# Rickyeeeeee/ParallelRayTracing

Measured on AMD Instinct MI355X. Metric: Mrays/sec at 1920x1080, 4 bounces, ~1M-tri scene, higher is better.
Workload: dtype f32; 1 GPU; C3: dragon.ply refined by longest-edge bisection = 870000 triangles + ground quad + emissive quad, 1920x1080, max_depth 5 segments (= 4 bounces), 256 spp per step (15360 spp timed of the config's 256), image tiled over 1 GPU(s) + per-step gather to rank 0; triangles=870000, bvh_nodes=681504, bvh_max_depth=25, bvh8_nodes=137301, bvh8_depth=9, width=1920, height=1080, max_depth=5, samples_in_flight=256, seed=0, jitter=0, variant=0, gather=render stream

## Files before the change

parallelraytracing_amd/csrc/prt_api.cpp:

```cpp
#include <hip/hip_runtime.h>

#include <algorithm>
#include <atomic>
#include <cfloat>
#include <chrono>
#include <cmath>
#include <cstdarg>
#include <cstdio>
#include <cstdlib>
#include <cstring>
#include <limits>
#include <string>
#include <utility>
#include <vector>

#include "../../include/prt.h"
#include "bvh.h"
#include "bvh_gpu.h"
#include "prt_adaptive.h"
#include "prt_denoise.h"
#include "prt_denoise_contract.h"
#include "prt_devmem.h"
#include "prt_feature_samples.h"
#include "prt_features.h"
// ... 12 lines not shown

int prt_dev_alloc(void** p, size_t bytes) {
    const hipError_t e = hipMalloc(p, bytes);
    if (e == hipSuccess) g_live_bytes += bytes, ++g_alloc_calls;
    return (int)e;
}
void prt_dev_free(void* p, size_t bytes) {
    (void)hipFree(p);
    g_live_bytes -= bytes;
}
int prt_dev_copy_in(void* dst, const void* src, size_t bytes) { return (int)hipMemcpy(dst, src, bytes, hipMemcpyHostToDevice); }
void prt_dev_adopted(size_t bytes) { g_live_bytes += bytes; }
void prt_dev_taken(size_t bytes) { g_live_bytes -= bytes; }
int prt_pinned_alloc(void** p, size_t bytes) { return (int)hipHostMalloc(p, bytes, hipHostMallocDefault); }
void prt_pinned_free(void* p) { (void)hipHostFree(p); }
int prt_event_create(void** ev, bool timing) {
    return (int)(timing ? hipEventCreate((hipEvent_t*)ev) : hipEventCreateWithFlags((hipEvent_t*)ev, hipEventDisableTiming));
}
void prt_event_destroy(void* ev) { (void)hipEventDestroy((hipEvent_t)ev); }

namespace {

constexpr float kPadCoeff = 1.0f / 262144.0f;
constexpr size_t kRayStatWords = (size_t)PRT_RAY_STAT_SLOTS * PRT_MAX_DEPTH;
constexpr uint32_t kTravStatsWords = 16 + PRT_TIMELINE_WORDS * (PRT_MAX_DEPTH + 1);
constexpr size_t kLightStatWords = 2 * (size_t)PRT_RAY_STAT_SLOTS;

struct EventPair {
    DevEvent a, b;
    int kind = 0;
};

hipEvent_t ev(const DevEvent& e) { return (hipEvent_t)e.h; }

struct RayMem {
    DevBuf o, d, t, hit, hd2;
    int alloc(uint64_t n) {
        int e = o.ensure(n * sizeof(float4));
        if (!e) e = d.ensure(n * sizeof(float4));
        if (!e) e = t.ensure(n * sizeof(float4));
        if (!e) e = hit.ensure(n * sizeof(uint32_t));
        if (!e) e = hd2.ensure(n * sizeof(float));
        return e;
    }
    PrtRayBuf view() const { return PrtRayBuf{o.as<float4>(), d.as<float4>(), t.as<float4>(), hit.as<uint32_t>(), hd2.as<float>()}; }
};
struct BuiltTree {
    DevBuf nodes8, tris, nrms;
    uint32_t n_nodes = 0;
};
struct SceneMem {
    DevBuf prims, mat_rgbs, mat_type, nodes, nodes4, nodes8, insts, tlas_inst, abvh_nodes, abvh_order, tris, nrms, lights, prim_light;
    DevBuf refit_keep;
};
struct MeshLightMem {
    DevBuf records, thr, bucket, runs;
    DevBuf lc_boxes, lc_range, lc_members, lc_thr, lc_cand, lc_pmf;
};
struct EnvMem {
    DevBuf texels, row, col, last;
};
struct TexMem {
    DevBuf texels, desc, mat, uvs, inst;
};
struct PathMem {
    RayMem rays[2];
    DevBuf rad;
};
struct LightMem {
    RayMem sh;
    DevBuf pdf_b, lrad;
};
struct PrimaryMem {
    DevBuf pid, list, hit;
};
struct FilmMem {
    DevBuf local;
    DevBuf stat;
    DevBuf tile_sel;
    PinnedBuf tile_count;
};
struct WorkMem {
    DevBuf counts;
    DevBuf ray_stats;
    DevBuf trav_stats;
    DevBuf work;
    DevBuf pix;
    DevBuf sort;
    DevBuf light_stats;
    PinnedBuf flag;
    PinnedBuf counts_host;
    DevEvent ev_counts[PRT_MAX_DEPTH + 2];
    DevEvent ev_prod[PRT_MAX_DEPTH + 2];
};

}

struct PrtContext {
    int device = -1;
    bool has_device = false;
    hipStream_t own_stream = nullptr;
    hipStream_t stream = nullptr;
    std::string err;

    bool has_scene = false;
    PrtHostScene hs;
    double refit_ms = 0.0;
    struct RefitKeep {
        bool ready = false;
        std::vector<uint32_t> tri_first, vert_first, level_start;
        uint32_t n_nodes = 0, n_light_tris = 0;
        uint32_t *d_corner = nullptr, *d_csr_start = nullptr, *d_csr_corner = nullptr, *d_light_tris = nullptr, *d_valid = nullptr;
        float *d_normals = nullptr, *d_light_verts = nullptr;
        PrtRefitScratch scratch{};
    } rk;
    bool host_copies_stale = false;
    PrtRefitInfo rinfo{};
    PrtCopyTally* tally = nullptr;
    PrtInstanceUpdateInfo inst_info{};
    DevScene dsc{};
    SceneMem scene;

    bool has_camera = false;
    DevCamera cam{};

    bool has_film = false;
    PrtTileMap tm{};
    uint32_t valid_local = 0;
    FilmMem film;
    bool film_stats = false;
    uint32_t tile_sel_entries = 0;

    uint32_t S = 1;
    uint64_t cap_paths = 0;
    PathMem path;
    PrtRayBuf rb[2] = {{nullptr, nullptr, nullptr, nullptr, nullptr}, {nullptr, nullptr, nullptr, nullptr, nullptr}};
    WorkMem wk;
    unsigned long long* ray_stats_target = nullptr;
    bool pix_records_blank = false;

    DevBuf scratch;

    bool timing = false;
    std::vector<EventPair> events;
    std::vector<EventPair> event_pool;
    PrtStats stats{};
    uint64_t dead_paths = 0;
    int variant = 0;
    int abvh_enabled = 1;
    int measure_spp = 1;
    float pad_coeff = kPadCoeff;
    int node_stride = 0;
    int compact_primary = 1;
    int primary_walk = 1;
    const char* shade_instance = "";
    const char* batch_instance[4] = {"", "", "", ""};
    bool batch_walked = false;
    int gpu_build = 0;
    PrtSampling sampling{0u, 0u, 0.0f};
    PrtLens lens{0.0f, 0.0f, 0.0f};
    PrtTravTuning tune{1024u, 256u, 16u, 0xFFFFFFFFu , 0u, 2u, 0u , 0u, 0u, 0u, 1u, 8u, 1u, 0u, nullptr, 0u, 2500000u, 2u , 8u , 96u , 32u , 1u};
    unsigned long long* d_shade_div = nullptr;
    uint32_t last_segment = 2;
    uint32_t last_segment_active = 0;
    uint32_t last_batch_depth = 0;
    uint32_t sort_rays = 0;
    size_t sort_entries = 0, sort_temp = 0;
    hipStream_t count_stream = nullptr;
    uint32_t pix_entries = 0;
    PrimaryMem prim;
    uint64_t prim_pid_entries = 0;
    uint32_t prim_pix_entries = 0;
    PrtPrimaryKey primary_key{};
    uint64_t camera_gen = 1, scene_gen = 1;
    uint32_t primary_counts[2] = {0u, 0u};
    int primary_reuse = 1;
    uint32_t primary_reuse_active = 0;
    uint32_t primary_reused_batches = 0;
    DevBuf spill;

    uint32_t lighting = PRT_LIGHTING_OFF;
    uint32_t light_sources = PRT_LIGHT_SOURCES_ANALYTIC;
    uint32_t light_selection = PRT_LIGHT_SELECTION_POWER;
    uint32_t light_max_clusters = 0;
    int light_buckets = 1;
    MeshLightMem ml;
    LightMem light;
    PrtLightBufs lb{};
    uint64_t cap_light = 0;

    PrtEnvTables env;
    EnvMem envm;
    uint64_t t_env_dev = 0;

    PrtTexTables tex;
    TexMem texm;
    uint64_t tex_bytes = 0;

    DevBuf feat;
    uint32_t feat_W = 0, feat_H = 0;
    bool feat_valid = false;
    PrtFeatureTrace ftrace{0u, 0.1f};
    DevBuf guide;
    bool guide_valid = false;
    PrtFeatureSampling fsamp{0u, 0u, 0u};
    DevBuf samp;
    bool samp_valid = false;
    int feature_chunk = 0;
    int radiance_chunk = 0;
    int bake_chunk = 0;
    DevBuf bake;
    DevBuf dn;
    DevBuf tp;
    DevBuf tp_mt;
    DevBuf tpa;
    uint32_t tp_W = 0, tp_H = 0;
    int tp_set = 0;
    bool tp_valid = false;
    PrtCameraBasis tp_K{};
    std::vector<float> tp_mats;
    std::vector<uint32_t> tp_mt_host;
    PrtTemporalInfo tp_info{};
    int dn_lds = 1;
};

namespace {

int fail(PrtContext* c, int code, const char* fmt, ...) {
    if (c) {
        char buf[512];
        va_list ap;
        va_start(ap, fmt);
        vsnprintf(buf, sizeof(buf), fmt, ap);
        va_end(ap);
        c->err = buf;
    }
    return code;
}

#define HIPCHECK(c, call)                                                                              \
    do {                                                                                               \
        const hipError_t e_ = (hipError_t)(call);                                                      \
        if (e_ != hipSuccess) return fail((c), PRT_ERR_HIP, "%s failed: %s", #call, hipGetErrorString(e_)); \
    } while (0)

int need_device(PrtContext* c) {
    if (!c) return PRT_ERR_INVALID;
    if (!c->has_device)
        return fail(c, PRT_ERR_NO_DEVICE,
                    "no HIP device bound to this context: the MI355X kernels are the only compute path (no CPU fallback)");
    const hipError_t e = hipSetDevice(c->device);
    if (e != hipSuccess) return fail(c, PRT_ERR_HIP, "hipSetDevice(%d) failed: %s", c->device, hipGetErrorString(e));
    return PRT_OK;
}

void drop_history(PrtContext* c) {
    c->tp_valid = false;
    c->tp_info.steps = 0;
    c->tp_info.hit_pixels = 0;
    c->tp_info.reprojected = 0;
    ++c->tp_info.resets;
}

int ensure(PrtContext* c, DevBuf& buf, size_t need) {
    HIPCHECK(c, buf.ensure(need));
    return PRT_OK;
}

int commit(PrtContext* c, const PrtWorkspace& ws, DevBuf& buf) {
    const int rc = ensure(c, buf, ws.bytes());
    if (rc || ws.bind(buf.p, buf.bytes)) return rc;
    return fail(c, PRT_ERR_INVALID, "a workspace of %d arrays in %zu bytes does not fit its buffer of %zu", ws.regions(), ws.bytes(), buf.bytes);
}

template <class T>
int upload(PrtContext* c, T* dst, const T* src, size_t count) {
    HIPCHECK(c, hipMemcpyAsync(dst, src, count * sizeof(T), hipMemcpyHostToDevice, c->stream));
    return PRT_OK;
}
template <class T>
int download(PrtContext* c, T* dst, const T* src, size_t count) {
    HIPCHECK(c, hipMemcpyAsync(dst, src, count * sizeof(T), hipMemcpyDeviceToHost, c->stream));
    return PRT_OK;
}

PrtFeatureBufs feature_view(void* base, size_t n) {
    float4* a = (float4*)base;
    return PrtFeatureBufs{a, a + n, a + 2 * n};
}

struct ChainScratch {
    float *o, *d;
    float4* s[4];
    uint32_t* cnt;
    void declare(PrtWorkspace& ws, size_t n) {
        ws.add(&o, 3 * n).add(&d, 3 * n);
        for (float4*& p : s) ws.add(&p, n);
        ws.add(&cnt, PRT_FEATURE_MAX_SPECULAR + 1u);
    }
};

struct FilterScratch {
    float4 *rec = nullptr, *cv0 = nullptr, *cv1 = nullptr;
    float *out = nullptr, *var = nullptr;
    void declare_arrays(PrtWorkspace& ws, size_t n) { ws.add(&rec, 3 * n).add(&cv0, n).add(&cv1, n); }
    int commit_film(PrtContext* c, size_t n) {
        PrtWorkspace ws;
        ws.add(&cv0, n).add(&cv1, n).add(&out, 3 * n).add(&var, n);
        return commit(c, ws, c->dn);
    }
};

void declare_history(PrtWorkspace& ws, PrtHistoryBufs* h, size_t n) { ws.add(&h->cn, n).add(&h->nrm, n).add(&h->pos, n).add(&h->mm, n); }

struct TemporalScratch {
    PrtHistoryBufs cur, prev, next;
    void declare(PrtWorkspace& ws, size_t n) {
        declare_history(ws, &cur, n);
        declare_history(ws, &prev, n);
        next.nrm = next.pos = nullptr;
        ws.add(&next.cn, n).add(&next.mm, n);
    }
};

int ensure_path_state(PrtContext* c, uint64_t n_paths) {
    if (n_paths <= c->cap_paths) return PRT_OK;
    c->path = PathMem();
    c->cap_paths = 0;
    const uint64_t n = std::max<uint64_t>(n_paths, 256);
    int e = c->path.rays[0].alloc(n);
    if (!e) e = c->path.rays[1].alloc(n);
    if (!e) e = c->path.rad.ensure(n * sizeof(float4));
    for (int i = 0; i < 2; ++i) c->rb[i] = c->path.rays[i].view();
    HIPCHECK(c, e);
    c->cap_paths = n;
    return PRT_OK;
}

void touch_scene(PrtContext* c) { ++c->scene_gen; }
void touch_camera(PrtContext* c) { ++c->camera_gen; }

int ensure_primary_state(PrtContext* c, uint64_t n_paths, uint32_t n_pix_local) {
    if (n_paths > c->prim_pid_entries) {
        c->primary_key.valid = false;
        c->prim_pid_entries = 0;
        const uint64_t n = std::max<uint64_t>(n_paths, 256);
        HIPCHECK(c, c->prim.pid.ensure(n * sizeof(uint32_t)));
        c->prim_pid_entries = n;
    }
    if (n_pix_local > c->prim_pix_entries) {
        c->primary_key.valid = false;
        c->prim_pix_entries = 0;
        const uint32_t n = std::max<uint32_t>(n_pix_local, 256u);
        HIPCHECK(c, c->prim.list.ensure((size_t)n * sizeof(uint32_t)));
        HIPCHECK(c, c->prim.hit.ensure((size_t)n * sizeof(uint32_t)));
        c->prim_pix_entries = n;
    }
    return PRT_OK;
}

int ensure_light_state(PrtContext* c, uint64_t n_paths) {
    if (!c->wk.light_stats.p) {
        HIPCHECK(c, c->wk.light_stats.ensure(kLightStatWords * sizeof(unsigned long long)));
        HIPCHECK(c, hipMemsetAsync(c->wk.light_stats.p, 0, kLightStatWords * sizeof(unsigned long long), c->stream));
    }
    c->lb.stats = c->wk.light_stats.as<unsigned long long>();
    if (n_paths <= c->cap_light) return PRT_OK;
    c->light = LightMem();
    c->cap_light = 0;
    const uint64_t n = std::max<uint64_t>(n_paths, 256);
    int e = c->light.sh.alloc(n);
    if (!e) e = c->light.pdf_b.ensure(n * sizeof(float));
    if (!e) e = c->light.lrad.ensure(n * sizeof(float4));
    c->lb.sh = c->light.sh.view();
    c->lb.pdf_b = c->light.pdf_b.as<float>();
    c->lb.lrad = c->light.lrad.as<float4>();
    HIPCHECK(c, e);
    c->cap_light = n;
    return PRT_OK;
}

bool mesh_lights_on(const PrtContext* c) { return (c->light_sources & PRT_LIGHT_SOURCES_MESH) != 0u; }

DevLights dev_lights(const PrtContext* c) {
    const uint32_t mode = c->lighting == PRT_LIGHTING_NEE ? (uint32_t)PRT_LIGHTING_NEE : (uint32_t)PRT_LIGHTING_NEE_MIS;
    if (mesh_lights_on(c)) return DevLights{c->ml.records.as<float4>(), c->scene.prim_light.as<uint32_t>(), c->hs.ml.n_search, mode};
    return DevLights{c->scene.lights.as<float4>(), c->scene.prim_light.as<uint32_t>(), (uint32_t)(c->hs.lights.size() / (4 * PRT_LIGHT_F4)), mode};
}

DevMeshLights dev_mesh_lights(const PrtContext* c) {
    return DevMeshLights{c->ml.thr.as<uint32_t>(), c->light_buckets ? c->ml.bucket.as<uint32_t>() : nullptr,
                         c->ml.runs.as<DevLightRun>(), c->hs.ml.bucket_shift, (uint32_t)c->hs.ml.runs.size()};
}

bool clusters_on(const PrtContext* c) { return mesh_lights_on(c) && c->light_selection == (uint32_t)PRT_LIGHT_SELECTION_CLUSTERED; }

DevLightClusters dev_light_clusters(const PrtContext* c) {
    const MeshLightMem& m = c->ml;
    return DevLightClusters{m.lc_boxes.as<float4>(), m.lc_range.as<uint4>(), m.lc_members.as<uint32_t>(),
                            m.lc_thr.as<uint32_t>(), m.lc_cand.as<uint32_t>(), m.lc_pmf.as<float>(), c->hs.lc.n_clusters()};
}

uint32_t light_set_size(const PrtContext* c) {
    return mesh_lights_on(c) ? (uint32_t)c->hs.ml.visible.size() : (uint32_t)(c->hs.lights.size() / (4 * PRT_LIGHT_F4));
}

bool env_on(const PrtContext* c) { return c->env.W != 0u; }
uint64_t env_threshold(const PrtContext* c) { return prt_environment_threshold(c->env, light_set_size(c)); }

DevEnv dev_env(const PrtContext* c) {
    const uint64_t te = env_threshold(c);
    return DevEnv{c->envm.texels.as<float4>(), c->envm.row.as<uint32_t>(), c->envm.col.as<uint32_t>(),
                  c->envm.last.as<uint32_t>(), c->env.W, c->env.H, c->env.row_last, (uint32_t)te, te == 4294967296ull ? 1u : 0u,
                  (float)((double)te / 4294967296.0)};
}

int upload_env(PrtContext* c) {
    HIPCHECK(c, hipSetDevice(c->device));
    HIPCHECK(c, hipStreamSynchronize(c->stream));
    c->envm = EnvMem();
    if (!env_on(c)) return PRT_OK;
    HIPCHECK(c, c->envm.texels.alloc_copy(c->env.texels.data(), c->env.texels.size() * 4));
    HIPCHECK(c, c->envm.row.alloc_copy(c->env.row_thr.data(), c->env.row_thr.size() * 4));
    HIPCHECK(c, c->envm.col.alloc_copy(c->env.col_thr.data(), c->env.col_thr.size() * 4));
    HIPCHECK(c, c->envm.last.alloc_copy(c->env.col_last.data(), c->env.col_last.size() * 4));
    return PRT_OK;
}

bool tex_on(const PrtContext* c) { return c->tex.is_set && c->tex.n_textured_materials != 0u; }

DevTex dev_tex(const PrtContext* c) {
    return DevTex{c->texm.texels.as<float4>(), c->texm.desc.as<uint4>(), c->texm.mat.as<uint32_t>(), c->texm.uvs.as<float2>(),
                  c->texm.inst.as<uint32_t>(), c->tex.n_textures};
}

void free_tex(PrtContext* c) {
    c->texm = TexMem();
    c->tex_bytes = 0;
}

int upload_tex(PrtContext* c) {
    HIPCHECK(c, hipSetDevice(c->device));
    HIPCHECK(c, hipStreamSynchronize(c->stream));
    free_tex(c);
    if (!c->tex.is_set) return PRT_OK;
    auto up = [&](DevBuf& dst, const auto& src) {
        const int e = dst.alloc_copy(src.data(), src.size() * 4);
        if (!e) c->tex_bytes += src.size() * 4;
        return e;
    };
    const PrtTexTables& t = c->tex;
    HIPCHECK(c, up(c->texm.texels, t.texels));
    HIPCHECK(c, up(c->texm.desc, t.desc));
    HIPCHECK(c, up(c->texm.mat, t.mat_tex));
    HIPCHECK(c, up(c->texm.uvs, t.uvs));
    HIPCHECK(c, up(c->texm.inst, t.inst_uv_base));
    return PRT_OK;
}

void drop_tex(PrtContext* c) {
    if (c->has_device && c->texm.texels.p) {
        (void)hipSetDevice(c->device);
        (void)hipStreamSynchronize(c->stream);
        free_tex(c);
    }
    c->tex = PrtTexTables();
}

int sync_light_tables(PrtContext* c) {
    const uint64_t te = env_threshold(c);
    if (te == c->t_env_dev || !c->has_device) return PRT_OK;
    std::vector<float> a, b;
    const bool ml = mesh_lights_on(c) && c->ml.records.p;
    prt_scaled_light_tables(c->hs, te, &a, ml ? &b : nullptr);
    HIPCHECK(c, hipSetDevice(c->device));
    HIPCHECK(c, hipStreamSynchronize(c->stream));
    if (!a.empty() && c->scene.lights.p) HIPCHECK(c, hipMemcpy(c->scene.lights.p, a.data(), a.size() * 4, hipMemcpyHostToDevice));
    if (!a.empty() && c->scene.lights.p && c->tally) c->tally->h2d += a.size() * 4;
    if (ml && !b.empty()) HIPCHECK(c, hipMemcpy(c->ml.records.p, b.data(), b.size() * 4, hipMemcpyHostToDevice));
    if (ml && !b.empty() && c->tally) c->tally->h2d += b.size() * 4;
    if (ml && c->ml.lc_pmf.p) {
        prt_cluster_pmf_in(c->hs, te, &a);
        if (!a.empty()) HIPCHECK(c, hipMemcpy(c->ml.lc_pmf.p, a.data(), a.size() * 4, hipMemcpyHostToDevice));
        if (!a.empty() && c->tally) c->tally->h2d += a.size() * 4;
    }
    c->t_env_dev = te;
    return PRT_OK;
}

int upload_mesh_lights(PrtContext* c) {
    static_assert(sizeof(DevLightRun) == sizeof(PrtLightRun), "DevLightRun is PrtLightRun");
    HIPCHECK(c, hipSetDevice(c->device));
    HIPCHECK(c, hipStreamSynchronize(c->stream));
    c->ml = MeshLightMem();
    const PrtMeshLights& ml = c->hs.ml;
    auto up = [&](DevBuf& dst, const void* src, size_t bytes) {
        const int e = dst.alloc_copy(src, bytes);
        if (!e && c->tally) c->tally->h2d += bytes;
        return e;
    };
    HIPCHECK(c, up(c->ml.records, ml.records.data(), ml.records.size() * 4));
    HIPCHECK(c, up(c->ml.thr, ml.thr.data(), ml.thr.size() * 4));
    HIPCHECK(c, up(c->ml.bucket, ml.bucket.data(), ml.bucket.size() * 4));
    HIPCHECK(c, up(c->ml.runs, ml.runs.data(), ml.runs.size() * sizeof(PrtLightRun)));
// ... 53 lines not shown
void free_scene(PrtContext* c) {
    drop_refit_keep(c);
    c->scene = SceneMem();
    c->ml = MeshLightMem();
    c->has_scene = false;
}

int read_ray_stats(PrtContext* c, const unsigned long long* d_set, unsigned long long (&out)[PRT_MAX_DEPTH]) {
    std::vector<unsigned long long> h(kRayStatWords);
    HIPCHECK(c, hipMemcpy(h.data(), d_set, kRayStatWords * sizeof(unsigned long long), hipMemcpyDeviceToHost));
    for (int d = 0; d < PRT_MAX_DEPTH; ++d) {
        out[d] = 0;
        for (size_t sl = 0; sl < PRT_RAY_STAT_SLOTS; ++sl) out[d] += h[sl * PRT_MAX_DEPTH + (size_t)d];
    }
    return PRT_OK;
}

int begin_event(PrtContext* c, int kind, EventPair* ep) {
    if (!c->timing) return PRT_OK;
    if (!c->event_pool.empty()) {
        *ep = std::move(c->event_pool.back());
        c->event_pool.pop_back();
    } else {
        HIPCHECK(c, ep->a.create(true));
        HIPCHECK(c, ep->b.create(true));
    }
    ep->kind = kind;
    HIPCHECK(c, hipEventRecord(ev(ep->a), c->stream));
    return PRT_OK;
}
int end_event(PrtContext* c, EventPair* ep) {
    if (!c->timing) return PRT_OK;
    HIPCHECK(c, hipEventRecord(ev(ep->b), c->stream));
    c->events.push_back(std::move(*ep));
    return PRT_OK;
}
int drain_events(PrtContext* c) {
    for (EventPair& ep : c->events) {
        float ms = 0.0f;
        HIPCHECK(c, hipEventSynchronize(ev(ep.b)));
        HIPCHECK(c, hipEventElapsedTime(&ms, ev(ep.a), ev(ep.b)));
        switch (ep.kind) {
            case 0: c->stats.raygen_ms += ms; break;
            case 1: c->stats.intersect_ms += ms; break;
            case 2: c->stats.shade_ms += ms; break;
            case 4: c->stats.scan_ms += ms; break;
            default: c->stats.accumulate_ms += ms; break;
        }
        c->event_pool.push_back(std::move(ep));
    }
    c->events.clear();
    return PRT_OK;
}

float lens_tan_fov_y(const PrtLens& l) { return l.fov_y == 0.0f ? tanf(0.5f) : tanf(0.5f * l.fov_y); }

f3 h_normalize(f3 v) {
    const float d = (v.x * v.x + v.y * v.y) + v.z * v.z;
    const float s = 1.0f / std::sqrt(d);
    return f3{v.x * s, v.y * s, v.z * s};
}
f3 h_cross(f3 a, f3 b) { return f3{a.y * b.z - b.y * a.z, a.z * b.x - b.z * a.x, a.x * b.y - b.x * a.y}; }

PrtBatchView whole_film(const PrtContext* c) { return PrtBatchView{c->tm, nullptr}; }

PrtWalkFacts walk_facts(const PrtContext* c, const PrtTravTuning& tune, PrtWalkRequest request, uint32_t max_rays, bool stats, bool primary) {
    PrtWalkFacts f{};
    f.has8 = c->dsc.nodes8 != nullptr, f.has4 = c->dsc.nodes4 != nullptr, f.has2 = c->dsc.nodes != nullptr;
    f.insts = c->dsc.n_insts != 0u, f.abvh = c->dsc.abvh_nodes != nullptr;
    f.depth8 = c->dsc.depth8, f.node_stride = c->dsc.node_stride, f.depth2 = c->hs.bvh.max_depth, f.max_stack4 = c->hs.bvh.max_stack4;
    f.wide = tune.wide, f.stack_lds = tune.stack_lds, f.stack_cap = tune.stack_cap, f.exit_max = tune.exit_max, f.tri_min = tune.tri_min;
    f.grid_blocks = tune.grid_blocks, f.steal = tune.steal, f.variant = c->variant, f.max_rays = max_rays, f.request = request, f.stats = stats, f.primary = primary;
    return f;
}

void walk_rays(PrtContext* c, const PrtRayBuf& rays, const uint32_t* count, uint32_t max_rays, bool any, const PrtTravTuning& tune,
               unsigned long long* stats, const PrtPrimary* primary, bool seeded = false) {
    const PrtWalkRequest request = !any ? PRT_WALK_CLOSEST : seeded ? PRT_WALK_SEEDED : PRT_WALK_ANY;
    const PrtWalkPlan plan = prt_plan_walk(walk_facts(c, tune, request, max_rays, stats != nullptr, primary != nullptr));
    prt_launch_walk(c->stream, plan, PrtWalkArgs{&c->dsc, rays, count, c->wk.work.as<uint32_t>(), c->spill.as<uint32_t>(), stats, primary, &tune});
}

int sort_front_rays(PrtContext* c, const PrtRayBuf& in, const uint32_t* front_count, uint32_t n_paths, EventPair* ep, PrtTravTuning* tune) {
    int rc;
    uint32_t n_front = 0;
    HIPCHECK(c, hipMemcpyAsync(&n_front, front_count, sizeof(uint32_t), hipMemcpyDeviceToHost, c->stream));
    HIPCHECK(c, hipStreamSynchronize(c->stream));
    if (n_front <= 1u) return PRT_OK;
    if (c->sort_entries < n_paths) {
        c->wk.sort = DevBuf();
        c->sort_entries = 0;
        c->sort_temp = prt_sort_rays_temp_bytes(n_paths);
        HIPCHECK(c, c->wk.sort.ensure(4 * (size_t)n_paths * sizeof(uint32_t) + c->sort_temp));
        c->sort_entries = n_paths;
    }
    EventPair es{};
    if ((rc = begin_event(c, 4, &es))) return rc;
    uint32_t* q = c->wk.sort.as<uint32_t>();
    if (prt_sort_rays(c->stream, in.o, in.d, n_front, c->dsc.root_min, c->dsc.root_max, c->sort_rays, q, q + n_paths,
                      q + 2 * (size_t)n_paths, q + 3 * (size_t)n_paths, q + 4 * (size_t)n_paths, c->sort_temp))
        return fail(c, PRT_ERR_HIP, "ray sort failed");
    if ((rc = end_event(c, &es))) return rc;
    if (c->timing) HIPCHECK(c, hipEventRecord(ev(ep->a), c->stream));
    tune->perm = q + 3 * (size_t)n_paths;
    return PRT_OK;
}

int run_batch(PrtContext* c, const PrtBatchView& view, uint32_t S_cur, uint32_t max_depth, uint32_t seed, uint32_t first_sample,
              bool accumulate, unsigned long long* trav_stats) {
    const PrtTileMap& tm = view.tm;
    if (view.list && !c->film.stat.p) return fail(c, PRT_ERR_INVALID, "a tile list needs film statistics");
    const uint64_t n_paths64 = (uint64_t)S_cur * tm.n_pix_local;
    c->batch_walked = false;
    c->primary_reuse_active = 0u;
    if (n_paths64 == 0) return PRT_OK;
    if (n_paths64 > 0xFFFFFF00ull) return fail(c, PRT_ERR_INVALID, "too many paths in flight");
    const uint32_t n_paths = (uint32_t)n_paths64;
    int rc = ensure_path_state(c, n_paths);
    if (rc) return rc;
    if ((rc = ensure_spill(c))) return rc;
    if ((rc = sync_light_tables(c))) return rc;
    const PrtWalkFacts wf = walk_facts(c, c->tune, PRT_WALK_PATH, n_paths, trav_stats != nullptr, false);
    PrtRouteFacts f{};
    f.lit = c->lighting != PRT_LIGHTING_OFF;
    f.mesh_lights = mesh_lights_on(c);
    f.light_clusters = clusters_on(c);
    f.env = env_on(c);
    f.tex = tex_on(c);
    f.lens = c->lens.aperture > 0.0f;
    f.listed = view.list != nullptr;
    f.film_stats = c->film_stats;
    f.has_nodes = c->dsc.n_nodes != 0u;
    f.has_bvh2 = wf.has2;
    f.insts = wf.insts;
    f.abvh = wf.abvh;
    f.few_prims = c->dsc.n_prims <= 16u;
    f.jitter = c->sampling.jitter != 0u;
    f.sa = c->sampling.rr_depth != 0u || c->sampling.clamp > 0.0f;
    f.multi_sample = S_cur > 1u;
    f.variant0 = wf.variant == 0;
    f.compact_primary = c->compact_primary;
    f.primary_walk = c->primary_walk;
    f.takes_primary = prt_traverse_takes_primary(wf);
    f.primary_hit = c->tune.primary_hit != 0u;
    f.path_gate = !trav_stats && !c->d_shade_div && c->sort_rays == 0u && n_paths <= c->tune.path_max && prt_path_kernel_applies(wf);
    f.path_kernel = c->tune.path_kernel;
    f.fuse = c->tune.fuse;
    f.mesh_emissive = c->hs.mesh_emissive;
    f.depth_ge2 = max_depth >= 2u;
    f.sort_rays = c->sort_rays != 0u;
    f.last_segment = c->last_segment;
    const PrtRoutePlan plan = prt_plan_route(f);
    const bool lit = f.lit, compact = plan.compact, walk = plan.walk;
    const DevEnv denv = dev_env(c);
    const DevTex dtex = dev_tex(c);
    const DevLens dlens{c->lens.aperture, c->lens.focus_distance};
    const bool exact = c->dsc.n_nodes != 0u && c->tune.exact_grids != 0u && (n_paths > (16384u * 512u) || c->tune.exact_grids == 2u);
    if (exact && !c->wk.counts_host.p) {
        HIPCHECK(c, c->wk.counts_host.alloc((PRT_MAX_DEPTH + 2) * 64 * sizeof(uint32_t)));
        for (DevEvent& e : c->wk.ev_counts) HIPCHECK(c, e.create(false));
        for (DevEvent& e : c->wk.ev_prod) HIPCHECK(c, e.create(false));
        HIPCHECK(c, hipStreamCreateWithFlags(&c->count_stream, hipStreamNonBlocking));
    }
    uint32_t* const d_counts = c->wk.counts.as<uint32_t>();
    uint32_t* const d_work = c->wk.work.as<uint32_t>();
    uint32_t* const h_counts = c->wk.counts_host.as<uint32_t>();
    float4* const d_rad = c->path.rad.as<float4>();
    auto read_back = [&](uint32_t d) -> hipError_t {
        hipError_t e = hipEventRecord(ev(c->wk.ev_prod[d]), c->stream);
        if (e == hipSuccess) e = hipStreamWaitEvent(c->count_stream, ev(c->wk.ev_prod[d]), 0);
        if (e == hipSuccess)
            e = hipMemcpyAsync(h_counts + 64 * (size_t)d, d_counts + (size_t)d * PRT_CNT_STRIDE, 33 * sizeof(uint32_t),
                               hipMemcpyDeviceToHost, c->count_stream);
        return e != hipSuccess ? e : hipEventRecord(ev(c->wk.ev_counts[d]), c->count_stream);
    };
    EventPair ep{};
    auto accumulate_batch = [&]() -> int {
        if ((rc = begin_event(c, 3, &ep))) return rc;
        const PrtAccumulateArgs aa{d_rad, lit ? c->lb.lrad : nullptr, c->film.local.as<float4>(), c->film.stat.as<float2>(), tm, S_cur, max_depth,
                                   accumulate, c->ray_stats_target, compact ? c->wk.pix.as<float4>() + tm.n_pix_local : nullptr, view.list};
        if (!prt_launch_accumulate(c->stream, plan.accumulate, aa)) return fail(c, PRT_ERR_INVALID, "no such accumulate instance");
        c->batch_instance[PRT_STAGE_ACCUMULATE] = prt_accumulate_name(plan.accumulate);
        if ((rc = end_event(c, &ep))) return rc;
        if (accumulate && !view.list) c->stats.samples += S_cur;
        HIPCHECK(c, hipGetLastError());
        return PRT_OK;
    };
    c->shade_instance = "";
    for (const char*& n : c->batch_instance) n = "";
    c->last_segment_active = plan.last_segment;
    c->last_batch_depth = plan.path ? 0u : max_depth;
    if (plan.path) {
        HIPCHECK(c, hipMemsetAsync(d_work, 0, 256 * sizeof(uint32_t), c->stream));
        PrtPathArgs pa{c->cam, tm, c->sampling, d_rad, first_sample, seed, max_depth, n_paths};
        if ((rc = begin_event(c, 1, &ep))) return rc;
        prt_launch_path(c->stream, prt_plan_walk(wf), c->dsc, pa, d_work, c->tune);
        if ((rc = end_event(c, &ep))) return rc;
        ++c->stats.intersect_launches;
        return accumulate_batch();
    }
    if (compact && c->pix_entries < tm.n_pix_local) {
        c->pix_entries = 0;
        c->primary_key.valid = false;
        HIPCHECK(c, c->wk.pix.ensure(4 * (size_t)tm.n_pix_local * sizeof(float4)));
        c->pix_entries = tm.n_pix_local;
        c->pix_records_blank = false;
    }
    const bool instrumented = trav_stats != nullptr || c->d_shade_div != nullptr;
    const bool persistent = compact && (walk || S_cur == 1u);
    if (persistent && (rc = ensure_primary_state(c, n_paths, tm.n_pix_local))) return rc;
    float4* const d_pix = c->wk.pix.as<float4>();
    PrtRayBuf rb0 = c->rb[0];
    if (persistent) rb0.t = c->prim.pid.as<float4>(), rb0.hd2 = c->prim.list.as<float>(), rb0.hit = c->prim.hit.as<uint32_t>();
    PrtPrimaryKey now{};
    now.valid = persistent && c->primary_reuse != 0 && !instrumented;
    if (now.valid) {
        const PrtWalkPlan wp0 = prt_plan_walk(walk_facts(c, c->tune, PRT_WALK_CLOSEST, walk ? tm.n_pix_local : n_paths, false, true));
        now.camera_gen = c->camera_gen, now.scene_gen = c->scene_gen;
        now.W = tm.W, now.H = tm.H, now.rank = tm.rank, now.world = tm.world, now.n_pix_local = tm.n_pix_local;
        now.S_cur = S_cur, now.max_depth = max_depth;
        now.plan = plan;
        now.walk_row = (uint32_t)wp0.launch[0].row, now.walk_prim = wp0.launch[0].prim;
        now.compact = compact, now.walk = walk, now.primary_hit = plan.primary_hit, now.lens = f.lens, now.jitter = f.jitter;
        now.rr_depth = c->sampling.rr_depth, now.clamp = c->sampling.clamp;
        now.listed = view.list != nullptr, now.instrumented = instrumented, now.exact = exact;
    }
    const bool reuse = prt_primary_reusable(c->primary_key, now);
    c->primary_reuse_active = reuse ? 1u : 0u;
    if (reuse) ++c->primary_reused_batches;
    if (reuse) HIPCHECK(c, hipMemsetAsync(d_counts + PRT_CNT_STRIDE, 0, (size_t)max_depth * PRT_CNT_STRIDE * sizeof(uint32_t), c->stream));
    else HIPCHECK(c, hipMemsetAsync(d_counts, 0, (size_t)(max_depth + 1) * PRT_CNT_STRIDE * sizeof(uint32_t), c->stream));
    const DevLights lt = dev_lights(c);
    const DevMeshLights mlt = dev_mesh_lights(c);
    const DevLightClusters lct = dev_light_clusters(c);
    if (lit) {
        if ((rc = ensure_light_state(c, n_paths))) return rc;
        HIPCHECK(c, hipMemsetAsync(c->lb.lrad, 0, (size_t)n_paths * sizeof(float4), c->stream));
    }
    c->batch_walked = walk;
    const PrtPrimary primary{(const uint32_t*)rb0.t, d_pix, {c->cam.pos.x, c->cam.pos.y, c->cam.pos.z}, tm.n_pix_local,
                             1.0f / (float)tm.n_pix_local, first_sample, seed, walk ? 1u : 0u};
    PrtPrimary primary_list = primary;
    if (walk) primary_list.pid = (const uint32_t*)rb0.hd2;
    c->batch_instance[PRT_STAGE_RAYGEN] = prt_raygen_name(plan.raygen);
    if (!reuse) {
        c->primary_key.valid = false;
        if ((rc = begin_event(c, 0, &ep))) return rc;
        const PrtRaygenArgs ra{&c->dsc, c->cam, tm, n_paths, first_sample, seed, max_depth, rb0, d_rad, d_counts, d_work, c->sampling,
                               compact ? d_pix : nullptr, walk, f.env ? &denv : nullptr, f.lens ? &dlens : nullptr, view.list};
        if (!prt_launch_raygen(c->stream, plan.raygen, ra)) return fail(c, PRT_ERR_INVALID, "no such raygen instance");
        if ((rc = end_event(c, &ep))) return rc;
        if (exact) HIPCHECK(c, read_back(0));
    }
    for (uint32_t d = 0; d < max_depth; ++d) {
        const PrtRayBuf& in = d == 0 ? rb0 : c->rb[d & 1];
        const PrtRayBuf& out = c->rb[(d + 1) & 1];
        const uint32_t* front_count = d_counts + (size_t)d * PRT_CNT_STRIDE;
        const PrtPrimary* prim_d = (compact && d == 0) ? &primary : nullptr;
        const bool held = reuse && d == 0;
        if (c->dsc.n_nodes && !held) {
            if ((rc = begin_event(c, 1, &ep))) return rc;
            PrtTravTuning tune = c->tune;
            tune.probe_slot = d;
            tune.perm = nullptr;
            if (plan.walk8 && c->sort_rays && !prim_d && (d > 0 || c->sampling.jitter || f.lens))
                if ((rc = sort_front_rays(c, in, front_count, n_paths, &ep, &tune))) return rc;
            if (walk && d == 0)
                walk_rays(c, in, d_counts + PRT_CNT_LIST, tm.n_pix_local, false, tune, trav_stats, &primary_list);
            else if (plan.last_segment == 2u && d + 1u == max_depth && !trav_stats)
                walk_rays(c, in, front_count, n_paths, true, tune, nullptr, nullptr, true);
            else
                walk_rays(c, in, front_count, n_paths, false, tune, trav_stats, prim_d);
            if ((rc = end_event(c, &ep))) return rc;
            ++c->stats.intersect_launches;
            if (prim_d) {
                if (plan.primary_hit) {
                    if ((rc = begin_event(c, 2, &ep))) return rc;
                    prt_launch_primary_hit(c->stream, c->dsc, primary, in.hit, d_pix, d_counts);
                    if ((rc = end_event(c, &ep))) return rc;
                    c->pix_records_blank = false;
                } else if (!c->pix_records_blank) {
                    HIPCHECK(c, hipMemsetAsync(d_pix + 2 * (size_t)tm.n_pix_local, 0xFF, 2 * (size_t)tm.n_pix_local * sizeof(float4), c->stream));
                    c->pix_records_blank = true;
                }
            }
        }
        uint32_t n_rays_known = 0xFFFFFFFFu;
        if (exact && held) {
            n_rays_known = c->primary_counts[0] + c->primary_counts[1];
        } else if (exact) {
            HIPCHECK(c, hipEventSynchronize(ev(c->wk.ev_counts[d])));
            n_rays_known = h_counts[64 * (size_t)d] + h_counts[64 * (size_t)d + 32];
            if (d == 0) c->primary_counts[0] = h_counts[0], c->primary_counts[1] = h_counts[32];
        }
        if (n_rays_known == 0u) break;
        if (d == 0 && !reuse && now.valid) c->primary_key = now;
        if (c->d_shade_div) prt_launch_shade_divstats(c->stream, c->dsc, in, d_counts, d, n_paths, c->d_shade_div, prim_d);
        if ((rc = begin_event(c, 2, &ep))) return rc;
        const PrtShadeInst shade = d == 0 ? plan.shade0 : plan.shade;
        const PrtShadeArgs sa{&c->dsc, in, out, d_rad, d_counts, d_work, d, max_depth, n_paths, c->sampling, n_rays_known, prim_d, plan.last_segment,
                              f.env ? &denv : nullptr, f.tex ? &dtex : nullptr, lit ? &lt : nullptr, (lit && f.mesh_lights) ? &mlt : nullptr,
                              lit ? &c->lb : nullptr, (lit && f.light_clusters) ? &lct : nullptr};
        if (!prt_launch_shade(c->stream, shade, sa)) return fail(c, PRT_ERR_INVALID, "no such shade instance");
        c->shade_instance = prt_shade_name(shade);
        c->batch_instance[(d == 0 && plan.shade0 != plan.shade) ? PRT_STAGE_SHADE0 : PRT_STAGE_SHADE] = c->shade_instance;
        if (lit && (lt.n_lights || (f.env && (denv.t_all | denv.t_env)))) {
            const uint32_t* scount = d_counts + (size_t)d * PRT_CNT_STRIDE + 48u;
            const uint32_t nmax = n_rays_known == 0xFFFFFFFFu ? n_paths : n_rays_known;
            prt_launch_scan_prims_bounded(c->stream, c->dsc, c->lb.sh, scount, d_work, nmax);
            if (c->dsc.n_nodes) walk_rays(c, c->lb.sh, scount, nmax, true, c->tune, nullptr, nullptr);
            prt_launch_light_accum(c->stream, c->dsc, c->lb, scount, d_work, nmax);
        }
        if ((rc = end_event(c, &ep))) return rc;
        if (exact && d + 1 < max_depth) HIPCHECK(c, read_back(d + 1));
    }
    return accumulate_batch();
}

void fill_dev_scene(PrtContext* c, uint32_t node_stride, uint32_t depth8) {
    const PrtSceneScalars& k = c->hs.sc;
    DevScene d{};
    const SceneMem& m = c->scene;
    d.prims = m.prims.as<DevPrim>();
    d.mat_rgbs = m.mat_rgbs.as<float4>();
    d.mat_type = m.mat_type.as<uint32_t>();
    d.nodes = m.nodes.as<float4>();
    d.nodes4 = m.nodes4.as<float4>();
    d.nodes8 = m.nodes8.as<uint4>();
    d.tris = m.tris.as<float4>();
    d.tri_normals = m.nrms.as<float4>();
    d.abvh_nodes = m.abvh_nodes.as<float4>();
    d.abvh_order = m.abvh_order.as<uint32_t>();
    d.insts = m.insts.as<DevInstance>();
    d.tlas_inst = m.tlas_inst.as<uint32_t>();
    d.n_insts = k.n_insts;
    d.node_stride = node_stride;
    d.depth8 = depth8;
    d.n_prims = k.n_prims;
    d.n_nodes = k.n_nodes;
    d.n_tris = k.n_tris;
    d.pad = k.pad;
    memcpy(d.abvh_q, k.abvh_q, sizeof(d.abvh_q));
    d.extent = k.extent;
    memcpy(d.root_min, k.root_min, sizeof(d.root_min));
    memcpy(d.root_max, k.root_max, sizeof(d.root_max));
    memcpy(d.sky, k.sky, sizeof(d.sky));
    c->dsc = d;
    touch_scene(c);
}

int upload_scene(PrtContext* c, BuiltTree* gb) {
    HIPCHECK(c, hipSetDevice(c->device));
    HIPCHECK(c, hipStreamSynchronize(c->stream));
    free_scene(c);
    SceneMem& m = c->scene;
    if (gb) {
        m.nodes8 = std::move(gb->nodes8);
        m.tris = std::move(gb->tris);
        m.nrms = std::move(gb->nrms);
    }
    const std::vector<uint32_t>& n8 = c->hs.nodes8_all.empty() ? c->hs.bvh.nodes8 : c->hs.nodes8_all;
    const size_t n_nodes8 = gb ? (size_t)gb->n_nodes : n8.size() / 20;
    const uint32_t node_stride = c->node_stride ? (uint32_t)c->node_stride : (n_nodes8 * 80 > ((size_t)64 << 20) ? 8u : 5u);
    if (node_stride == 8u && n_nodes8) {
        DevBuf wide;
        HIPCHECK(c, wide.ensure(128 * n_nodes8));
        hipError_t e = hipMemset(wide.p, 0, 128 * n_nodes8);
        if (e == hipSuccess)
            e = gb ? hipMemcpy2D(wide.p, 128, m.nodes8.p, 80, 80, n_nodes8, hipMemcpyDeviceToDevice)
                   : hipMemcpy2D(wide.p, 128, n8.data(), 80, 80, n_nodes8, hipMemcpyHostToDevice);
        if (e == hipSuccess) e = hipDeviceSynchronize();
        HIPCHECK(c, e);
        m.nodes8 = std::move(wide);
    }
    std::vector<float> rgbs(4 * c->hs.materials.size());
    std::vector<uint32_t> mtype(c->hs.materials.size());
    for (size_t i = 0; i < c->hs.materials.size(); ++i) {
        rgbs[4 * i + 0] = c->hs.materials[i].rgb[0];
        rgbs[4 * i + 1] = c->hs.materials[i].rgb[1];
        rgbs[4 * i + 2] = c->hs.materials[i].rgb[2];
        rgbs[4 * i + 3] = c->hs.materials[i].scalar;
        mtype[i] = c->hs.materials[i].type;
    }
    HIPCHECK(c, m.prims.alloc_copy(c->hs.prims.data(), c->hs.prims.size() * sizeof(DevPrim)));
    HIPCHECK(c, m.mat_rgbs.alloc_copy(rgbs.data(), rgbs.size() * 4));
    HIPCHECK(c, m.mat_type.alloc_copy(mtype.data(), mtype.size() * 4));
    if (!c->hs.scene_device_built) {
        HIPCHECK(c, m.nodes.alloc_copy(c->hs.bvh.nodes.data(), c->hs.bvh.nodes.size() * 4));
        HIPCHECK(c, m.nodes4.alloc_copy(c->hs.bvh.nodes4.data(), c->hs.bvh.nodes4.size() * 4));
    }
    if (!gb && !n8.empty() && node_stride != 8u) HIPCHECK(c, m.nodes8.alloc_copy(n8.data(), n8.size() * 4));
    if (!c->hs.abvh.nodes4.empty()) {
        HIPCHECK(c, m.abvh_nodes.alloc_copy(c->hs.abvh.nodes4.data(), c->hs.abvh.nodes4.size() * 4));
        HIPCHECK(c, m.abvh_order.alloc_copy(c->hs.abvh.order.data(), c->hs.abvh.order.size() * 4));
    }
    if (!c->hs.dev_insts.empty()) {
        HIPCHECK(c, m.insts.alloc_copy(c->hs.dev_insts.data(), c->hs.dev_insts.size() * sizeof(DevInstance)));
        HIPCHECK(c, m.tlas_inst.alloc_copy(c->hs.tlas_inst.data(), c->hs.tlas_inst.size() * 4));
    }
    HIPCHECK(c, m.lights.alloc_copy(c->hs.lights.data(), c->hs.lights.size() * 4));
    HIPCHECK(c, m.prim_light.alloc_copy(c->hs.prim_light.data(), c->hs.prim_light.size() * 4));
    if (!gb) {
        HIPCHECK(c, m.tris.alloc_copy(c->hs.tri_records.data(), c->hs.tri_records.size() * 4));
        HIPCHECK(c, m.nrms.alloc_copy(c->hs.nrm_records.data(), c->hs.nrm_records.size() * 4));
    }
    if (mesh_lights_on(c)) {
        const int rc_ml = upload_mesh_lights(c);
        if (rc_ml) return rc_ml;
    }
    fill_dev_scene(c, node_stride, c->hs.bvh_info.depth8);
    const int rc_cnt = ensure_counters(c);
    if (rc_cnt) return rc_cnt;
    c->has_scene = true;
    c->t_env_dev = 0;
    return sync_light_tables(c);
}

int device_build(PrtContext* c, const float* verts, const float* norms, const uint32_t* tri_mat, uint32_t n, uint32_t n_prims,
                 std::vector<uint32_t>& nodes8, uint32_t& depth, float* tri_rec, float* nrm_rec, BuiltTree* keep, float leaf_cost, double* ms,
                 int builder) {
    float cmin[3] = {FLT_MAX, FLT_MAX, FLT_MAX}, cmax[3] = {-FLT_MAX, -FLT_MAX, -FLT_MAX};
    for (size_t t = 0; t < (size_t)n; ++t)
        for (int a = 0; a < 3; ++a) {
            const float* v = &verts[9 * t];
            const float lo = std::min(v[a], std::min(v[3 + a], v[6 + a])), hi = std::max(v[a], std::max(v[3 + a], v[6 + a]));
            const float cc = 0.5f * lo + 0.5f * hi;
            cmin[a] = std::min(cmin[a], cc);
            cmax[a] = std::max(cmax[a], cc);
        }
    HIPCHECK(c, hipSetDevice(c->device));
    HIPCHECK(c, hipStreamSynchronize(c->stream));
    PrtGpuBvh gb{};
    int brc = 0;
    {
        DevBuf dv, dn, dm;
        hipError_t e = (hipError_t)dv.ensure(36 * (size_t)n);
        if (e == hipSuccess) e = (hipError_t)dn.ensure(36 * (size_t)n);
        if (e == hipSuccess) e = (hipError_t)dm.ensure(4 * (size_t)n);
        if (e == hipSuccess) e = hipMemcpy(dv.p, verts, 36 * (size_t)n, hipMemcpyHostToDevice);
        if (e == hipSuccess) e = norms ? hipMemcpy(dn.p, norms, 36 * (size_t)n, hipMemcpyHostToDevice) : hipMemsetAsync(dn.p, 0, 36 * (size_t)n, c->stream);
        if (e == hipSuccess) e = tri_mat ? hipMemcpy(dm.p, tri_mat, 4 * (size_t)n, hipMemcpyHostToDevice) : hipMemsetAsync(dm.p, 0, 4 * (size_t)n, c->stream);
        if (e != hipSuccess) return fail(c, PRT_ERR_HIP, "device-side BVH build: %s", hipGetErrorString(e));
        const auto t0 = std::chrono::steady_clock::now();
        brc = builder == 2 ? prt_gpu_bvh8_build(c->stream, dv.as<float>(), dn.as<float>(), dm.as<uint32_t>(), n, n_prims, cmin, cmax, &gb)
                           : prt_gpu_bvh8_build_ploc(c->stream, dv.as<float>(), dn.as<float>(), dm.as<uint32_t>(), n, n_prims, cmin, cmax, &gb, leaf_cost);
        *ms += std::chrono::duration<double, std::milli>(std::chrono::steady_clock::now() - t0).count();
    }
    if (brc < 0) {
        (void)fail(c, PRT_ERR_INVALID, "device-side BVH build gave up (%d)", brc);
// ... 2767 lines not shown

int prt_measure_shade_divergence(PrtContext* c, uint32_t max_depth, uint32_t seed, uint32_t sample, uint64_t* out) {
    int rc = check_ready(c);
    if (rc) return rc;
    if (!out || max_depth == 0 || max_depth > PRT_MAX_DEPTH) return PRT_ERR_INVALID;
    HIPCHECK(c, hipStreamSynchronize(c->stream));
    const size_t bytes = 16 * (size_t)PRT_MAX_DEPTH * sizeof(unsigned long long);
    DevBuf buf;
    HIPCHECK(c, buf.ensure(bytes));
    hipError_t e = hipMemsetAsync(buf.p, 0, bytes, c->stream);
    if (e == hipSuccess) {
        c->d_shade_div = buf.as<unsigned long long>();
        c->ray_stats_target = c->wk.ray_stats.as<unsigned long long>() + kRayStatWords;
        const bool timing = c->timing;
        const uint64_t launches = c->stats.intersect_launches;
        c->timing = false;
        rc = run_batch(c, whole_film(c), (uint32_t)std::max(1, c->measure_spp), max_depth, seed, sample, false, nullptr);
        c->timing = timing;
        c->stats.intersect_launches = launches;
        c->d_shade_div = nullptr;
        c->ray_stats_target = c->wk.ray_stats.as<unsigned long long>();
        if (!rc) e = hipStreamSynchronize(c->stream);
        if (!rc && e == hipSuccess) e = hipMemcpy(out, buf.p, 16 * (size_t)max_depth * sizeof(unsigned long long), hipMemcpyDeviceToHost);
    }
    if (rc) return rc;
    HIPCHECK(c, e);
    return PRT_OK;
}

int prt_kernel_occupancy(PrtContext* c, PrtOccupancy* out) {
    int rc = need_device(c);
    if (rc) return rc;
    if (!out) return PRT_ERR_INVALID;
    if (!c->has_scene) return fail(c, PRT_ERR_INVALID, "prt_set_scene has not been called");
    int nb = 0, vg = 0, sg = 0, lds = 0;
    const PrtWalkPlan plan = prt_plan_walk(walk_facts(c, c->tune, PRT_WALK_CLOSEST, 0u, false, false));
    if (prt_walk_occupancy(plan, &nb, &vg, &sg, &lds)) return fail(c, PRT_ERR_HIP, "occupancy query failed");
    hipDeviceProp_t prop;
    HIPCHECK(c, hipGetDeviceProperties(&prop, c->device));
    out->blocks_per_cu = (uint32_t)nb;
    out->waves_per_cu = (uint32_t)nb * 4u;
    out->max_waves_per_cu = (uint32_t)(prop.maxThreadsPerMultiProcessor / 64);
    out->vgprs = (uint32_t)vg;
    out->lds_bytes_per_block = (uint32_t)lds;
    out->compute_units = (uint32_t)prop.multiProcessorCount;
    out->resident_grid_blocks = plan.resident_grid;
    return PRT_OK;
}

int prt_kernel_instance(PrtContext* c, char* name, uint32_t capacity) {
    if (!c || !name || capacity == 0u) return PRT_ERR_INVALID;
    if (!c->has_scene) return fail(c, PRT_ERR_INVALID, "prt_set_scene has not been called");
    snprintf(name, capacity, "%s", prt_plan_walk(walk_facts(c, c->tune, PRT_WALK_CLOSEST, 0u, false, false)).name);
    return PRT_OK;
}

int prt_shade_instance(PrtContext* c, char* name, uint32_t capacity) {
    if (!c || !name || capacity == 0u) return PRT_ERR_INVALID;
    snprintf(name, capacity, "%s", c->shade_instance);
    return PRT_OK;
}

int prt_batch_instance(PrtContext* c, uint32_t stage, char* name, uint32_t capacity) {
    if (!c || !name || capacity == 0u || stage > PRT_STAGE_ACCUMULATE) return PRT_ERR_INVALID;
    snprintf(name, capacity, "%s", c->batch_instance[stage]);
    return PRT_OK;
}

int prt_instance_name(uint32_t stage, uint32_t index, char* name, uint32_t capacity) {
    if (!name || capacity == 0u) return PRT_ERR_INVALID;
    const char* s = nullptr;
    if (stage == PRT_STAGE_RAYGEN && index < PRT_RAYGEN_NONE) s = prt_raygen_name(PrtRaygenInst(index));
    else if ((stage == PRT_STAGE_SHADE0 || stage == PRT_STAGE_SHADE) && index < PRT_SHADE_NONE) s = prt_shade_name(PrtShadeInst(index));
    else if (stage == PRT_STAGE_ACCUMULATE && index < PRT_ACCUMULATE_NONE) s = prt_accumulate_name(PrtAccumulateInst(index));
    if (!s) return PRT_ERR_INVALID;
    snprintf(name, capacity, "%s", s);
    return PRT_OK;
}

int prt_last_segment(PrtContext* c, uint32_t* active, uint32_t* front_rays) {
    if (!c || !active) return PRT_ERR_INVALID;
    *active = c->last_segment_active;
    if (front_rays) {
        *front_rays = 0u;
        if (c->last_batch_depth != 0u && c->wk.counts.p) {
            HIPCHECK(c, hipSetDevice(c->device));
            HIPCHECK(c, hipStreamSynchronize(c->stream));
            HIPCHECK(c, hipMemcpy(front_rays, c->wk.counts.as<uint32_t>() + (size_t)(c->last_batch_depth - 1u) * PRT_CNT_STRIDE, sizeof(uint32_t),
                                  hipMemcpyDeviceToHost));
        }
    }
    return PRT_OK;
}

int prt_primary_reuse(PrtContext* c, uint32_t* active, uint32_t* reused_batches) {
    if (!c || !active) return PRT_ERR_INVALID;
    *active = c->primary_reuse_active;
    if (reused_batches) *reused_batches = c->primary_reused_batches;
    return PRT_OK;
}

int prt_bvh_info(PrtContext* c, PrtBvhInfo* out) {
    if (!c || !out) return PRT_ERR_INVALID;
    if (!c->has_scene) return fail(c, PRT_ERR_INVALID, "prt_set_scene has not been called");
    *out = c->hs.bvh_info;
    return PRT_OK;
}

int prt_bvh_read4(PrtContext* c, float* nodes4) {
    if (!c) return PRT_ERR_INVALID;
    if (!c->has_scene) return fail(c, PRT_ERR_INVALID, "prt_set_scene has not been called");
    if (nodes4) memcpy(nodes4, c->hs.bvh.nodes4.data(), c->hs.bvh.nodes4.size() * 4);
    return PRT_OK;
}

int prt_bvh_read8(PrtContext* c, uint32_t* nodes8) {
    if (!c) return PRT_ERR_INVALID;
    if (!c->has_scene) return fail(c, PRT_ERR_INVALID, "prt_set_scene has not been called");
    if (const int rc = refresh_host_copies(c)) return rc;
    const std::vector<uint32_t>& n8 = c->hs.nodes8_all.empty() ? c->hs.bvh.nodes8 : c->hs.nodes8_all;
    if (nodes8) memcpy(nodes8, n8.data(), n8.size() * 4);
    return PRT_OK;
}

int prt_bvh_read(PrtContext* c, float* nodes, float* tris) {
    if (!c) return PRT_ERR_INVALID;
    if (!c->has_scene) return fail(c, PRT_ERR_INVALID, "prt_set_scene has not been called");
    if (const int rc = refresh_host_copies(c)) return rc;
    if (nodes) memcpy(nodes, c->hs.bvh.nodes.data(), c->hs.bvh.nodes.size() * 4);
    if (tris) memcpy(tris, c->hs.tri_records.data(), c->hs.tri_records.size() * 4);
    return PRT_OK;
}

int prt_set_param(PrtContext* c, const char* name, int value) {
    if (!c || !name) return PRT_ERR_INVALID;
    touch_scene(c);
    const std::string n = name;
    if (n == "variant") c->variant = value;
    else if (n == "primary_reuse" && (value == 0 || value == 1)) c->primary_reuse = value;
    else if (n == "grid_blocks" && value > 0 && value <= 8192) c->tune.grid_blocks = (uint32_t)value;
    else if (n == "chunk" && value >= 64 && value % 64 == 0) c->tune.chunk = (uint32_t)value;
    else if (n == "xcd_affinity" && (value == 0 || value == 1)) c->tune.xcd_affinity = (uint32_t)value;
    else if (n == "wide" && (value == 0 || value == 1 || value == 2)) c->tune.wide = (uint32_t)value;
    else if (n == "stack_lds" && (value == 0 || value == 1 || value == 2 || value == 3 || value == 4 || value == 5 || value == 6 || value == 24 || value == 39)) c->tune.stack_lds = (uint32_t)value;
    else if (n == "exact_grids" && (value == 0 || value == 1 || value == 2)) c->tune.exact_grids = (uint32_t)value;
    else if (n == "steal" && value >= 0 && value <= 64) c->tune.steal = (uint32_t)value;
    else if (n == "primary_hit" && (value == 0 || value == 1)) c->tune.primary_hit = (uint32_t)value;
    else if (n == "path_kernel" && value >= 0 && value <= 2) c->tune.path_kernel = (uint32_t)value;
    else if (n == "path_max" && value >= 1) c->tune.path_max = (uint32_t)value;
    else if (n == "sort_rays" && value >= 0 && value <= 2) c->sort_rays = (uint32_t)value;
    else if (n == "last_segment" && value >= 0 && value <= 2) c->last_segment = (uint32_t)value;
    else if (n == "compact_primary" && (value == 0 || value == 1)) c->compact_primary = value;
    else if (n == "primary_walk" && (value == 0 || value == 1)) c->primary_walk = value;
    else if (n == "node_stride" && (value == 0 || value == 5 || value == 8)) c->node_stride = value;
    else if (n == "pad_log2" && value >= 8 && value <= 22) c->pad_coeff = std::ldexp(1.0f, -value);
    else if (n == "tail" && value >= 0 && value <= 64) c->tune.tail = (uint32_t)value;
    else if (n == "big" && value >= 1 && value <= 16) c->tune.big = (uint32_t)value;
    else if (n == "static_small" && value >= 0 && value <= 4096) c->tune.static_small = (uint32_t)value;
    else if (n == "big_min" && value >= 1 && value <= 100000) c->tune.big_min = (uint32_t)value;
    else if (n == "big_keep" && value >= 0 && value <= 1024) c->tune.big_keep = (uint32_t)value;
    else if (n == "stack_cap" && value >= 0 && value <= 64) c->tune.stack_cap = (uint32_t)value;
    else if (n == "prim_bvh" && (value == 0 || value == 1)) c->abvh_enabled = value;
    else if (n == "measure_spp" && value >= 1 && value <= 1024) c->measure_spp = value;
    else if (n == "gpu_build" && (value == 0 || value == 1 || value == 2)) c->gpu_build = value;
    else if (n == "fuse" && (value == 0 || value == 1)) c->tune.fuse = (uint32_t)value;
    else if (n == "tri_min" && value >= 0 && value <= 1024) c->tune.tri_min = (uint32_t)value;
    else if (n == "refill_min" && value >= 1 && value <= 64) c->tune.refill_min = (uint32_t)value;
    else if (n == "light_buckets" && (value == 0 || value == 1)) c->light_buckets = value;
    else if (n == "denoise_lds" && value >= 0 && value <= 2) c->dn_lds = value;
    else if (n == "feature_chunk" && value >= 0 && value <= (int)PRT_FEATURE_MAX_SAMPLES) c->feature_chunk = value;
    else if (n == "radiance_chunk" && value >= 0 && value <= (int)PRT_RADIANCE_MAX_SAMPLES) c->radiance_chunk = value;
    else if (n == "bake_chunk" && value >= 0 && value <= (int)PRT_RADIANCE_MAX_SAMPLES) c->bake_chunk = value;
    else if (n == "exit_max" && value >= 0 && value < 64) c->tune.exit_max = (uint32_t)value;
    else return fail(c, PRT_ERR_INVALID, "unknown parameter or bad value: %s = %d", name, value);
    return PRT_OK;
}

int prt_set_variant(PrtContext* c, int variant) {
    if (!c) return PRT_ERR_INVALID;
    touch_scene(c);
    c->variant = variant;
    return PRT_OK;
}

}
```

parallelraytracing_amd/csrc/prt_kernels.h:

```cpp
#pragma once
#include <hip/hip_runtime_api.h>
#include <hip/hip_vector_types.h>
#include <stdint.h>

#include "../../include/prt.h"
#include "prt_route.h"
#include "prt_walk.h"
#include "prt_scene_pod.h"

struct f3 {
    float x, y, z;
};

struct DevCamera {
    f3 pos, front, right, up;
    float W, H, tan_fov_y;
};
struct DevLens {
    float aperture, focus;
};

#define PRT_DIR_MIN 9.094947017729282e-13f

struct DevScene {
    const DevPrim* prims;
    const float4* mat_rgbs;
    const uint32_t* mat_type;
    const float4* nodes;
    const float4* nodes4;
    const uint4* nodes8;
    const float4* tris;
    const float4* tri_normals;
    const float4* abvh_nodes;
    const uint32_t* abvh_order;
    const DevInstance* insts;
    const uint32_t* tlas_inst;
    uint32_t n_insts;
    uint32_t node_stride;
    uint32_t depth8;
    uint32_t n_prims;
    uint32_t n_nodes;
    uint32_t n_tris;
    float pad;
    float abvh_q[3];
    float extent;
    float root_min[3], root_max[3];
    float sky[3];
};

struct PrtTileMap {
    uint32_t W, H, tiles_x, tiles_y, rank, world;
    uint32_t n_tiles_local;
    uint32_t n_pix_local;
    uint32_t stride;
};

struct PrtBatchView {
    PrtTileMap tm;
    const uint32_t* list;
};

#define PRT_TIMELINE_WORDS 8
#define PRT_RAY_STAT_SLOTS 256u

struct PrtRayBuf {
    float4* o;
    float4* d;
    float4* t;
    uint32_t* hit;
    float* hd2;
};

struct PrtPrimary {
    const uint32_t* pid;
    const float4* pix;
    float origin[3];
    uint32_t n_pix_local;
    float inv_n;
    uint32_t first_sample, seed;
    uint32_t walk;
};

struct PrtPathArgs {
    DevCamera cam;
    PrtTileMap tm;
    PrtSampling sp;
    float4* rad;
    uint32_t first_sample, seed, max_depth, n_paths;
};

#define PRT_CNT_STRIDE 64u
#define PRT_CNT_LIST 8u

struct DevLights {
    const float4* lights;
    const uint32_t* prim_light;
    uint32_t n_lights;
    uint32_t mode;
};
struct DevLightRun {
    uint32_t prim_first, n_tris, light_first, world;
};
struct DevMeshLights {
    const uint32_t* thr;
    const uint32_t* bucket;
    const DevLightRun* runs;
    uint32_t bucket_shift;
    uint32_t n_runs;
};
struct DevLightClusters {
    const float4* boxes;
    const uint4* range;
    const uint32_t* members;
    const uint32_t* thr;
    const uint32_t* cand_cluster;
    const float* cand_pmf_in;
    uint32_t n_clusters;
};
struct DevEnv {
    const float4* texels;
    const uint32_t* row_thr;
    const uint32_t* col_thr;
    const uint32_t* col_last;
    uint32_t W, H;
    uint32_t row_last;
    uint32_t t_env;
    uint32_t t_all;
    float p_env;
};

struct DevTex {
    const float4* texels;
    const uint4* desc;
    const uint32_t* mat_tex;
    const float2* uvs;
    const uint32_t* inst_uv_base;
    uint32_t n_textures;
};

struct PrtLightBufs {
    PrtRayBuf sh;
    float* pdf_b;
    float4* lrad;
    unsigned long long* stats;
};

struct PrtRaygenArgs {
    const DevScene* sc;
    DevCamera cam;
    PrtTileMap tm;
    uint32_t n_paths, first_sample, seed, max_depth;
    PrtRayBuf out;
    float4* rad;
    uint32_t* counts;
    uint32_t* work;
    PrtSampling sp;
    float4* compact_pix;
    bool primary_walk;
    const DevEnv* env;
    const DevLens* lens;
    const uint32_t* list;
};
bool prt_launch_raygen(hipStream_t st, PrtRaygenInst inst, const PrtRaygenArgs& a);
void prt_launch_scan_prims(hipStream_t st, const DevScene& sc, const PrtRayBuf& in, const uint32_t* count_ptr,
                           uint32_t* work, uint32_t max_rays, unsigned long long* stats);
struct PrtWalkArgs {
    const DevScene* sc;
    PrtRayBuf rays;
    const uint32_t* count;
    uint32_t* work;
    uint32_t* spill;
    unsigned long long* stats;
    const PrtPrimary* primary;
    const PrtTravTuning* tune;
};
void prt_launch_walk(hipStream_t st, const PrtWalkPlan& plan, const PrtWalkArgs& a);
void prt_launch_path(hipStream_t st, const PrtWalkPlan& plan, const DevScene& sc, const PrtPathArgs& pa, uint32_t* work, const PrtTravTuning& tune);
int prt_walk_occupancy(const PrtWalkPlan& plan, int* blocks_per_cu, int* vgprs, int* sgprs, int* lds_bytes);
#define PRT_LAST_SEGMENT_FLAG 0x80000000u
struct PrtShadeArgs {
    const DevScene* sc;
    PrtRayBuf in, out;
    float4* rad;
    uint32_t* counts;
    uint32_t* work;
    uint32_t depth, max_depth, cap;
    PrtSampling sp;
    uint32_t n_rays_known;
    const PrtPrimary* primary;
    uint32_t last_segment;
    const DevEnv* env;
    const DevTex* tex;
    const DevLights* lights;
    const DevMeshLights* mesh_lights;
    const PrtLightBufs* lb;
    const DevLightClusters* clusters;
};
bool prt_launch_shade(hipStream_t st, PrtShadeInst inst, const PrtShadeArgs& a);
void prt_launch_shade_divstats(hipStream_t st, const DevScene& sc, const PrtRayBuf& in, const uint32_t* counts, uint32_t iter,
                               uint32_t cap, unsigned long long* out, const PrtPrimary* primary = nullptr);
void prt_launch_primary_hit(hipStream_t st, const DevScene& sc, const PrtPrimary& pr, const uint32_t* hit, float4* pix,
                            const uint32_t* counts);
struct PrtAccumulateArgs {
    const float4* rad;
    const float4* lrad;
    float4* film_local;
    float2* stat;
    PrtTileMap tm;
    uint32_t S, max_depth;
    bool update_film;
    unsigned long long* ray_stats;
    const float4* pix_end;
    const uint32_t* list;
};
bool prt_launch_accumulate(hipStream_t st, PrtAccumulateInst inst, const PrtAccumulateArgs& a);
void prt_launch_resolve(hipStream_t st, const float4* gathered, uint32_t world, uint32_t stride, uint32_t W,
                        uint32_t H, float* rgb, float* weight);
void prt_launch_tonemap(hipStream_t st, const float* rgb, const float* weight, uint32_t n_pix, float exposure,
                        float inv_gamma, uint8_t* out);
void prt_launch_camera_rays(hipStream_t st, const DevCamera& cam, uint32_t n, const float* px, const float* py,
                            float* o, float* d);
void prt_launch_camera_rays_lens(hipStream_t st, const DevCamera& cam, const DevLens& lens, uint32_t n, const float* px,
                                 const float* py, uint32_t* keys, float* o, float* d);
void prt_launch_pack_rays(hipStream_t st, uint32_t n, const float* o, const float* d, const PrtRayBuf& out,
                          uint32_t* counts);
void prt_launch_hit_records(hipStream_t st, const DevScene& sc, uint32_t n, const PrtRayBuf& in, PrtHit* out);
void prt_launch_pack_occlusion_rays(hipStream_t st, uint32_t n, const float* o, const float* d, const float* tmax,
                                    const PrtRayBuf& out, uint32_t* counts);
void prt_launch_scan_prims_bounded(hipStream_t st, const DevScene& sc, const PrtRayBuf& in, const uint32_t* count_ptr,
                                   uint32_t* work, uint32_t max_rays);
void prt_launch_occlusion_bytes(hipStream_t st, const DevScene& sc, uint32_t n, const PrtRayBuf& in, const float* tmax,
                                uint8_t* out);
void prt_launch_scatter_test(hipStream_t st, const DevScene& sc, uint32_t n, const float* in_d, const PrtHit* hits,
                             uint32_t* rng_io, uint32_t* scattered, float* atten, float* emitted, float* o_out,
                             float* d_out);
void prt_launch_light_accum(hipStream_t st, const DevScene& sc, const PrtLightBufs& lb, const uint32_t* count_ptr,
                            uint32_t* work, uint32_t max_rays);
void prt_launch_sample_light_test(hipStream_t st, const DevScene& sc, const DevLights& lt, uint32_t n, const float* in_d,
                                  const PrtHit* hits, const uint32_t* keys, float* out_f, uint32_t* out_light,
                                  const DevMeshLights* ml = nullptr, const DevEnv* env = nullptr, const DevLightClusters* lc = nullptr);
void prt_launch_light_cluster_pmf(hipStream_t st, const DevLightClusters& lc, uint32_t n, const float* x, uint32_t* M);
void prt_launch_environment_eval(hipStream_t st, const DevEnv& env, uint32_t n, const float* dirs, float* rgb, uint32_t* texel,
                                 float* pdf_w);
void prt_launch_texture_eval(hipStream_t st, const DevTex& tex, uint32_t n, const uint32_t* texture, const float* uv, float* rgb);
void prt_launch_hit_uv(hipStream_t st, const DevScene& sc, const DevTex& tex, uint32_t n, const PrtRayBuf& in, float* uv, float* albedo);

void prt_launch_tile_select(hipStream_t st, const float4* film_local, const float2* stat, const PrtTileMap& tm, const uint32_t* prev,
                            uint32_t n_in, float threshold, float noise_floor, uint32_t* flags, uint32_t* out, uint32_t* count);
```

parallelraytracing_amd/csrc/prt_kernels.hip:

```cpp
#include "prt_kernels.h"

#include "prt_adaptive.h"
#include "prt_device.h"

#define HIT_MISS 0xFFFFFFFFu
#define HIT_DEAD 0xFFFFFFFEu

PRT_DEV uint32_t xcd_remap(uint32_t b, uint32_t n) {
    const uint32_t q = n >> 3, r = n & 7u;
    const uint32_t xcd = b & 7u, i = b >> 3;
    const uint32_t start = xcd < r ? xcd * (q + 1u) : r * (q + 1u) + (xcd - r) * q;
    return start + i;
}

#define CNT_STRIDE PRT_CNT_STRIDE
#define CNT_A(c, d) (c)[(d) * CNT_STRIDE]
#define CNT_B(c, d) (c)[(d) * CNT_STRIDE + 32u]
#define CNT_C(c, d) (c)[(d) * CNT_STRIDE + 16u]
#define PRODUCER_BLOCK 1024
#ifndef SHADE_BLOCK
#define SHADE_BLOCK 512
#endif

template <int BLOCK>
PRT_DEV uint32_t block_alloc2(bool front, bool back, bool done, uint32_t* cntA, uint32_t* cntB, uint32_t* cntC,
                              uint32_t cap, uint32_t mult = 1u, uint32_t* stride = nullptr, uint32_t* base = nullptr) {
    __shared__ uint32_t s_a[BLOCK / 64], s_b[BLOCK / 64], s_c[BLOCK / 64];
    __shared__ uint32_t s_base_a, s_base_b, s_tot_a, s_tot_b;
    const unsigned long long ma = __ballot(front), mb = __ballot(back), mc = __ballot(done);
    const uint32_t lane = lane_id(), wave = threadIdx.x >> 6;
    if (lane == 0) {
        s_a[wave] = (uint32_t)__popcll(ma);
        s_b[wave] = (uint32_t)__popcll(mb);
        s_c[wave] = (uint32_t)__popcll(mc);
    }
    __syncthreads();
    if (threadIdx.x == 0) {
        uint32_t ta = 0, tb = 0, tc = 0;
        for (uint32_t w = 0; w < BLOCK / 64; ++w) {
            ta += s_a[w];
            tb += s_b[w];
            tc += s_c[w];
        }
        s_base_a = ta ? atomicAdd(cntA, ta * mult) : 0u;
        s_base_b = tb ? atomicAdd(cntB, tb * mult) : 0u;
        if (tc) atomicAdd(cntC, tc);
        s_tot_a = ta;
        s_tot_b = tb;
    }
    __syncthreads();
    uint32_t slot = 0xFFFFFFFFu;
    if (front) {
        uint32_t j = s_base_a + (uint32_t)__popcll(ma & ((1ull << lane) - 1ull));
        for (uint32_t w = 0; w < wave; ++w) j += s_a[w];
        slot = j;
        if (stride) *stride = s_tot_a;
        if (base) *base = s_base_a;
    } else if (back) {
        uint32_t j = s_base_b + (uint32_t)__popcll(mb & ((1ull << lane) - 1ull));
        for (uint32_t w = 0; w < wave; ++w) j += s_b[w];
        slot = cap - 1u - j;
        if (stride) *stride = s_tot_b;
        if (base) *base = s_base_b;
    }
    return slot;
}

template <int BLOCK, int K>
PRT_DEV void block_alloc2k(const bool (&front)[K], const bool (&back)[K], uint32_t* cntA, uint32_t* cntB, uint32_t cap,
                           uint32_t (&slot)[K]) {
    __shared__ uint32_t s_a[BLOCK / 64], s_b[BLOCK / 64];
    __shared__ uint32_t s_base_a, s_base_b;
    const uint32_t lane = lane_id(), wave = threadIdx.x >> 6;
    const unsigned long long below = (1ull << lane) - 1ull;
    uint32_t ja[K], jb[K], na = 0, nb = 0;
#pragma unroll
    for (int k = 0; k < K; ++k) {
        const unsigned long long ma = __ballot(front[k]), mb = __ballot(back[k]);
        ja[k] = na + (uint32_t)__popcll(ma & below);
        jb[k] = nb + (uint32_t)__popcll(mb & below);
        na += (uint32_t)__popcll(ma);
        nb += (uint32_t)__popcll(mb);
    }
    if (lane == 0) {
        s_a[wave] = na;
        s_b[wave] = nb;
    }
    __syncthreads();
    if (threadIdx.x == 0) {
        uint32_t ta = 0, tb = 0;
        for (uint32_t w = 0; w < BLOCK / 64; ++w) {
            ta += s_a[w];
            tb += s_b[w];
        }
        s_base_a = ta ? atomicAdd(cntA, ta) : 0u;
        s_base_b = tb ? atomicAdd(cntB, tb) : 0u;
    }
    __syncthreads();
    uint32_t wa = s_base_a, wb = s_base_b;
    for (uint32_t w = 0; w < wave; ++w) {
        wa += s_a[w];
        wb += s_b[w];
    }
#pragma unroll
    for (int k = 0; k < K; ++k) slot[k] = front[k] ? wa + ja[k] : back[k] ? cap - 1u - (wb + jb[k]) : 0xFFFFFFFFu;
}

PRT_DEV bool tile_pixel(const PrtTileMap& tm, uint32_t pl, uint32_t& x, uint32_t& y) {
    const uint32_t lt = pl >> 6, lane = pl & 63u;
    const uint32_t gt = lt * tm.world + tm.rank;
    const uint32_t tx = gt % tm.tiles_x, ty = gt / tm.tiles_x;
    x = tx * 8u + (lane & 7u);
    y = ty * 8u + (lane >> 3);
    return gt < tm.tiles_x * tm.tiles_y && x < tm.W && y < tm.H;
}

PRT_DEV void primary_ray(const PrtPrimary& pr, uint32_t i, f3& o, f3& d, uint32_t& pixel, uint32_t& sample, uint32_t* local_pixel = nullptr) {
    uint32_t q = (uint32_t)((float)i * pr.inv_n);
    uint32_t r = i - q * pr.n_pix_local;
    if ((int32_t)r < 0) {
        --q;
        r += pr.n_pix_local;
    }
    if (r >= pr.n_pix_local) {
        ++q;
        r -= pr.n_pix_local;
    }
    sample = q;
    if (local_pixel) *local_pixel = r;
    const float4 P = pr.pix[r];
    o = mk3(pr.origin[0], pr.origin[1], pr.origin[2]);
    d = mk3(P.x, P.y, P.z);
    pixel = __float_as_uint(P.w);
}

template <bool ABVH, int BLOCK>
__device__ bool classify_ray(const DevScene& sc, f3 o, f3 d, uint32_t& id0, float& d2_0);
__device__ bool ends_here(const DevScene& sc, bool front, uint32_t id0, f3 thr, f3& L);

PRT_DEV float4 path_result(f3 L, float clamp, uint32_t depth) {
    if (clamp > 0.0f) {
        L.x = L.x > clamp ? clamp : L.x;
        L.y = L.y > clamp ? clamp : L.y;
        L.z = L.z > clamp ? clamp : L.z;
    }
    return make_float4(L.x, L.y, L.z, __uint_as_float(depth));
}


template <int BUDGET, bool INST, bool ABVH, int BLOCK, bool PRE = false, bool ENV = false, bool TEX = false, bool LASTSEG = false>
PRT_DEV int advance_path(const DevScene& sc, uint32_t id, f3& o, f3& d, f3& thr, uint32_t& rng, uint32_t& depth,
                         uint32_t max_depth, const PrtSampling& sp, float4* __restrict__ rad_slot, uint32_t& id0,
                         float& d2_0, float4 pre_a = float4{0.f, 0.f, 0.f, 0.f}, float4 pre_b = float4{0.f, 0.f, 0.f, 0.f},
                         const DevEnv* env = nullptr, const DevTex* tex = nullptr, bool last_route = false) {
#pragma unroll
    for (int it = 0; it <= BUDGET; ++it) {
        if (id == HIT_MISS) {
            st_stream(rad_slot, path_result(thr * (ENV ? env_radiance(*env, d) : mk3(sc.sky[0], sc.sky[1], sc.sky[2])), sp.clamp, depth));
            return 0;
        }
        if (LASTSEG && last_route && it == 0 && depth + 1u >= max_depth && id >= sc.n_prims) {
            st_stream(rad_slot, path_result(thr * mk3(0.f, 0.f, 0.f), sp.clamp, depth));
            return 0;
        }
        if (it == BUDGET) {
            const uint32_t m = sc.prims[id].material;
            if (sc.mat_type[m] == 4u) {
                const float4 e = sc.mat_rgbs[m];
                st_stream(rad_slot, path_result(thr * mk3(e.x, e.y, e.z), sp.clamp, depth));
                return 0;
            }
            id0 = id;
            return 2;
        }
        WorldHit w;
        float uv[2] = {0.0f, 0.0f};
        if (PRE && it == 0 && __float_as_uint(pre_a.w) == id) {
            w.pos = mk3(pre_a.x, pre_a.y, pre_a.z);
            w.normal = mk3(pre_b.x, pre_b.y, pre_b.z);
            w.material = __float_as_uint(pre_b.w) & 0x7FFFFFFFu;
            w.front = (__float_as_uint(pre_b.w) >> 31) != 0u;
        } else if (TEX) {
            world_hit_from_id<INST, true>(sc, id, o, d, w, tex, uv);
        } else {
            world_hit_from_id<INST>(sc, id, o, d, w);
        }
        const uint32_t type = sc.mat_type[w.material];
        const float4 rgbs = TEX ? textured_rgbs(sc, *tex, w.material, uv) : sc.mat_rgbs[w.material];
        f3 atten, emitted, so, sd;
        bool scattered = false;
        if (depth + 1u >= max_depth) {
            emitted = (type == 4u) ? mk3(rgbs.x, rgbs.y, rgbs.z) : mk3(0.f, 0.f, 0.f);
        } else {
            scattered = material_scatter(type, rgbs, d, w.pos, w.normal, w.front, rng, atten, emitted, so, sd);
        }
        if (!scattered) {
            st_stream(rad_slot, path_result(thr * emitted, sp.clamp, depth));
            return 0;
        }
        thr = thr * atten;
        o = so;
        d = normalize3(sd);
        if (sp.rr_depth != 0u && depth + 1u >= sp.rr_depth) {
            float p = thr.x > thr.y ? thr.x : thr.y;
            p = p > thr.z ? p : thr.z;
            p = p > 1.0f ? 1.0f : p;
            p = p < 0.05f ? 0.05f : p;
            if (!(rnd01(rng) < p)) {
                st_stream(rad_slot, path_result(mk3(0.f, 0.f, 0.f), 0.0f, depth));
                return 0;
            }
            thr = mk3(thr.x / p, thr.y / p, thr.z / p);
        }
        ++depth;
        if (LASTSEG) {
            const bool front = classify_ray<ABVH, BLOCK>(sc, o, d, id0, d2_0);
            if (last_route && depth + 1u >= max_depth && id0 != HIT_MISS && sc.mat_type[sc.prims[id0].material] != 4u) {
                st_stream(rad_slot, path_result(thr * mk3(0.f, 0.f, 0.f), sp.clamp, depth));
                return 0;
            }
            if (front) return 1;
        } else if (classify_ray<ABVH, BLOCK>(sc, o, d, id0, d2_0)) return 1;
        id = id0;
    }
    return 2;
}

#define RAYGEN_GROUP 8
#ifndef RAYGEN_ALLOC
#define RAYGEN_ALLOC 4
#endif
#define RAYGEN_GROUP_NOJITTER 64u
template <bool JITTER, bool SAMPLING, bool ABVH, bool COMPACT, bool ENV, bool LENS = false, bool LIST = false>
PRT_DEV void raygen_step(DevScene sc, DevCamera cam, PrtTileMap tm, uint32_t S, uint32_t first_sample, uint32_t seed,
                         float4* __restrict__ ro, float4* __restrict__ rd, float4* __restrict__ rt, uint32_t* __restrict__ hit,
                         float* __restrict__ hd2, float4* __restrict__ rad, uint32_t* __restrict__ counts,
                         uint32_t* __restrict__ work, uint32_t max_depth, PrtSampling sp_arg, float4* __restrict__ pix,
                         const DevEnv* env, const DevLens* lens = nullptr, const uint32_t* __restrict__ list = nullptr) {
    const PrtSampling sp = SAMPLING ? sp_arg : PrtSampling{0u, 0u, 0.0f};
    const uint32_t pl = blockIdx.x * (uint32_t)PRODUCER_BLOCK + threadIdx.x;
    if (blockIdx.y == 0 && pl < 8u) work[32u * pl] = 0u;
    if (blockIdx.y == 0 && pl == 8u) work[512] = 0u;
    const uint32_t n_paths = S * tm.n_pix_local;
    const bool in_range = pl < tm.n_pix_local;
    bool valid = false, front0 = false;
    f3 o0 = mk3(0.f, 0.f, 0.f), d0 = mk3(0.f, 0.f, 1.f);
    uint32_t id00 = HIT_MISS, pixel = 0, px = 0, py = 0;
    float d2_00 = 3.402823466e+38f;
    if (in_range) {
        valid = tile_pixel(tm, LIST ? (list[pl >> 6] << 6) | (pl & 63u) : pl, px, py);
        if (valid) {
            pixel = py * tm.W + px;
            if (!JITTER && !LENS) {
                camera_ray(cam, (float)px + 0.5f, (float)py + 0.5f, o0, d0);
                if (COMPACT && blockIdx.y == 0) pix[pl] = make_float4(d0.x, d0.y, d0.z, __uint_as_float(pixel));
                front0 = classify_ray<ABVH, PRODUCER_BLOCK>(sc, o0, d0, id00, d2_00);
            }
        }
    }
    const uint32_t group = (JITTER || LENS) ? RAYGEN_GROUP : RAYGEN_GROUP_NOJITTER;
    const uint32_t s0 = blockIdx.y * group;
    const uint32_t s1 = (s0 + group < S) ? s0 + group : S;
    if (!JITTER && !LENS) {
        f3 o = o0, d = d0, thr = mk3(1.f, 1.f, 1.f);
        uint32_t rng = 0, depth = 0, id0 = id00;
        float d2_0 = d2_00;
        float4 L0 = make_float4(0.f, 0.f, 0.f, __uint_as_float(0xFFFFFFFFu));
        bool front = false, back = false;
        if (valid) {
            front = front0;
            if (!front) {
                const int r = advance_path<0, false, ABVH, PRODUCER_BLOCK, false, ENV>(sc, id00, o, d, thr, rng, depth, max_depth, sp, &L0, id0, d2_0,
                                                                                         float4{0.f, 0.f, 0.f, 0.f}, float4{0.f, 0.f, 0.f, 0.f}, env);
                back = r == 2;
            }
        }
        uint32_t stride = 0, base = 0;
        const uint32_t slot0 = block_alloc2<PRODUCER_BLOCK>(front, back, false, &CNT_A(counts, 0), &CNT_B(counts, 0),
                                                            &CNT_C(counts, 0), n_paths, s1 - s0, &stride, &base);
        uint32_t first_slot = slot0;
        const bool walk = COMPACT && hd2 != nullptr;
        uint32_t list_slot = 0xFFFFFFFFu;
        if (walk && blockIdx.y == 0) {
            __shared__ uint32_t s_list_base;
            if (front && slot0 == base) s_list_base = atomicAdd(&counts[PRT_CNT_LIST], stride);
            __syncthreads();
            if (front) {
                list_slot = s_list_base + (slot0 - base);
                ((uint32_t*)hd2)[list_slot] = pl;
            }
        }
        if (s1 - s0 < 8u) {
            if (in_range && slot0 != 0xFFFFFFFFu) {
                for (uint32_t sl = s0; sl < s1; ++sl) {
                    const uint32_t i = sl * tm.n_pix_local + pl;
                    const uint32_t slot = front ? slot0 + (sl - s0) * stride : slot0 - (sl - s0) * stride;
                    if (COMPACT) {
                        ((uint32_t*)rt)[slot] = i;
                    } else {
                        ro[slot] = make_float4(o.x, o.y, o.z, __uint_as_float(i));
                        rd[slot] = make_float4(d.x, d.y, d.z, __uint_as_float(path_seed(pixel, first_sample + sl, seed)));
                        rt[slot] = make_float4(1.f, 1.f, 1.f, __uint_as_float(0u));
                    }
                    if (!COMPACT) {
                        hit[slot] = id0;
                        hd2[slot] = d2_0;
                    }
                }
            }
        } else {
            const uint32_t mult = s1 - s0;
            const bool stored = slot0 != 0xFFFFFFFFu;
            uint32_t first = 0u;
            if (front) first = base + (slot0 - base) * mult;
            if (back) first = n_paths - 1u - (base + ((n_paths - 1u - slot0) - base) * mult);
            first_slot = first;
            const uint32_t lane = lane_id();
            for (unsigned long long m = __ballot(stored); m; m &= m - 1ull) {
                const int p = __builtin_ctzll(m);
                const uint32_t f = (uint32_t)__builtin_amdgcn_readlane((int)first, p);
                const bool fr = __builtin_amdgcn_readlane((int)front, p) != 0;
                const uint32_t plp = (uint32_t)__builtin_amdgcn_readlane((int)pl, p);
                const uint32_t idp = (uint32_t)__builtin_amdgcn_readlane((int)id0, p);
                const float d2p = __uint_as_float((uint32_t)__builtin_amdgcn_readlane((int)__float_as_uint(d2_0), p));
                float4 Op = make_float4(0.f, 0.f, 0.f, 0.f), Dp = Op;
                uint32_t pixp = 0u;
                if (!COMPACT) {
#define PRT_RL(X) __uint_as_float((uint32_t)__builtin_amdgcn_readlane((int)__float_as_uint(X), p))
                    Op = make_float4(PRT_RL(o.x), PRT_RL(o.y), PRT_RL(o.z), 0.f);
                    Dp = make_float4(PRT_RL(d.x), PRT_RL(d.y), PRT_RL(d.z), 0.f);
#undef PRT_RL
                    pixp = (uint32_t)__builtin_amdgcn_readlane((int)pixel, p);
                }
                if (lane < mult) {
                    const uint32_t slot = fr ? f + lane : f - lane;
                    const uint32_t i = (s0 + lane) * tm.n_pix_local + plp;
                    if (COMPACT) {
                        ((uint32_t*)rt)[slot] = i;
                    } else {
                        ro[slot] = make_float4(Op.x, Op.y, Op.z, __uint_as_float(i));
                        rd[slot] = make_float4(Dp.x, Dp.y, Dp.z, __uint_as_float(path_seed(pixp, first_sample + s0 + lane, seed)));
                        rt[slot] = make_float4(1.f, 1.f, 1.f, __uint_as_float(0u));
                    }
                    if (!COMPACT) {
                        hit[slot] = idp;
                        hd2[slot] = d2p;
                    }
                }
            }
        }
        {
            const bool stored = slot0 != 0xFFFFFFFFu;
            if (COMPACT) {
                if (in_range && blockIdx.y == 0)
                    pix[tm.n_pix_local + pl] = stored ? make_float4(__uint_as_float(walk ? list_slot : first_slot), __uint_as_float(id0), d2_0, __uint_as_float(0xFFFFFFFEu)) : L0;
            } else if (in_range && !stored) {
                for (uint32_t sl = s0; sl < s1; ++sl) rad[sl * tm.n_pix_local + pl] = L0;
            }
        }
        return;
    }
    constexpr int KA = (ABVH || LENS) ? 2 : RAYGEN_ALLOC;
    for (uint32_t sl = s0; sl < s1; sl += KA) {
        f3 dk[KA];
        f3 ok[KA];
        uint32_t rngk[KA], idk[KA], slotk[KA];
        float d2k[KA];
        bool frontk[KA], backk[KA];
#pragma unroll
        for (int kk = 0; kk < KA; ++kk) {
            const uint32_t sk = sl + (uint32_t)kk;
            const uint32_t i = sk * tm.n_pix_local + pl;
            f3 o = o0, d = d0, thr = mk3(1.f, 1.f, 1.f);
            uint32_t rng = 0, depth = 0, id0 = id00;
            float d2_0 = d2_00;
            bool front = false, back = false;
            if (sk < s1 && valid) {
                rng = path_seed(pixel, first_sample + sk, seed);
                {
                    const float u1 = JITTER ? rnd01(rng) : 0.5f;
                    const float u2 = JITTER ? rnd01(rng) : 0.5f;
                    if (LENS)
                        lens_camera_ray(cam, *lens, (float)px + u1, (float)py + u2, rng, o, d);
                    else
                        camera_ray(cam, (float)px + u1, (float)py + u2, o, d);
                    front = classify_ray<ABVH, PRODUCER_BLOCK>(sc, o, d, id0, d2_0);
                }
                if (!front) {
                    const int r = advance_path<0, false, ABVH, PRODUCER_BLOCK, false, ENV>(sc, id0, o, d, thr, rng, depth, max_depth, sp, &rad[i], id0, d2_0,
                                                                                             float4{0.f, 0.f, 0.f, 0.f}, float4{0.f, 0.f, 0.f, 0.f}, env);
                    front = r == 1;
                    back = r == 2;
                }
            } else if (sk < s1 && in_range) {
                rad[i] = make_float4(0.f, 0.f, 0.f, __uint_as_float(0xFFFFFFFFu));
            }
            dk[kk] = d;
            if (LENS) ok[kk] = o;
            rngk[kk] = rng;
            idk[kk] = id0;
            d2k[kk] = d2_0;
            frontk[kk] = front;
            backk[kk] = back;
        }
        block_alloc2k<PRODUCER_BLOCK, KA>(frontk, backk, &CNT_A(counts, 0), &CNT_B(counts, 0), n_paths, slotk);
#pragma unroll
        for (int kk = 0; kk < KA; ++kk) {
            const uint32_t slot = slotk[kk];
            if (slot != 0xFFFFFFFFu) {
                const uint32_t i = (sl + (uint32_t)kk) * tm.n_pix_local + pl;
                const f3 ok_ = LENS ? ok[kk] : cam.pos;
                ro[slot] = make_float4(ok_.x, ok_.y, ok_.z, __uint_as_float(i));
                rd[slot] = make_float4(dk[kk].x, dk[kk].y, dk[kk].z, __uint_as_float(rngk[kk]));
                rt[slot] = make_float4(1.f, 1.f, 1.f, __uint_as_float(0u));
                hit[slot] = idk[kk];
                hd2[slot] = d2k[kk];
            }
        }
        __syncthreads();
    }
}

template <bool JITTER, bool SAMPLING, bool ABVH, bool COMPACT = false>
__global__ void __launch_bounds__(PRODUCER_BLOCK) k_raygen(DevScene sc, DevCamera cam, PrtTileMap tm, uint32_t S,
                                                            uint32_t first_sample, uint32_t seed,
                                                            float4* __restrict__ ro, float4* __restrict__ rd,
                                                            float4* __restrict__ rt, uint32_t* __restrict__ hit,
                                                            float* __restrict__ hd2, float4* __restrict__ rad,
                                                            uint32_t* __restrict__ counts, uint32_t* __restrict__ work,
                                                            uint32_t max_depth, PrtSampling sp_arg, float4* __restrict__ pix) {
    raygen_step<JITTER, SAMPLING, ABVH, COMPACT, false>(sc, cam, tm, S, first_sample, seed, ro, rd, rt, hit, hd2, rad, counts, work,
                                                        max_depth, sp_arg, pix, nullptr);
}

template <bool JITTER, bool ABVH>
__global__ void __launch_bounds__(PRODUCER_BLOCK) k_raygen_env(DevScene sc, DevEnv env, DevCamera cam, PrtTileMap tm, uint32_t S,
                                                                uint32_t first_sample, uint32_t seed,
                                                                float4* __restrict__ ro, float4* __restrict__ rd,
                                                                float4* __restrict__ rt, uint32_t* __restrict__ hit,
                                                                float* __restrict__ hd2, float4* __restrict__ rad,
                                                                uint32_t* __restrict__ counts, uint32_t* __restrict__ work,
                                                                uint32_t max_depth, PrtSampling sp_arg) {
    raygen_step<JITTER, true, ABVH, false, true>(sc, cam, tm, S, first_sample, seed, ro, rd, rt, hit, hd2, rad, counts, work,
                                                 max_depth, sp_arg, nullptr, &env);
}

template <bool JITTER, bool ABVH>
__global__ void __launch_bounds__(PRODUCER_BLOCK) k_raygen_lens(DevScene sc, DevLens lens, DevCamera cam, PrtTileMap tm, uint32_t S,
                                                                 uint32_t first_sample, uint32_t seed,
                                                                 float4* __restrict__ ro, float4* __restrict__ rd,
                                                                 float4* __restrict__ rt, uint32_t* __restrict__ hit,
                                                                 float* __restrict__ hd2, float4* __restrict__ rad,
                                                                 uint32_t* __restrict__ counts, uint32_t* __restrict__ work,
                                                                 uint32_t max_depth, PrtSampling sp_arg) {
    raygen_step<JITTER, true, ABVH, false, false, true>(sc, cam, tm, S, first_sample, seed, ro, rd, rt, hit, hd2, rad, counts, work,
                                                        max_depth, sp_arg, nullptr, nullptr, &lens);
}
template <bool JITTER, bool ABVH>
__global__ void __launch_bounds__(PRODUCER_BLOCK) k_raygen_lens_env(DevScene sc, DevEnv env, DevLens lens, DevCamera cam, PrtTileMap tm,
                                                                     uint32_t S, uint32_t first_sample, uint32_t seed,
                                                                     float4* __restrict__ ro, float4* __restrict__ rd,
                                                                     float4* __restrict__ rt, uint32_t* __restrict__ hit,
                                                                     float* __restrict__ hd2, float4* __restrict__ rad,
                                                                     uint32_t* __restrict__ counts, uint32_t* __restrict__ work,
                                                                     uint32_t max_depth, PrtSampling sp_arg) {
    raygen_step<JITTER, true, ABVH, false, true, true>(sc, cam, tm, S, first_sample, seed, ro, rd, rt, hit, hd2, rad, counts, work,
                                                       max_depth, sp_arg, nullptr, &env, &lens);
}

template <bool JITTER, bool ABVH, bool ENV, bool LENS>
__global__ void __launch_bounds__(PRODUCER_BLOCK) k_raygen_list(DevScene sc, DevEnv env, DevLens lens, DevCamera cam, PrtTileMap tm,
                                                                 const uint32_t* __restrict__ list, uint32_t S,
                                                                 uint32_t first_sample, uint32_t seed,
                                                                 float4* __restrict__ ro, float4* __restrict__ rd,
                                                                 float4* __restrict__ rt, uint32_t* __restrict__ hit,
                                                                 float* __restrict__ hd2, float4* __restrict__ rad,
                                                                 uint32_t* __restrict__ counts, uint32_t* __restrict__ work,
                                                                 uint32_t max_depth, PrtSampling sp_arg) {
    raygen_step<JITTER, true, ABVH, false, ENV, LENS, true>(sc, cam, tm, S, first_sample, seed, ro, rd, rt, hit, hd2, rad, counts, work,
                                                            max_depth, sp_arg, nullptr, ENV ? &env : nullptr, LENS ? &lens : nullptr,
                                                            list);
}

struct Closest {
    float d2;
    uint32_t id;
    uint32_t prim;
};

PRT_DEV float limit_from_d2(float d2, float pad) {
    return (d2 < 3.0e38f) ? __builtin_sqrtf(d2) * 1.0000153f + 4.0f * pad : 3.4e38f;
}

#define ABVH_STACK 20
template <bool ABVH, int BLOCK = 1>
PRT_DEV void scan_analytic(const DevScene& sc, f3 o, f3 d, Closest& best, uint32_t& n_tests) {
    if (!ABVH) {
        for (uint32_t i = 0; i < sc.n_prims; ++i) {
            WorldHit w;
            analytic_hit(sc.prims[i], o, d, w);
            ++n_tests;
            if (w.has && w.d2 < best.d2) {
                best.d2 = w.d2;
                best.id = i;
                best.prim = i;
            }
        }
        return;
    }
    const f3 ld = normalize3(d);
    const float A1 = __builtin_fabsf(o.x) + __builtin_fabsf(o.y) + __builtin_fabsf(o.z);
    const float pad = sc.pad * (A1 + sc.extent) + ((sc.abvh_q[0] * A1 + sc.abvh_q[1]) * A1 + sc.abvh_q[2]);
    const float ix = 1.0f / (__builtin_fabsf(ld.x) < PRT_DIR_MIN ? __builtin_copysignf(PRT_DIR_MIN, ld.x) : ld.x);
    const float iy = 1.0f / (__builtin_fabsf(ld.y) < PRT_DIR_MIN ? __builtin_copysignf(PRT_DIR_MIN, ld.y) : ld.y);
    const float iz = 1.0f / (__builtin_fabsf(ld.z) < PRT_DIR_MIN ? __builtin_copysignf(PRT_DIR_MIN, ld.z) : ld.z);
    const float ax = (o.x + pad) * ix, ay = (o.y + pad) * iy, az = (o.z + pad) * iz;
    const float bx = (o.x - pad) * ix, by = (o.y - pad) * iy, bz = (o.z - pad) * iz;
    float tlimit = limit_from_d2(best.d2, pad);
    __shared__ uint32_t s_astk[ABVH ? ABVH_STACK * BLOCK : 1];
    uint32_t* const stk = &s_astk[threadIdx.x];
    const uint32_t sstride = (uint32_t)BLOCK;
    int sp = 0;
    uint32_t node = 0;
    for (;;) {
        const float4* nb = sc.abvh_nodes + 8 * (size_t)node;
        const float4 mnx = nb[0], mxx = nb[1], mny = nb[2], mxy = nb[3], mnz = nb[4], mxz = nb[5], rf = nb[6];
#define ABVH_CHILD(C)                                                                                              \
    {                                                                                                              \
        const float x0 = __builtin_fmaf(mnx.C, ix, -ax), x1 = __builtin_fmaf(mxx.C, ix, -bx);                      \
        const float y0 = __builtin_fmaf(mny.C, iy, -ay), y1 = __builtin_fmaf(mxy.C, iy, -by);                      \
        const float z0 = __builtin_fmaf(mnz.C, iz, -az), z1 = __builtin_fmaf(mxz.C, iz, -bz);                      \
        const float tn = __builtin_fmaxf(__builtin_fmaxf(__builtin_fminf(x0, x1), __builtin_fminf(y0, y1)),        \
                                         __builtin_fmaxf(__builtin_fminf(z0, z1), 0.0f));                          \
        const float tf = __builtin_fminf(__builtin_fminf(__builtin_fmaxf(x0, x1), __builtin_fmaxf(y0, y1)),        \
                                         __builtin_fminf(__builtin_fmaxf(z0, z1), tlimit));                        \
        if (tn <= tf * 1.0000005f) {                                                                               \
            const int ref = __float_as_int(rf.C);                                                                  \
            if (ref >= 0) {                                                                                        \
                stk[(sp++) * sstride] = (uint32_t)ref;                                                             \
            } else {                                                                                               \
                const uint32_t lr = ~(uint32_t)ref, first = lr >> 4, cnt = lr & 15u;                               \
                for (uint32_t k = 0; k < cnt; ++k) {                                                               \
                    const uint32_t i = sc.abvh_order[first + k];                                                   \
                    WorldHit w;                                                                                    \
                    analytic_hit(sc.prims[i], o, d, w);                                                            \
                    ++n_tests;                                                                                     \
                    if (w.has && (w.d2 < best.d2 || (w.d2 == best.d2 && best.id != HIT_MISS && i < best.prim))) {  \
                        best.d2 = w.d2;                                                                            \
                        best.id = i;                                                                               \
                        best.prim = i;                                                                             \
                        tlimit = limit_from_d2(best.d2, pad);                                                      \
                    }                                                                                              \
                }                                                                                                  \
            }                                                                                                      \
        }                                                                                                          \
    }
        if (sp + 4 > ABVH_STACK) {
            best.d2 = 3.402823466e+38f;
            best.id = HIT_MISS;
            best.prim = 0xFFFFFFFFu;
            scan_analytic<false, 1>(sc, o, d, best, n_tests);
            return;
        }
        ABVH_CHILD(x)
        ABVH_CHILD(y)
        ABVH_CHILD(z)
        ABVH_CHILD(w)
#undef ABVH_CHILD
        if (sp == 0) break;
        node = stk[(--sp) * sstride];
    }
}


template <bool ABVH, int BLOCK>
__device__ __forceinline__ bool classify_ray(const DevScene& sc, f3 o, f3 d, uint32_t& id0, float& d2_0) {
    Closest best;
    best.d2 = 3.402823466e+38f;
    best.id = HIT_MISS;
    best.prim = 0xFFFFFFFFu;
    uint32_t n_tests = 0;
    scan_analytic<ABVH, BLOCK>(sc, o, d, best, n_tests);
    id0 = best.id;
    d2_0 = best.d2;
    if (sc.n_nodes == 0u) return false;
// ... 1114 lines not shown
                    gx = I.root;
                    in_blas = true;
                } else {
                    sp = spr;
                    ld = normalize3(dw);
                    pad = pad_w;
                    lscale = 1.0f;
                    padw4 = 0.0f;
                    gx = 0u;
                    in_blas = false;
                }
                ix = __builtin_amdgcn_rcpf(__builtin_fabsf(ld.x) < PRT_DIR_MIN ? __builtin_copysignf(PRT_DIR_MIN, ld.x) : ld.x);
                iy = __builtin_amdgcn_rcpf(__builtin_fabsf(ld.y) < PRT_DIR_MIN ? __builtin_copysignf(PRT_DIR_MIN, ld.y) : ld.y);
                iz = __builtin_amdgcn_rcpf(__builtin_fabsf(ld.z) < PRT_DIR_MIN ? __builtin_copysignf(PRT_DIR_MIN, ld.z) : ld.z);
                const bool nx = ix < 0.0f, ny = iy < 0.0f, nz = iz < 0.0f;
                anx = (nx ? o.x - pad : o.x + pad) * ix; afx = (nx ? o.x + pad : o.x - pad) * ix;
                any = (ny ? o.y - pad : o.y + pad) * iy; afy = (ny ? o.y + pad : o.y - pad) * iy;
                anz = (nz ? o.z - pad : o.z + pad) * iz; afz = (nz ? o.z + pad : o.z - pad) * iz;
                octinv4 = (7u - ((nx ? 1u : 0u) | (ny ? 2u : 0u) | (nz ? 4u : 0u))) * 0x01010101u;
                tlimit = (limit_from_d2(best.d2, 0.0f) + padw4) * lscale + 4.0f * pad;
                gy = next ? (1u << (24u + (octinv4 & 7u))) : 0u;
                if (sp > STACK_L) {
                    overflow = true;
                    gy = 0u;
                    sp = 0;
                    ipm = 0u;
                    in_blas = false;
                }
                stall = false;
            }
        }
        if (PATH) {
            const unsigned long long shade_m = __ballot(need_shade);
            const uint32_t n_wait = n_idle + (uint32_t)__popcll(shade_m);
            const bool others_busy = __ballot(k != 0xFFFFFFFFu && !need_shade) != 0ull;
            if ((shade_m != 0ull || (!exhausted && n_idle != 0u)) && (n_wait >= tune.refill_min || !others_busy)) {
                bool fresh = false;
                if (!exhausted && n_idle != 0u) {
                    if (cur == cur_end) {
                        uint32_t c = blockIdx.x * 4u + wv;
                        if (!first_grab) {
                            if (n_grabs <= n_wv) c = n_grabs;
                            else if (lane == 0) c = atomicAdd(work, 1u) + n_wv;
                            c = (uint32_t)__shfl((int)c, 0, 64);
                        }
                        first_grab = false;
                        if (c >= n_grabs) {
                            exhausted = true;
                        } else {
                            const uint32_t cb = c - n_big + n_big * big;
                            const uint32_t g0 = c < n_big ? c * big * gran_per_chunk : cb < n_bulk ? cb * gran_per_chunk : n_bulk * gran_per_chunk + (cb - n_bulk);
                            const uint32_t g1 = c < n_big ? g0 + big * gran_per_chunk : cb < n_bulk ? g0 + gran_per_chunk : g0 + 1u;
                            cur = g0 << 6;
                            cur_end = (g1 << 6) < count ? (g1 << 6) : count;
                        }
                    }
                    if (!exhausted) {
                        const uint32_t qi = cur + (uint32_t)__popcll(idle_mask & ((1ull << lane) - 1ull));
                        fresh = idle && qi < cur_end;
                        if (fresh) k = qi;
                        cur = (cur + n_idle < cur_end) ? cur + n_idle : cur_end;
                    }
                }
                int r = 0;
                uint32_t id = HIT_MISS, id0 = HIT_MISS;
                float d2_0 = 3.402823466e+38f;
                if (fresh) {
                    const uint32_t smp = k / pa.tm.n_pix_local, pl = k - smp * pa.tm.n_pix_local;
                    uint32_t px, py;
                    if (!tile_pixel(pa.tm, pl, px, py)) {
                        pa.rad[k] = make_float4(0.f, 0.f, 0.f, __uint_as_float(0xFFFFFFFFu));
                    } else {
                        prng = path_seed(py * pa.tm.W + px, pa.first_sample + smp, pa.seed);
                        float fx = (float)px + 0.5f, fy = (float)py + 0.5f;
                        if (pa.sp.jitter) {
                            const float u1 = rnd01(prng);
                            const float u2 = rnd01(prng);
                            fx = (float)px + u1;
                            fy = (float)py + u2;
                        }
                        camera_ray(pa.cam, fx, fy, o, pd);
                        pthr = mk3(1.f, 1.f, 1.f);
                        pdepth = 0u;
                        r = classify_ray<false, 256>(sc, o, pd, id0, d2_0) ? 1 : 2;
                        id = id0;
                    }
                }
                if (need_shade) {
                    r = 2;
                    id = best.id;
                    need_shade = false;
                }
                while (r == 2) {
                    r = advance_path<1, false, false, 256>(sc, id, o, pd, pthr, prng, pdepth, pa.max_depth, pa.sp, &pa.rad[k], id0, d2_0);
                    id = id0;
                }
                if (r == 1) {
                    ld = normalize3(pd);
                    pad = sc.pad * (__builtin_fabsf(o.x) + __builtin_fabsf(o.y) + __builtin_fabsf(o.z) + sc.extent);
                    ix = __builtin_amdgcn_rcpf(__builtin_fabsf(ld.x) < PRT_DIR_MIN ? __builtin_copysignf(PRT_DIR_MIN, ld.x) : ld.x);
                    iy = __builtin_amdgcn_rcpf(__builtin_fabsf(ld.y) < PRT_DIR_MIN ? __builtin_copysignf(PRT_DIR_MIN, ld.y) : ld.y);
                    iz = __builtin_amdgcn_rcpf(__builtin_fabsf(ld.z) < PRT_DIR_MIN ? __builtin_copysignf(PRT_DIR_MIN, ld.z) : ld.z);
                    const bool nx = ix < 0.0f, ny = iy < 0.0f, nz = iz < 0.0f;
                    anx = (nx ? o.x - pad : o.x + pad) * ix; afx = (nx ? o.x + pad : o.x - pad) * ix;
                    any = (ny ? o.y - pad : o.y + pad) * iy; afy = (ny ? o.y + pad : o.y - pad) * iy;
                    anz = (nz ? o.z - pad : o.z + pad) * iz; afz = (nz ? o.z + pad : o.z - pad) * iz;
                    octinv4 = (7u - ((nx ? 1u : 0u) | (ny ? 2u : 0u) | (nz ? 4u : 0u))) * 0x01010101u;
                    best.id = id0;
                    best.prim = id0;
                    best.d2 = d2_0;
                    tlimit = limit_from_d2(best.d2, pad);
                    gx = 0u;
                    gy = 1u << (24u + (octinv4 & 7u));
                    sp = 0;
                } else if ((fresh || ((shade_m >> lane) & 1ull)) && r == 0) {
                    k = 0xFFFFFFFFu;
                }
            }
        }
        if (!PATH && !exhausted && (n_idle >= tune.refill_min || (INST && do_sw && n_idle != 0u))) {
            if (cur == cur_end) {
                uint32_t c = blockIdx.x * 4u + wv;
                if (!first_grab) {
                    if (n_grabs <= n_wv) c = n_grabs;
                    else if (static_small) c += my_grabs * n_wv;
                    else if (lane == 0) c = atomicAdd(work, 1u) + n_wv;
                    c = (uint32_t)__shfl((int)c, 0, 64);
                }
                first_grab = false;
                ++my_grabs;
                if (c >= n_grabs) {
                    exhausted = true;
                    if (STATS) t_exh = __builtin_amdgcn_s_memrealtime();
                } else {
                    const uint32_t cb = c - n_big + n_big * big;
                    const uint32_t g0 = c < n_big ? c * big * gran_per_chunk : cb < n_bulk ? cb * gran_per_chunk : n_bulk * gran_per_chunk + (cb - n_bulk);
                    const uint32_t g1 = c < n_big ? g0 + big * gran_per_chunk : cb < n_bulk ? g0 + gran_per_chunk : g0 + 1u;
                    cur = g0 << 6;
                    cur_end = (g1 << 6) < count ? (g1 << 6) : count;
                }
            }
            if (!exhausted) {
                const uint32_t qi_seq = cur + (uint32_t)__popcll(idle_mask & ((1ull << lane) - 1ull));
                if (idle && qi_seq < cur_end) {
                    const uint32_t qi = (!PRIM && tune.perm) ? tune.perm[qi_seq] : qi_seq;
                    uint32_t hid = PRIM ? HIT_MISS : ld_stream(&hit[qi]);
                    if (hid != HIT_DEAD && !(ANY && !SEEDED && hid != HIT_MISS)) {
                        float4 O, D;
                        float hd2_0 = 0.0f;
                        if (PRIM) {
                            f3 po, pd;
                            uint32_t pixel, sample, lp;
                            primary_ray(pr, ld_stream(&pr.pid[qi]), po, pd, pixel, sample, &lp);
                            const float4 E = pr.pix[pr.n_pix_local + lp];
                            hid = __float_as_uint(E.y);
                            hd2_0 = E.z;
#ifndef PRT_NO_OPAQUE_ORIGIN
                            asm volatile("" : "+v"(po.x), "+v"(po.y), "+v"(po.z));
#endif
                            O = make_float4(po.x, po.y, po.z, 0.f);
                            D = make_float4(pd.x, pd.y, pd.z, 0.f);
                        } else {
                            O = ld_stream(&ro[qi]);
                            D = ld_stream(&rd[qi]);
                        }
                        o = mk3(O.x, O.y, O.z);
                        ld = normalize3(mk3(D.x, D.y, D.z));
                        pad = sc.pad * (__builtin_fabsf(o.x) + __builtin_fabsf(o.y) + __builtin_fabsf(o.z) + sc.extent);
                        ix = __builtin_amdgcn_rcpf(__builtin_fabsf(ld.x) < PRT_DIR_MIN ? __builtin_copysignf(PRT_DIR_MIN, ld.x) : ld.x);
                        iy = __builtin_amdgcn_rcpf(__builtin_fabsf(ld.y) < PRT_DIR_MIN ? __builtin_copysignf(PRT_DIR_MIN, ld.y) : ld.y);
                        iz = __builtin_amdgcn_rcpf(__builtin_fabsf(ld.z) < PRT_DIR_MIN ? __builtin_copysignf(PRT_DIR_MIN, ld.z) : ld.z);
                        const bool nx = ix < 0.0f, ny = iy < 0.0f, nz = iz < 0.0f;
                        anx = (nx ? o.x - pad : o.x + pad) * ix; afx = (nx ? o.x + pad : o.x - pad) * ix;
                        any = (ny ? o.y - pad : o.y + pad) * iy; afy = (ny ? o.y + pad : o.y - pad) * iy;
                        anz = (nz ? o.z - pad : o.z + pad) * iz; afz = (nz ? o.z + pad : o.z - pad) * iz;
                        octinv4 = (7u - ((nx ? 1u : 0u) | (ny ? 2u : 0u) | (nz ? 4u : 0u))) * 0x01010101u;
                        best.id = hid;
                        best.prim = hid;
                        best.d2 = PRIM ? hd2_0 : ld_stream(&hd2[qi]);
                        tlimit = limit_from_d2(best.d2, pad);
                        if (LEAN) {
                            s_lray[0 * 256 + tid] = o.x; s_lray[1 * 256 + tid] = o.y; s_lray[2 * 256 + tid] = o.z;
                            s_lray[3 * 256 + tid] = ld.x; s_lray[4 * 256 + tid] = ld.y; s_lray[5 * 256 + tid] = ld.z;
                            s_key[tid] = ((unsigned long long)__float_as_uint(best.d2) << 32) | (hid == HIT_MISS ? 0u : hid);
                            s_slot[tid] = hid;
                        }
                        k = qi;
                        if (STATS) ray_steps = 0u;
                        gx = 0u;
                        gy = 1u << (24u + (octinv4 & 7u));
                        sp = 0;
                        if (INST) {
                            in_blas = false;
                            stall = false;
                            ipm = 0u;
                            lscale = 1.0f;
                            padw4 = 0.0f;
                            s_wray[0 * 256 + tid] = O.x; s_wray[1 * 256 + tid] = O.y; s_wray[2 * 256 + tid] = O.z;
                            s_wray[3 * 256 + tid] = D.x; s_wray[4 * 256 + tid] = D.y; s_wray[5 * 256 + tid] = D.z;
                        }
                    }
                }
                cur = (cur + n_idle < cur_end) ? cur + n_idle : cur_end;
            }
        }
        if (__ballot(k != 0xFFFFFFFFu) == 0ull) {
            if (exhausted) break;
            continue;
        }
        if (STATS) {
            const unsigned long long t = __builtin_amdgcn_s_memtime();
            cyc_refill += t - t_mark;
            t_mark = t;
        }
        bool walk = (k != 0xFFFFFFFFu) && ((gy > 0x00FFFFFFu) || sp > 0 || (INST && ipm != 0u)) && !(INST && stall);
        uint32_t q_groups = 0u;
        while (walk) {
            uint32_t tm = 0u, tb = 0u;
            {
                const int spr = sp > 0 ? sp - 1 : 0;
                const uint2 top = s_stack[spr * 256 + tid];
                const bool has = gy > 0x00FFFFFFu;
                bool level_switch = false;
                if (INST) {
                    const bool enter = !in_blas && ipm != 0u;
                    const bool leave = in_blas && !has && top.x == T8_SENTINEL;
                    if (enter || leave) {
                        stall = true;
                        walk = false;
                        level_switch = true;
                    }
                }
                if (!level_switch) {
                    const uint32_t cx = has ? gx : top.x;
                    uint32_t cy = has ? gy : top.y;
                    sp = has ? sp : spr;
                    const uint32_t bit = 31u - (uint32_t)__builtin_clz(cy);
                    cy &= ~(1u << bit);
                    s_stack[sp * 256 + tid] = make_uint2(cx, cy);
                    sp += (cy > 0x00FFFFFFu) ? 1 : 0;
                    const uint32_t slot = (bit - 24u) ^ (octinv4 & 7u);
                    const uint32_t idx = cx + (uint32_t)__popc(cy & ((1u << slot) - 1u));
                    const uint4* nb = sc.nodes8 + (size_t)sc.node_stride * idx;
                    const uint4 w0 = nb[0], w1 = nb[1], w2 = nb[2], w3 = nb[3], w4 = nb[4];
                    if (STATS) {
                        ++n_nodes;
                        ++ray_steps;
                        if (ray_steps > ray_steps_max) ray_steps_max = ray_steps;
                        if ((int)lane == __ffsll((long long)__ballot(true)) - 1) ++s_iters[wv];
                        if ((uint32_t)sp > max_sp) max_sp = (uint32_t)sp;
                    }
                    T8_BOXTEST()
                    gx = w1.x;
                    gy = (hitmask & 0xFF000000u) | (eim >> 24);
                    tm = hitmask & 0x00FFFFFFu;
                    tb = w1.y;
                    if (sp > stack_cap) {
                        overflow = true;
                        gy = 0u;
                        sp = 0;
                        tm = 0u;
                        if (INST) {
                            ipm = 0u;
                            in_blas = false;
                        }
                    } else if (INST && !in_blas) {
                        ipb = tb;
                        ipm = tm;
                        tm = 0u;
                    }
                    walk = (gy > 0x00FFFFFFu) || sp > 0 || (INST && ipm != 0u);
                }
            }
            const unsigned long long qm = __ballot(tm != 0u);
            if (tm != 0u) {
                const uint32_t own = (STEAL && k >= 0xFFFFFF00u) ? (k & 63u) : lane;
                const uint32_t pos = q_groups + (uint32_t)__builtin_amdgcn_mbcnt_hi((uint32_t)(qm >> 32), __builtin_amdgcn_mbcnt_lo((uint32_t)qm, 0u));
                ((uint2*)queue)[pos] = make_uint2(tb, (own << 24) | tm);
                s_qn[wv] = q_groups + (uint32_t)__popcll(qm);
                pending = true;
            }
            q_groups += (uint32_t)__popcll(qm);
            if ((uint32_t)__popcll(__ballot(walk)) <= tune.exit_max || q_groups >= tri_min) break;
        }
        if (STATS) {
            const unsigned long long t = __builtin_amdgcn_s_memtime();
            cyc_node += t - t_mark;
            t_mark = t;
        }
        {
            __builtin_amdgcn_fence(__ATOMIC_SEQ_CST, "wavefront");
            const uint32_t G = ((volatile uint32_t*)s_qn)[wv];
            if (G != 0u) {
                const unsigned long long key_best =
                    LEAN ? 0ull : ((unsigned long long)__float_as_uint(best.d2) << 32) | (best.id == HIT_MISS ? 0u : best.prim);
                if (!LEAN) s_key[tid] = key_best;
                if (lane == 0) s_qn[wv] = 0u;
                for (uint32_t g0 = 0u; g0 < G; g0 += 64u) {
                const uint32_t cap = (G - g0 > 64u) ? T8_QCAP / 2u : T8_QCAP;
                const unsigned long long ga = g0 + lane < G ? ((volatile unsigned long long*)queue)[g0 + lane] : 0ull;
                const uint32_t base_a = (uint32_t)ga, own_a = (uint32_t)(ga >> 56);
                uint32_t ma = (uint32_t)(ga >> 32) & 0x00FFFFFFu;
                __builtin_amdgcn_fence(__ATOMIC_SEQ_CST, "wavefront");
                while (__ballot(ma != 0u) != 0ull) {
                    const uint32_t ca = (uint32_t)__popc(ma);
                    const uint32_t ia = wave_scan_add(ca);
                    const bool fit_a = ia <= cap;
// ... 47 lines not shown
                                key = ((unsigned long long)__float_as_uint(d2) << 32) | prim;
                                if (ANY)
                                    cand = key < atomicMin(&s_key[wbase + owner], key);
                                else {
                                    cand = true;
                                    atomicMin(&s_key[wbase + owner], key);
                                }
                            }
                        }
                        if (STATS && lane == 0) ++s_iters[4 + wv];
                        __builtin_amdgcn_fence(__ATOMIC_SEQ_CST, "wavefront");
                        if (cand && ((volatile unsigned long long*)s_key)[wbase + owner] == key) s_slot[wbase + owner] = LEAN ? sc.n_prims + win : win;
                        __builtin_amdgcn_fence(__ATOMIC_SEQ_CST, "wavefront");
                    }
                }
                }
                const unsigned long long won =
                    ((volatile unsigned long long*)s_key)[(STEAL && k >= 0xFFFFFF00u && k != 0xFFFFFFFFu) ? wbase + (k & 63u) : tid];
                if (LEAN) {
                    tlimit = limit_from_d2(__uint_as_float((uint32_t)(won >> 32)), pad);
                    if (ANY && k != 0xFFFFFFFFu) {
                        const uint32_t sl = ((volatile uint32_t*)s_slot)[(STEAL && k >= 0xFFFFFF00u) ? wbase + (k & 63u) : tid];
                        if (sl != HIT_MISS && (!SEEDED || sl >= sc.n_prims)) {
                            gy = 0u;
                            sp = 0;
                        }
                    }
                } else if (won != key_best) {
                    best.d2 = __uint_as_float((uint32_t)(won >> 32));
                    best.prim = (uint32_t)won;
                    best.id = sc.n_prims + ((volatile uint32_t*)s_slot)[tid];
                    tlimit = INST ? (limit_from_d2(best.d2, 0.0f) + padw4) * lscale + 4.0f * pad : limit_from_d2(best.d2, pad);
                    if (ANY && k != 0xFFFFFFFFu) {
                        gy = 0u;
                        sp = 0;
                        if (INST) {
                            ipm = 0u;
                            in_blas = false;
                            stall = false;
                        }
                    }
                }
                pending = false;
            }
        }
        if (STATS) {
            const unsigned long long t = __builtin_amdgcn_s_memtime();
            cyc_tri += t - t_mark;
            t_mark = t;
        }
    }
    if (STATS) {
        if (lane == 0) {
            atomicAdd(&stats[6], cyc_refill);
            atomicAdd(&stats[7], cyc_node);
            atomicAdd(&stats[8], cyc_tri);
            unsigned long long* tl = stats + 16 + PRT_TIMELINE_WORDS * tune.probe_slot;
            const unsigned long long t_end = __builtin_amdgcn_s_memrealtime();
            if (t_exh == 0ull) t_exh = t_end;
            if (my_xcd == 0u) {
                atomicMin(&tl[0], t_start);
                atomicMax(&tl[1], t_end);
                atomicMin(&tl[2], t_exh);
                atomicMax(&tl[3], t_exh);
            }
            atomicAdd(&tl[4], t_end - t_exh);
            atomicAdd(&tl[5], t_end - t_start);
            atomicAdd(&tl[6], 1ull);
        }
        uint32_t w_nodes = n_nodes, w_tris = n_tris, w_steps = ray_steps_max, w_sp = max_sp;
        for (int off = 32; off > 0; off >>= 1) {
            w_nodes += (uint32_t)__shfl_xor((int)w_nodes, off, 64);
            w_tris += (uint32_t)__shfl_xor((int)w_tris, off, 64);
            const uint32_t a = (uint32_t)__shfl_xor((int)w_steps, off, 64), b = (uint32_t)__shfl_xor((int)w_sp, off, 64);
            w_steps = a > w_steps ? a : w_steps;
            w_sp = b > w_sp ? b : w_sp;
        }
        if (lane == 0) {
            atomicMax(&stats[16 + PRT_TIMELINE_WORDS * tune.probe_slot + 7], (unsigned long long)w_steps);
            atomicAdd(&stats[0], (unsigned long long)w_nodes);
            atomicAdd(&stats[1], (unsigned long long)w_tris);
            atomicMax(&stats[5], (unsigned long long)w_sp);
        }
        __syncthreads();
        if (threadIdx.x < 4) atomicAdd(&stats[3], 64ull * s_iters[threadIdx.x]);
        if (threadIdx.x < 4) atomicAdd(&stats[4], 64ull * s_iters[4 + threadIdx.x]);
    }
}

template <int STACK_L, int WAVES, bool STATS, bool INST, bool LEAN = false, bool PRIM = false, bool PATH = false>
__global__ void __launch_bounds__(256, WAVES) k_traverse8_persistent(DevScene sc, const float4* __restrict__ ro,
                                                                    const float4* __restrict__ rd,
                                                                    uint32_t* __restrict__ hit,
                                                                    const float* __restrict__ hd2,
                                                                    const uint32_t* __restrict__ count_ptr,
                                                                    uint32_t* __restrict__ work,
                                                                    uint32_t* __restrict__ ovf, PrtTravTuning tune,
                                                                    unsigned long long* __restrict__ stats, PrtPrimary pr,
                                                                    PrtPathArgs pa) {
    traverse8_body<STACK_L, WAVES, STATS, INST, LEAN, PRIM, PATH, false>(sc, ro, rd, hit, hd2, count_ptr, work, ovf, tune,
                                                                         stats, pr, pa);
}

template <int STACK_L, int WAVES, bool INST, bool LEAN = false>
__global__ void __launch_bounds__(256, WAVES) k_occluded8_persistent(DevScene sc, const float4* __restrict__ ro,
                                                                    const float4* __restrict__ rd,
                                                                    uint32_t* __restrict__ hit,
                                                                    const float* __restrict__ hd2,
                                                                    const uint32_t* __restrict__ count_ptr,
                                                                    uint32_t* __restrict__ work,
                                                                    uint32_t* __restrict__ ovf, PrtTravTuning tune) {
    traverse8_body<STACK_L, WAVES, false, INST, LEAN, false, false, true>(sc, ro, rd, hit, hd2, count_ptr, work, ovf, tune,
                                                                          nullptr, PrtPrimary{}, PrtPathArgs{});
}

template <int STACK_L, int WAVES, bool INST, bool LEAN = false>
__global__ void __launch_bounds__(256, WAVES) k_occluded8_seeded(DevScene sc, const float4* __restrict__ ro,
                                                                const float4* __restrict__ rd, uint32_t* __restrict__ hit,
                                                                const float* __restrict__ hd2,
                                                                const uint32_t* __restrict__ count_ptr,
                                                                uint32_t* __restrict__ work, uint32_t* __restrict__ ovf,
                                                                PrtTravTuning tune) {
    traverse8_body<STACK_L, WAVES, false, INST, LEAN, false, false, true, true>(sc, ro, rd, hit, hd2, count_ptr, work, ovf, tune,
                                                                                nullptr, PrtPrimary{}, PrtPathArgs{});
}

template <int FUSE, bool SAMPLING, bool INST, bool ABVH, bool PRIM, bool ENV, bool TEX = false>
PRT_DEV void shade_step(DevScene sc, const float4* __restrict__ ro, const float4* __restrict__ rd, const float4* __restrict__ rt,
                        const uint32_t* __restrict__ hit, float4* __restrict__ no, float4* __restrict__ nd, float4* __restrict__ nt,
                        uint32_t* __restrict__ nhit, float* __restrict__ nhd2, float4* __restrict__ rad, uint32_t* __restrict__ counts,
                        uint32_t* __restrict__ work, uint32_t iter, uint32_t max_depth_arg, uint32_t cap, PrtSampling sp_arg, PrtPrimary pr,
                        const DevEnv* env, const DevTex* tex = nullptr) {
    const bool last_route = (max_depth_arg & PRT_LAST_SEGMENT_FLAG) != 0u;
    const uint32_t max_depth = max_depth_arg & ~PRT_LAST_SEGMENT_FLAG;
    const PrtSampling sp = SAMPLING ? sp_arg : PrtSampling{0u, 0u, 0.0f};
    const uint32_t nA = CNT_A(counts, iter), nB = CNT_B(counts, iter);
    const uint32_t count = nA + nB;
    if (blockIdx.x * (uint32_t)SHADE_BLOCK >= count) return;
    const uint32_t k = blockIdx.x * (uint32_t)SHADE_BLOCK + threadIdx.x;
    if (k < 8u) work[32u * k] = 0u;
    if (k == 8u) work[512] = 0u;
    bool front = false, back = false;
    f3 o = mk3(0.f, 0.f, 0.f), d = mk3(0.f, 0.f, 1.f), thr = mk3(0.f, 0.f, 0.f);
    uint32_t id0 = HIT_MISS, rng = 0, depth = 0, pid = 0;
    float d2_0 = 3.402823466e+38f;
    float4 pre_a = make_float4(0.f, 0.f, 0.f, 0.f), pre_b = pre_a;
    if (k < count) {
        const uint32_t src = k < nA ? k : cap - 1u - (k - nA);
        uint32_t id = (PRIM && (k >= nA || pr.walk)) ? HIT_MISS : ld_stream(&hit[src]);
        if (PRIM) {
            pid = ld_stream(&pr.pid[src]);
            uint32_t pixel, sample, lp;
            primary_ray(pr, pid, o, d, pixel, sample, &lp);
            if (k >= nA) id = __float_as_uint(pr.pix[pr.n_pix_local + lp].y);
            else if (pr.walk) id = hit[__float_as_uint(pr.pix[pr.n_pix_local + lp].x)];
            rng = path_seed(pixel, pr.first_sample + sample, pr.seed);
            depth = 0u;
            thr = mk3(1.f, 1.f, 1.f);
            pre_a = pr.pix[2u * pr.n_pix_local + lp];
            pre_b = pr.pix[3u * pr.n_pix_local + lp];
        } else {
            const float4 O = ld_stream(&ro[src]);
            const float4 D = ld_stream(&rd[src]);
            const float4 T = ld_stream(&rt[src]);
            pid = __float_as_uint(O.w);
            rng = __float_as_uint(D.w);
            depth = __float_as_uint(T.w);
            thr = mk3(T.x, T.y, T.z);
            o = mk3(O.x, O.y, O.z);
            d = mk3(D.x, D.y, D.z);
        }
        if (id != HIT_DEAD) {
            const int r = advance_path<1 + FUSE, INST, ABVH, SHADE_BLOCK, PRIM, ENV, TEX, FUSE == 0>(sc, id, o, d, thr, rng, depth, max_depth, sp, &rad[pid], id0, d2_0, pre_a, pre_b, env, tex, last_route);
            front = r == 1;
            back = r == 2;
        }
    }
    const uint32_t slot = block_alloc2<SHADE_BLOCK>(front, back, false, &CNT_A(counts, iter + 1u), &CNT_B(counts, iter + 1u),
                                                    &CNT_C(counts, iter + 1u), cap);
    if (slot != 0xFFFFFFFFu) {
        st_stream(&no[slot], make_float4(o.x, o.y, o.z, __uint_as_float(pid)));
        st_stream(&nd[slot], make_float4(d.x, d.y, d.z, __uint_as_float(rng)));
        st_stream(&nt[slot], make_float4(thr.x, thr.y, thr.z, __uint_as_float(depth)));
        st_stream(&nhit[slot], id0);
        st_stream(&nhd2[slot], d2_0);
    }
}

template <int FUSE, bool SAMPLING, bool INST, bool ABVH, bool PRIM = false>
__global__ void __launch_bounds__(SHADE_BLOCK) k_shade(DevScene sc, const float4* __restrict__ ro,
                                                      const float4* __restrict__ rd, const float4* __restrict__ rt,
                                                      const uint32_t* __restrict__ hit, float4* __restrict__ no,
                                                      float4* __restrict__ nd, float4* __restrict__ nt,
                                                      uint32_t* __restrict__ nhit, float* __restrict__ nhd2,
                                                      float4* __restrict__ rad, uint32_t* __restrict__ counts,
                                                      uint32_t* __restrict__ work, uint32_t iter, uint32_t max_depth,
                                                      uint32_t cap, PrtSampling sp_arg, PrtPrimary pr) {
    shade_step<FUSE, SAMPLING, INST, ABVH, PRIM, false>(sc, ro, rd, rt, hit, no, nd, nt, nhit, nhd2, rad, counts, work, iter, max_depth,
                                                        cap, sp_arg, pr, nullptr);
}

template <bool INST, bool ABVH>
__global__ void __launch_bounds__(SHADE_BLOCK) k_shade_env(DevScene sc, DevEnv env, const float4* __restrict__ ro,
                                                          const float4* __restrict__ rd, const float4* __restrict__ rt,
                                                          const uint32_t* __restrict__ hit, float4* __restrict__ no,
                                                          float4* __restrict__ nd, float4* __restrict__ nt,
                                                          uint32_t* __restrict__ nhit, float* __restrict__ nhd2,
                                                          float4* __restrict__ rad, uint32_t* __restrict__ counts,
                                                          uint32_t* __restrict__ work, uint32_t iter, uint32_t max_depth,
                                                          uint32_t cap, PrtSampling sp_arg) {
    shade_step<0, true, INST, ABVH, false, true>(sc, ro, rd, rt, hit, no, nd, nt, nhit, nhd2, rad, counts, work, iter, max_depth, cap,
                                                 sp_arg, PrtPrimary{}, &env);
}

template <bool INST, bool ABVH, bool ENV>
__global__ void __launch_bounds__(SHADE_BLOCK) k_shade_tex(DevScene sc, DevTex tex, DevEnv env, const float4* __restrict__ ro,
                                                          const float4* __restrict__ rd, const float4* __restrict__ rt,
                                                          const uint32_t* __restrict__ hit, float4* __restrict__ no,
                                                          float4* __restrict__ nd, float4* __restrict__ nt,
                                                          uint32_t* __restrict__ nhit, float* __restrict__ nhd2,
                                                          float4* __restrict__ rad, uint32_t* __restrict__ counts,
                                                          uint32_t* __restrict__ work, uint32_t iter, uint32_t max_depth,
                                                          uint32_t cap, PrtSampling sp_arg) {
    shade_step<0, true, INST, ABVH, false, ENV, true>(sc, ro, rd, rt, hit, no, nd, nt, nhit, nhd2, rad, counts, work, iter, max_depth, cap,
                                                      sp_arg, PrtPrimary{}, ENV ? &env : nullptr, &tex);
}

__global__ void __launch_bounds__(256) k_primary_hit(DevScene sc, PrtPrimary pr, const uint32_t* __restrict__ hit,
                                                     float4* __restrict__ pix, const uint32_t* __restrict__ counts) {
    const uint32_t pl = blockIdx.x * 256u + threadIdx.x;
    if (pl >= pr.n_pix_local) return;
    const float4 E = pix[pr.n_pix_local + pl];
    float4 a = make_float4(0.f, 0.f, 0.f, __uint_as_float(HIT_DEAD)), b = make_float4(0.f, 0.f, 0.f, 0.f);
    if (__float_as_uint(E.w) == 0xFFFFFFFEu) {
        const uint32_t first = __float_as_uint(E.x);
        const bool walked = pr.walk ? first != 0xFFFFFFFFu : first < CNT_A(counts, 0);
        const uint32_t id = walked ? hit[first] : __float_as_uint(E.y);
        if (id != HIT_MISS && id != HIT_DEAD) {
            const float4 P = pix[pl];
            WorldHit w;
            world_hit_from_id<false>(sc, id, mk3(pr.origin[0], pr.origin[1], pr.origin[2]), mk3(P.x, P.y, P.z), w);
            if (w.has) {
                a = make_float4(w.pos.x, w.pos.y, w.pos.z, __uint_as_float(id));
                b = make_float4(w.normal.x, w.normal.y, w.normal.z, __uint_as_float(w.material | (w.front ? 0x80000000u : 0u)));
            }
        }
    }
    pix[2u * pr.n_pix_local + pl] = a;
    pix[3u * pr.n_pix_local + pl] = b;
}

__global__ void __launch_bounds__(SHADE_BLOCK) k_shade_divstats(DevScene sc, const uint32_t* __restrict__ hit,
                                                                 const uint32_t* __restrict__ counts, uint32_t iter, uint32_t cap,
                                                                 unsigned long long* __restrict__ out, PrtPrimary pr, int compact) {
    const uint32_t nA = CNT_A(counts, iter), nB = CNT_B(counts, iter);
    const uint32_t count = nA + nB;
    if (blockIdx.x * (uint32_t)SHADE_BLOCK >= count) return;
    const uint32_t k = blockIdx.x * (uint32_t)SHADE_BLOCK + threadIdx.x;
    uint32_t type = 5u;
    if (k < count) {
        const uint32_t src = k < nA ? k : cap - 1u - (k - nA);
        uint32_t id;
        if (compact && (k >= nA || pr.walk)) {
            f3 o_, d_;
            uint32_t pixel, sample, lp;
            primary_ray(pr, pr.pid[src], o_, d_, pixel, sample, &lp);
            const float4 E = pr.pix[pr.n_pix_local + lp];
            id = k >= nA ? __float_as_uint(E.y) : hit[__float_as_uint(E.x)];
        } else {
            id = hit[src];
        }
        type = 0u;
        if (id != HIT_MISS && id != HIT_DEAD) {
            uint32_t m;
            if (id < sc.n_prims) {
                m = sc.prims[id].material;
            } else if (sc.n_insts) {
                const uint32_t v = id - sc.n_prims;
                uint32_t lo = 0, hi = sc.n_insts;
                while (hi - lo > 1u) {
                    const uint32_t mid = (lo + hi) >> 1;
                    if (sc.insts[mid].virt_base <= v) lo = mid; else hi = mid;
                }
                const DevInstance& I = sc.insts[lo];
                m = I.material == 0xFFFFFFFFu ? __float_as_uint(sc.tris[3 * (size_t)(I.slot_base + (v - I.virt_base)) + 1].w) : I.material;
            } else {
                m = __float_as_uint(sc.tris[3 * (size_t)(id - sc.n_prims) + 1].w);
            }
            type = sc.mat_type[m] <= 4u ? sc.mat_type[m] : 0u;
        }
    }
    unsigned long long* o = out + 16u * iter;
    const uint32_t lane = lane_id();
    uint32_t distinct = 0u;
    for (uint32_t t = 0; t < 5u; ++t) {
        const unsigned long long mk = __ballot(type == t);
        if (mk != 0ull && lane == 0u) {
            atomicAdd(&o[2 + t], (unsigned long long)__popcll(mk));
            atomicAdd(&o[8 + t], 1ull);
        }
        if (t >= 1u && t <= 3u && mk != 0ull) ++distinct;
    }
    const unsigned long long any = __ballot(type != 5u);
    if (lane == 0u && any != 0ull) {
        atomicAdd(&o[0], 1ull);
        atomicAdd(&o[1], (unsigned long long)__popcll(any));
        if (distinct) {
            atomicAdd(&o[14], (unsigned long long)distinct);
            atomicAdd(&o[15], 1ull);
        }
    }
}

__global__ void __launch_bounds__(256) k_accumulate(const float4* __restrict__ rad, float4* __restrict__ film_local,
                                                    PrtTileMap tm, uint32_t S, uint32_t max_depth, int update_film,
                                                    unsigned long long* __restrict__ ray_stats,
                                                    const float4* __restrict__ pix_end) {
    __shared__ uint32_t s_ends[PRT_MAX_DEPTH];
    if (threadIdx.x < PRT_MAX_DEPTH) s_ends[threadIdx.x] = 0u;
    __syncthreads();
    for (uint32_t pl0 = blockIdx.x * 256u; pl0 < tm.n_pix_local; pl0 += gridDim.x * 256u) {
    const uint32_t pl = pl0 + threadIdx.x;
    uint32_t x, y;
    const bool valid = pl < tm.n_pix_local && tile_pixel(tm, pl, x, y);
    float4 f = valid ? film_local[pl] : make_float4(0.f, 0.f, 0.f, 0.f);
    float4 E = make_float4(0.f, 0.f, 0.f, __uint_as_float(0xFFFFFFFEu));
    if (valid && pix_end) E = pix_end[pl];
    const bool ended = __float_as_uint(E.w) != 0xFFFFFFFEu;
    const float weight = 1.0f;
    const uint32_t lane = lane_id();
    for (uint32_t s0 = 0; s0 < S; s0 += 8u) {
        float4 r[8];
#pragma unroll
        for (uint32_t j = 0; j < 8u; ++j)
            r[j] = (valid && !ended && s0 + j < S) ? ld_stream(&rad[(size_t)(s0 + j) * tm.n_pix_local + pl]) : E;
#pragma unroll
        for (uint32_t j = 0; j < 8u; ++j) {
            if (s0 + j >= S) break;
            uint32_t e = 0xFFFFFFFFu;
            if (valid) {
                f.x += r[j].x * weight;
                f.y += r[j].y * weight;
                f.z += r[j].z * weight;
                f.w += weight;
                e = __float_as_uint(r[j].w);
            }
            for (uint32_t dd = 0; dd < max_depth; ++dd) {
                const unsigned long long mk = __ballot(e == dd);
                if (mk != 0ull && lane == 0) atomicAdd(&s_ends[dd], (uint32_t)__popcll(mk));
            }
        }
    }
    if (valid && update_film) film_local[pl] = f;
    }
    __syncthreads();
    if (threadIdx.x < max_depth) {
        unsigned long long n = 0;
        for (uint32_t e = threadIdx.x; e < max_depth; ++e) n += s_ends[e];
        if (n) atomicAdd(&ray_stats[(blockIdx.x & (PRT_RAY_STAT_SLOTS - 1u)) * PRT_MAX_DEPTH + threadIdx.x], n);
    }
}

__global__ void __launch_bounds__(256) k_accumulate_lit(const float4* __restrict__ rad, const float4* __restrict__ lrad,
                                                        float4* __restrict__ film_local, PrtTileMap tm, uint32_t S,
                                                        uint32_t max_depth, int update_film,
                                                        unsigned long long* __restrict__ ray_stats) {
    __shared__ uint32_t s_ends[PRT_MAX_DEPTH];
    if (threadIdx.x < PRT_MAX_DEPTH) s_ends[threadIdx.x] = 0u;
    __syncthreads();
    for (uint32_t pl0 = blockIdx.x * 256u; pl0 < tm.n_pix_local; pl0 += gridDim.x * 256u) {
    const uint32_t pl = pl0 + threadIdx.x;
    uint32_t x, y;
    const bool valid = pl < tm.n_pix_local && tile_pixel(tm, pl, x, y);
    float4 f = valid ? film_local[pl] : make_float4(0.f, 0.f, 0.f, 0.f);
    const float4 E = make_float4(0.f, 0.f, 0.f, __uint_as_float(0xFFFFFFFFu));
    const float weight = 1.0f;
    const uint32_t lane = lane_id();
    for (uint32_t s0 = 0; s0 < S; s0 += 8u) {
        float4 r[8];
#pragma unroll
        for (uint32_t j = 0; j < 8u; ++j)
            r[j] = (valid && s0 + j < S) ? ld_stream(&rad[(size_t)(s0 + j) * tm.n_pix_local + pl]) : E;
#pragma unroll
        for (uint32_t j = 0; j < 8u; ++j) {
            if (valid && s0 + j < S) {
                const float4 l = ld_stream(&lrad[(size_t)(s0 + j) * tm.n_pix_local + pl]);
                r[j].x = r[j].x + l.x;
                r[j].y = r[j].y + l.y;
                r[j].z = r[j].z + l.z;
            }
        }
#pragma unroll
        for (uint32_t j = 0; j < 8u; ++j) {
            if (s0 + j >= S) break;
            uint32_t e = 0xFFFFFFFFu;
            if (valid) {
                f.x += r[j].x * weight;
                f.y += r[j].y * weight;
                f.z += r[j].z * weight;
                f.w += weight;
                e = __float_as_uint(r[j].w);
            }
            for (uint32_t dd = 0; dd < max_depth; ++dd) {
                const unsigned long long mk = __ballot(e == dd);
                if (mk != 0ull && lane == 0) atomicAdd(&s_ends[dd], (uint32_t)__popcll(mk));
            }
        }
    }
    if (valid && update_film) film_local[pl] = f;
    }
    __syncthreads();
    if (threadIdx.x < max_depth) {
        unsigned long long n = 0;
        for (uint32_t e = threadIdx.x; e < max_depth; ++e) n += s_ends[e];
        if (n) atomicAdd(&ray_stats[(blockIdx.x & (PRT_RAY_STAT_SLOTS - 1u)) * PRT_MAX_DEPTH + threadIdx.x], n);
    }
}

template <bool LIT, bool LIST>
__global__ void __launch_bounds__(256) k_accumulate_stat(const float4* __restrict__ rad, const float4* __restrict__ lrad,
                                                         float4* __restrict__ film_local, float2* __restrict__ stat, PrtTileMap tm,
                                                         uint32_t S, uint32_t max_depth, int update_film,
                                                         unsigned long long* __restrict__ ray_stats,
                                                         const float4* __restrict__ pix_end, const uint32_t* __restrict__ list) {
    __shared__ uint32_t s_ends[PRT_MAX_DEPTH];
    if (threadIdx.x < PRT_MAX_DEPTH) s_ends[threadIdx.x] = 0u;
    __syncthreads();
    for (uint32_t pl0 = blockIdx.x * 256u; pl0 < tm.n_pix_local; pl0 += gridDim.x * 256u) {
    const uint32_t pl = pl0 + threadIdx.x;
    const bool in_range = pl < tm.n_pix_local;
    uint32_t fl = pl;
    if (LIST && in_range) fl = (list[pl >> 6] << 6) | (pl & 63u);
    uint32_t x, y;
    const bool valid = in_range && tile_pixel(tm, fl, x, y);
    float4 f = valid ? film_local[fl] : make_float4(0.f, 0.f, 0.f, 0.f);
    float2 m2 = valid ? stat[fl] : make_float2(0.f, 0.f);
    float4 E = make_float4(0.f, 0.f, 0.f, __uint_as_float((LIT || LIST) ? 0xFFFFFFFFu : 0xFFFFFFFEu));
    if (!LIT && !LIST && valid && pix_end) E = pix_end[pl];
    const bool ended = !LIT && !LIST && __float_as_uint(E.w) != 0xFFFFFFFEu;
    const float weight = 1.0f;
    const uint32_t lane = lane_id();
    for (uint32_t s0 = 0; s0 < S; s0 += 8u) {
        float4 r[8];
#pragma unroll
        for (uint32_t j = 0; j < 8u; ++j)
            r[j] = (valid && !ended && s0 + j < S) ? ld_stream(&rad[(size_t)(s0 + j) * tm.n_pix_local + pl]) : E;
        if (LIT) {
#pragma unroll
            for (uint32_t j = 0; j < 8u; ++j) {
                if (valid && s0 + j < S) {
                    const float4 l = ld_stream(&lrad[(size_t)(s0 + j) * tm.n_pix_local + pl]);
                    r[j].x = r[j].x + l.x;
                    r[j].y = r[j].y + l.y;
                    r[j].z = r[j].z + l.z;
                }
            }
        }
#pragma unroll
        for (uint32_t j = 0; j < 8u; ++j) {
            if (s0 + j >= S) break;
            uint32_t e = 0xFFFFFFFFu;
            if (valid) {
                f.x += r[j].x * weight;
                f.y += r[j].y * weight;
                f.z += r[j].z * weight;
                f.w += weight;
                const float lum = __fadd_rn(__fadd_rn(__fmul_rn(0.2126f, r[j].x), __fmul_rn(0.7152f, r[j].y)), __fmul_rn(0.0722f, r[j].z));
                m2.x = __fadd_rn(m2.x, lum);
                m2.y = __fadd_rn(m2.y, __fmul_rn(lum, lum));
                e = __float_as_uint(r[j].w);
            }
            for (uint32_t dd = 0; dd < max_depth; ++dd) {
                const unsigned long long mk = __ballot(e == dd);
                if (mk != 0ull && lane == 0) atomicAdd(&s_ends[dd], (uint32_t)__popcll(mk));
            }
        }
    }
    if (valid && update_film) {
        film_local[fl] = f;
        stat[fl] = m2;
    }
    }
    __syncthreads();
    if (threadIdx.x < max_depth) {
        unsigned long long n = 0;
        for (uint32_t e = threadIdx.x; e < max_depth; ++e) n += s_ends[e];
        if (n) atomicAdd(&ray_stats[(blockIdx.x & (PRT_RAY_STAT_SLOTS - 1u)) * PRT_MAX_DEPTH + threadIdx.x], n);
    }
}

__global__ void __launch_bounds__(256) k_tile_select(const float4* __restrict__ film_local, const float2* __restrict__ stat,
                                                     PrtTileMap tm, const uint32_t* __restrict__ prev, uint32_t n_in, float threshold,
                                                     float noise_floor, uint32_t* __restrict__ flags) {
    const uint32_t w = blockIdx.x * 4u + (threadIdx.x >> 6);
    if (w >= n_in) return;
    const uint32_t t = prev ? prev[w] : w;
    const uint32_t pl = (t << 6) | lane_id();
    uint32_t x, y;
    bool unconverged = false;
    const bool inside = tile_pixel(tm, pl, x, y);
    if (inside) {
        const float2 m2 = stat[pl];
        unconverged = prt_adaptive_rule(film_local[pl].w, m2.x, m2.y, threshold, noise_floor);
    }
    const unsigned long long mk = __ballot(unconverged), in_image = __ballot(inside);
    if (lane_id() == 0u) flags[w] = mk != 0ull ? (uint32_t)__popcll(in_image) : 0u;
}

__global__ void __launch_bounds__(1024) k_tile_compact(const uint32_t* __restrict__ flags, const uint32_t* __restrict__ prev,
                                                       uint32_t n_in, uint32_t* __restrict__ out, uint32_t* __restrict__ count) {
    __shared__ uint32_t s_wave[16];
    __shared__ uint32_t s_pixels;
    if (threadIdx.x == 0u) s_pixels = 0u;
    const uint32_t lane = lane_id(), wave = threadIdx.x >> 6;
    uint32_t run = 0u, pixels = 0u;
    for (uint32_t i0 = 0; i0 < n_in; i0 += 1024u) {
        const uint32_t i = i0 + threadIdx.x;
        const uint32_t flag = i < n_in ? flags[i] : 0u;
        const bool on = flag != 0u;
        pixels += flag;
        const unsigned long long mk = __ballot(on);
        if (lane == 0u) s_wave[wave] = (uint32_t)__popcll(mk);
        __syncthreads();
        uint32_t before = 0u, total = 0u;
        for (uint32_t k = 0; k < 16u; ++k) {
            const uint32_t nk = s_wave[k];
            if (k < wave) before += nk;
            total += nk;
        }
        if (on) out[run + before + (uint32_t)__popcll(mk & ((1ull << lane) - 1ull))] = prev ? prev[i] : i;
        run += total;
        __syncthreads();
    }
    __syncthreads();
    if (pixels) atomicAdd(&s_pixels, pixels);
    __syncthreads();
    if (threadIdx.x == 0u) {
        count[0] = run;
        count[1] = s_pixels;
    }
}


__global__ void __launch_bounds__(256) k_resolve(const float4* __restrict__ gathered, uint32_t world, uint32_t stride,
                                                 uint32_t W, uint32_t H, float* __restrict__ rgb,
                                                 float* __restrict__ weight) {
    const uint32_t idx = blockIdx.x * 256u + threadIdx.x;
    if (idx >= W * H) return;
    const uint32_t x = idx % W, y = idx / W;
    const uint32_t tiles_x = (W + 7u) >> 3;
    const uint32_t gt = (y >> 3) * tiles_x + (x >> 3);
    const uint32_t rank = gt % world, lt = gt / world;
    const uint32_t pl = lt * 64u + (y & 7u) * 8u + (x & 7u);
    const float4 f = gathered[(size_t)rank * stride + pl];
    rgb[3 * (size_t)idx + 0] = f.x;
    rgb[3 * (size_t)idx + 1] = f.y;
    rgb[3 * (size_t)idx + 2] = f.z;
    weight[idx] = f.w;
}

__global__ void __launch_bounds__(256) k_tonemap(const float* __restrict__ rgb, const float* __restrict__ weight,
                                                 uint32_t n_pix, float exposure, float inv_gamma,
                                                 uint8_t* __restrict__ out) {
    const uint32_t idx = blockIdx.x * 256u + threadIdx.x;
    if (idx >= n_pix * 4u) return;
    const uint32_t p = idx >> 2, c = idx & 3u;
    if (c == 3u) {
        out[idx] = 255;
        return;
    }
    const float w = weight[p];
    float value = 0.0f;
    if (w > 0.0f) {
        const float invW = 1.0f / w;
        value = rgb[3 * (size_t)p + c] * invW;
        value = value * exposure;
        value = value / (1.0f + value);
        value = powf(value, inv_gamma);
    }
    value = __builtin_fmaxf(0.0f, __builtin_fminf(1.0f, value));
    out[idx] = (uint8_t)(value * 255.0f + 0.5f);
}

__global__ void k_camera_rays_lens(DevCamera cam, DevLens lens, uint32_t n, const float* __restrict__ px, const float* __restrict__ py,
                                   uint32_t* __restrict__ keys, float* __restrict__ o_out, float* __restrict__ d_out) {
    const uint32_t i = blockIdx.x * blockDim.x + threadIdx.x;
    if (i >= n) return;
    f3 o, d;
    uint32_t rng = keys[i];
    lens_camera_ray(cam, lens, px[i], py[i], rng, o, d);
    keys[i] = rng;
    o_out[3 * (size_t)i + 0] = o.x;
    o_out[3 * (size_t)i + 1] = o.y;
    o_out[3 * (size_t)i + 2] = o.z;
    d_out[3 * (size_t)i + 0] = d.x;
    d_out[3 * (size_t)i + 1] = d.y;
    d_out[3 * (size_t)i + 2] = d.z;
}
__global__ void k_camera_rays(DevCamera cam, uint32_t n, const float* __restrict__ px, const float* __restrict__ py,
                              float* __restrict__ o_out, float* __restrict__ d_out) {
    const uint32_t i = blockIdx.x * 256u + threadIdx.x;
    if (i >= n) return;
    f3 o, d;
    camera_ray(cam, px[i], py[i], o, d);
    o_out[3 * i + 0] = o.x;
    o_out[3 * i + 1] = o.y;
    o_out[3 * i + 2] = o.z;
    d_out[3 * i + 0] = d.x;
    d_out[3 * i + 1] = d.y;
    d_out[3 * i + 2] = d.z;
}

__global__ void k_pack_rays(uint32_t n, const float* __restrict__ o, const float* __restrict__ d,
                            float4* __restrict__ ro, float4* __restrict__ rd, uint32_t* __restrict__ counts) {
    const uint32_t i = blockIdx.x * 256u + threadIdx.x;
    if (i == 0) counts[0] = n;
    if (i >= n) return;
    ro[i] = make_float4(o[3 * i], o[3 * i + 1], o[3 * i + 2], __uint_as_float(i));
    rd[i] = make_float4(d[3 * i], d[3 * i + 1], d[3 * i + 2], 0.f);
}

__global__ void k_hit_records(DevScene sc, uint32_t n, const float4* __restrict__ ro, const float4* __restrict__ rd,
                              const uint32_t* __restrict__ hit, PrtHit* __restrict__ out) {
    const uint32_t i = blockIdx.x * 256u + threadIdx.x;
    if (i >= n) return;
    PrtHit h;
    h.prim = -1;
    h.front_face = 0;
    h.material_id = 0xFFFFFFFFu;
    h.d2 = 3.402823466e+38f;
    h.position[0] = h.position[1] = h.position[2] = 0.f;
    h.normal[0] = h.normal[1] = h.normal[2] = 0.f;
    const uint32_t id = hit[i];
// ... 436 lines not shown
    if (blockIdx.x * 256u >= count) return;
    if (threadIdx.x < 2u) s_n[threadIdx.x] = 0u;
    __syncthreads();
    bool occ = false;
    if (k < count) {
        const uint32_t id = lb.sh.hit[k];
        const float4 O = lb.sh.o[k];
        const float4 T = lb.sh.t[k];
        if (id != HIT_MISS && id != HIT_DEAD) {
            const float4 D = lb.sh.d[k];
            WorldHit w;
            if (sc.n_insts)
                world_hit_from_id<true>(sc, id, mk3(O.x, O.y, O.z), mk3(D.x, D.y, D.z), w);
            else
                world_hit_from_id<false>(sc, id, mk3(O.x, O.y, O.z), mk3(D.x, D.y, D.z), w);
            occ = w.has && w.d2 < T.w * T.w;
        }
        if (!occ) {
            float4* p = &lb.lrad[__float_as_uint(O.w)];
            float4 a = *p;
            a.x = a.x + T.x;
            a.y = a.y + T.y;
            a.z = a.z + T.z;
            *p = a;
        }
    }
    const unsigned long long mn = __ballot(k < count), mo = __ballot(occ);
    if (lane_id() == 0u) {
        atomicAdd(&s_n[0], (uint32_t)__popcll(mn));
        atomicAdd(&s_n[1], (uint32_t)__popcll(mo));
    }
    __syncthreads();
    if (threadIdx.x < 2u && s_n[threadIdx.x])
        atomicAdd(&lb.stats[2u * (blockIdx.x & (PRT_RAY_STAT_SLOTS - 1u)) + threadIdx.x], (unsigned long long)s_n[threadIdx.x]);
}

template <bool MESHL, bool ENV = false, bool CLUS = false>
PRT_DEV void sample_light_test(DevScene sc, DevLights lt, const DevMeshLights* ml, uint32_t n, const float* __restrict__ in_d,
                               const PrtHit* __restrict__ hits, const uint32_t* __restrict__ keys, float* __restrict__ out,
                               uint32_t* __restrict__ out_light, const DevEnv* env = nullptr, const DevLightClusters* lc = nullptr) {
    const uint32_t i = blockIdx.x * 256u + threadIdx.x;
    if (i >= n) return;
    const PrtHit h = hits[i];
    float r[11] = {0.f, 0.f, 0.f, 0.f, 0.f, 0.f, 0.f, 0.f, 0.f, 0.f, 0.f};
    uint32_t light = 0xFFFFFFFFu;
    if (ENV && h.prim >= 0 && sc.mat_type[h.material_id] == 1u && (env->t_all | env->t_env) != 0u && env_selected(*env, keys[i])) {
        const float4 a = sc.mat_rgbs[h.material_id];
        LightSample s;
        float pb = 0.0f, wl = 0.0f, wb = 1.0f;
        f3 C;
        if (env_sample_term(*env, lt.mode, mk3(h.normal[0], h.normal[1], h.normal[2]), mk3(a.x, a.y, a.z), mk3(1.f, 1.f, 1.f), keys[i], 0.0f,
                            s, pb, wl, C)) {
            light = s.light;
            (void)env_miss(*env, lt.mode, s.w, pb, wb);
            const float vals[11] = {s.w.x, s.w.y, s.w.z, s.tmax, C.x, C.y, C.z, s.pdf_l, pb, wl, wb};
            for (int j = 0; j < 11; ++j) r[j] = vals[j];
        }
    } else if (h.prim >= 0 && sc.mat_type[h.material_id] == 1u && lt.n_lights) {
        const float4 a = sc.mat_rgbs[h.material_id];
        const f3 x = mk3(h.position[0], h.position[1], h.position[2]);
        LightSample s;
        float pb = 0.0f, wl = 0.0f;
        f3 C;
        if (light_sample_term<MESHL, CLUS>(lt, x, mk3(h.normal[0], h.normal[1], h.normal[2]), mk3(a.x, a.y, a.z), mk3(1.f, 1.f, 1.f), keys[i],
                                           0.0f, s, pb, wl, C, ml, lc)) {
            light = s.light;
            const uint32_t prim = __float_as_uint(lt.lights[PRT_LIGHT_F4 * s.light + 4u].w);
            const float vals[11] = {s.w.x, s.w.y, s.w.z, s.tmax, C.x, C.y, C.z, s.pdf_l, pb, wl,
                                    bsdf_hit_weight<MESHL, CLUS>(lt, prim, x, s.w, s.t_light * s.t_light, pb, ml, sc.n_prims, lc)};
            for (int j = 0; j < 11; ++j) r[j] = vals[j];
        }
    }
    for (int j = 0; j < 11; ++j) out[11 * (size_t)i + j] = r[j];
    out_light[i] = light;
}

__global__ void k_sample_light_test(DevScene sc, DevLights lt, uint32_t n, const float* __restrict__ in_d,
                                    const PrtHit* __restrict__ hits, const uint32_t* __restrict__ keys, float* __restrict__ out,
                                    uint32_t* __restrict__ out_light) {
    sample_light_test<false>(sc, lt, nullptr, n, in_d, hits, keys, out, out_light);
}

__global__ void k_sample_light_test_mesh(DevScene sc, DevLights lt, DevMeshLights ml, uint32_t n, const float* __restrict__ in_d,
                                         const PrtHit* __restrict__ hits, const uint32_t* __restrict__ keys, float* __restrict__ out,
                                         uint32_t* __restrict__ out_light) {
    sample_light_test<true>(sc, lt, &ml, n, in_d, hits, keys, out, out_light);
}

__global__ void k_sample_light_test_env(DevScene sc, DevLights lt, DevEnv env, uint32_t n, const float* __restrict__ in_d,
                                        const PrtHit* __restrict__ hits, const uint32_t* __restrict__ keys, float* __restrict__ out,
                                        uint32_t* __restrict__ out_light) {
    sample_light_test<false, true>(sc, lt, nullptr, n, in_d, hits, keys, out, out_light, &env);
}

__global__ void k_sample_light_test_mesh_env(DevScene sc, DevLights lt, DevMeshLights ml, DevEnv env, uint32_t n,
                                             const float* __restrict__ in_d, const PrtHit* __restrict__ hits,
                                             const uint32_t* __restrict__ keys, float* __restrict__ out, uint32_t* __restrict__ out_light) {
    sample_light_test<true, true>(sc, lt, &ml, n, in_d, hits, keys, out, out_light, &env);
}

__global__ void k_sample_light_test_clus(DevScene sc, DevLights lt, DevMeshLights ml, DevLightClusters lc, uint32_t n,
                                         const float* __restrict__ in_d, const PrtHit* __restrict__ hits,
                                         const uint32_t* __restrict__ keys, float* __restrict__ out, uint32_t* __restrict__ out_light) {
    sample_light_test<true, false, true>(sc, lt, &ml, n, in_d, hits, keys, out, out_light, nullptr, &lc);
}

__global__ void k_sample_light_test_clus_env(DevScene sc, DevLights lt, DevMeshLights ml, DevLightClusters lc, DevEnv env, uint32_t n,
                                             const float* __restrict__ in_d, const PrtHit* __restrict__ hits,
                                             const uint32_t* __restrict__ keys, float* __restrict__ out, uint32_t* __restrict__ out_light) {
    sample_light_test<true, true, true>(sc, lt, &ml, n, in_d, hits, keys, out, out_light, &env, &lc);
}

__global__ void k_light_cluster_pmf(DevLightClusters lc, uint32_t n, const float* __restrict__ x, uint32_t* __restrict__ M) {
    const uint32_t i = blockIdx.x * 256u + threadIdx.x;
    if (i >= n) return;
    uint32_t* row = M + (size_t)i * lc.n_clusters;
    cluster_thresholds(lc, mk3(x[3 * (size_t)i], x[3 * (size_t)i + 1], x[3 * (size_t)i + 2]),
                       [&](uint32_t c, uint32_t, uint32_t mc) { row[c] = mc; });
}

__global__ void k_environment_eval(DevEnv env, uint32_t n, const float* __restrict__ dirs, float* __restrict__ rgb,
                                   uint32_t* __restrict__ texel, float* __restrict__ pdf_w) {
    const uint32_t i = blockIdx.x * 256u + threadIdx.x;
    if (i >= n) return;
    const f3 d = mk3(dirs[3 * (size_t)i], dirs[3 * (size_t)i + 1], dirs[3 * (size_t)i + 2]);
    float pw;
    const f3 le = env_radiance(env, d, pw);
    if (rgb) {
        rgb[3 * (size_t)i + 0] = le.x;
        rgb[3 * (size_t)i + 1] = le.y;
        rgb[3 * (size_t)i + 2] = le.z;
    }
    if (texel) texel[i] = env_texel(env, d);
    if (pdf_w) pdf_w[i] = pw;
}

static inline uint32_t blocks_for(uint64_t n) { return (uint32_t)((n + 255u) / 256u); }

template <class T>
static const T& or_empty(const T* p) {
    static const T none{};
    return p ? *p : none;
}

bool prt_launch_raygen(hipStream_t st, PrtRaygenInst inst, const PrtRaygenArgs& a) {
    const uint32_t S = a.tm.n_pix_local ? a.n_paths / a.tm.n_pix_local : 0u;
    const uint32_t group = (a.sp.jitter || a.lens) ? (uint32_t)RAYGEN_GROUP : RAYGEN_GROUP_NOJITTER;
    const dim3 grid((a.tm.n_pix_local + PRODUCER_BLOCK - 1) / PRODUCER_BLOCK, (S + group - 1) / group);
    const DevScene& sc = *a.sc;
    const DevEnv& e = or_empty(a.env);
    const DevLens& l = or_empty(a.lens);
#define PRT_RAYGEN_HEAD a.cam, a.tm, S, a.first_sample, a.seed, a.out.o, a.out.d, a.out.t, a.out.hit
#define PRT_RAYGEN_TAIL a.rad, a.counts, a.work, a.max_depth, a.sp
#define PRT_RAYGEN_ARGS_PLAIN sc, PRT_RAYGEN_HEAD, a.out.hd2, PRT_RAYGEN_TAIL, nullptr
#define PRT_RAYGEN_ARGS_COMPACT sc, PRT_RAYGEN_HEAD, a.primary_walk ? a.out.hd2 : nullptr, PRT_RAYGEN_TAIL, a.compact_pix
#define PRT_RAYGEN_ARGS_ENV sc, e, PRT_RAYGEN_HEAD, a.out.hd2, PRT_RAYGEN_TAIL
#define PRT_RAYGEN_ARGS_LENS sc, l, PRT_RAYGEN_HEAD, a.out.hd2, PRT_RAYGEN_TAIL
#define PRT_RAYGEN_ARGS_LENS_ENV sc, e, l, PRT_RAYGEN_HEAD, a.out.hd2, PRT_RAYGEN_TAIL
#define PRT_RAYGEN_ARGS_LIST sc, e, l, a.cam, a.tm, a.list, S, a.first_sample, a.seed, a.out.o, a.out.d, a.out.t, a.out.hit, a.out.hd2, PRT_RAYGEN_TAIL
#define PRT_RAYGEN_CASE(sig, kernel, tag, ...) \
    case PRT_INST(kernel, tag): hipLaunchKernelGGL((kernel<__VA_ARGS__>), grid, dim3(PRODUCER_BLOCK), 0, st, PRT_RAYGEN_ARGS_##sig); return true;
    switch (inst) {
        PRT_RAYGEN_INSTANCES(PRT_RAYGEN_CASE)
        default: return false;
    }
#undef PRT_RAYGEN_CASE
#undef PRT_RAYGEN_ARGS_LIST
#undef PRT_RAYGEN_ARGS_LENS_ENV
#undef PRT_RAYGEN_ARGS_LENS
#undef PRT_RAYGEN_ARGS_ENV
#undef PRT_RAYGEN_ARGS_COMPACT
#undef PRT_RAYGEN_ARGS_PLAIN
#undef PRT_RAYGEN_TAIL
#undef PRT_RAYGEN_HEAD
}

void prt_launch_scan_prims(hipStream_t st, const DevScene& sc, const PrtRayBuf& in, const uint32_t* count_ptr,
                           uint32_t* work, uint32_t max_rays, unsigned long long* stats) {
    hipLaunchKernelGGL(k_scan_prims, dim3(blocks_for(max_rays)), dim3(256), 0, st, sc, in.o, in.d, in.hit, in.hd2,
                       count_ptr, work, stats);
}

__global__ void k_reset_cursors(uint32_t* work) {
    if (threadIdx.x < 8u) work[32u * threadIdx.x] = 0u;
}

static PrtTravTuning walk_tuning(const PrtTravTuning& in, const PrtWalkLaunch& l) {
    PrtTravTuning t = in;
    t.exit_max = l.exit_max, t.tri_min = l.tri_min, t.stack_cap = l.stack_cap, t.steal = l.steal;
    if (!l.keep_perm) t.perm = nullptr;
    return t;
}

template <int L, int W, bool IN, bool LN>
static void launch_walk8(hipStream_t st, const PrtWalkLaunch& l, const PrtWalkArgs& a, const PrtTravTuning& tune) {
    const dim3 grid(l.grid), block(256);
    const PrtRayBuf& in = a.rays;
    unsigned long long* stats = l.stats ? a.stats : nullptr;
#define PRT_WALK8_ARGS *a.sc, in.o, in.d, in.hit, in.hd2, a.count, a.work, a.work + 512, tune
    if (l.form == PRT_WALK_SEEDED) hipLaunchKernelGGL((k_occluded8_seeded<L, W, IN, LN>), grid, block, 0, st, PRT_WALK8_ARGS);
    else if (l.form == PRT_WALK_ANY) hipLaunchKernelGGL((k_occluded8_persistent<L, W, IN, LN>), grid, block, 0, st, PRT_WALK8_ARGS);
    else if (LN && l.prim) {
        if constexpr (LN) {
            if (stats) hipLaunchKernelGGL((k_traverse8_persistent<L, W, true, IN, LN, true>), grid, block, 0, st, PRT_WALK8_ARGS, stats, *a.primary, PrtPathArgs{});
            else hipLaunchKernelGGL((k_traverse8_persistent<L, W, false, IN, LN, true>), grid, block, 0, st, PRT_WALK8_ARGS, stats, *a.primary, PrtPathArgs{});
        }
    } else if (stats) hipLaunchKernelGGL((k_traverse8_persistent<L, W, true, IN, LN>), grid, block, 0, st, PRT_WALK8_ARGS, stats, PrtPrimary{}, PrtPathArgs{});
    else hipLaunchKernelGGL((k_traverse8_persistent<L, W, false, IN, LN>), grid, block, 0, st, PRT_WALK8_ARGS, stats, PrtPrimary{}, PrtPathArgs{});
#undef PRT_WALK8_ARGS
}

static void launch_walk_row(hipStream_t st, const PrtWalkLaunch& l, const PrtWalkArgs& a) {
    const PrtTravTuning tune = walk_tuning(*a.tune, l);
    const dim3 grid(l.grid), block(256);
    const PrtRayBuf& in = a.rays;
    uint32_t* ovf = a.work + 512;
    const uint32_t* count = l.overflow ? ovf : a.count;
    const uint32_t* list = l.overflow ? ovf + 1 : nullptr;
    unsigned long long* stats = l.stats ? a.stats : nullptr;
    if (l.reset) hipLaunchKernelGGL(k_reset_cursors, dim3(1), dim3(64), 0, st, a.work);
#define PRT_WALK_T_ARGS *a.sc, in.o, in.d, in.hit, in.hd2, count, a.work, a.spill, list, ovf, tune, stats
#define PRT_WALK_T(KERNEL, L, W, MODE)                                                                          \
    {                                                                                                           \
        if (stats) hipLaunchKernelGGL((KERNEL<L, W, MODE, true>), grid, block, 0, st, PRT_WALK_T_ARGS);         \
        else hipLaunchKernelGGL((KERNEL<L, W, MODE, false>), grid, block, 0, st, PRT_WALK_T_ARGS);              \
        break;                                                                                                  \
    }
#define PRT_WALK8_CASE(name, L, W, IN, LN) case PRT_W8_##name: launch_walk8<L, W, IN, LN>(st, l, a, tune); break;
#define PRT_WALK4_CASE(tag, L, W, MODE) case PRT_W4_##tag: PRT_WALK_T(k_traverse4_persistent, L, W, MODE)
#define PRT_WALK2_CASE(tag, L, W, MODE) case PRT_W2_##tag: PRT_WALK_T(k_traverse_persistent, L, W, MODE)
#define PRT_INTERSECT_CASE(tag, S, V)                                                                                         \
    case PRT_WI_##tag:                                                                                                        \
        if (stats) hipLaunchKernelGGL((k_intersect<S, true, V>), grid, block, 0, st, *a.sc, in.o, in.d, in.hit, a.count, stats);  \
        else hipLaunchKernelGGL((k_intersect<S, false, V>), grid, block, 0, st, *a.sc, in.o, in.d, in.hit, a.count, stats);       \
        break;
    switch (l.row) {
        PRT_WALK8_ROWS(PRT_WALK8_CASE)
        PRT_WALK4_ROWS(PRT_WALK4_CASE)
        PRT_WALK2_ROWS(PRT_WALK2_CASE)
        PRT_INTERSECT_ROWS(PRT_INTERSECT_CASE)
        case PRT_WALK_ROWS: break;
    }
#undef PRT_INTERSECT_CASE
#undef PRT_WALK2_CASE
#undef PRT_WALK4_CASE
#undef PRT_WALK8_CASE
#undef PRT_WALK_T
#undef PRT_WALK_T_ARGS
}

void prt_launch_walk(hipStream_t st, const PrtWalkPlan& plan, const PrtWalkArgs& a) {
#ifdef PRT_PROBE_REBOUND
    if (plan.launch[0].stats && a.stats && prt_walk_row(plan.launch[0].row).family != 0u) {
        PrtWalkPlan plain = plan;
        plain.launch[0].stats = plain.launch[1].stats = false;
        prt_launch_walk(st, plain, a);
        hipLaunchKernelGGL(k_reset_cursors, dim3(1), dim3(64), 0, st, a.work);
    }
#endif
    for (uint32_t i = 0; i < plan.n; ++i) launch_walk_row(st, plan.launch[i], a);
}

void prt_launch_path(hipStream_t st, const PrtWalkPlan& plan, const DevScene& sc, const PrtPathArgs& pa, uint32_t* work, const PrtTravTuning& tune_in) {
    const PrtTravTuning tune = walk_tuning(tune_in, plan.launch[0]);
    hipLaunchKernelGGL((k_traverse8_persistent<15, 4, false, false, false, false, true>), dim3(plan.launch[0].grid), dim3(256), 0, st, sc,
                       (const float4*)nullptr, (const float4*)nullptr, (uint32_t*)nullptr, (const float*)nullptr, (const uint32_t*)nullptr, work,
                       work + 512, tune, (unsigned long long*)nullptr, PrtPrimary{}, pa);
}

int prt_walk_occupancy(const PrtWalkPlan& plan, int* blocks_per_cu, int* vgprs, int* sgprs, int* lds_bytes) {
    const void* fn = (const void*)k_traverse4_persistent<32, 4, 3, false>;
#define PRT_WALK8_CASE(name, L, W, IN, LN) if (plan.occupancy == PRT_W8_##name) fn = (const void*)k_traverse8_persistent<L, W, false, IN, LN>;
    PRT_WALK8_ROWS(PRT_WALK8_CASE)
#undef PRT_WALK8_CASE
    hipFuncAttributes at;
    hipError_t e = hipFuncGetAttributes(&at, fn);
    if (e != hipSuccess) return (int)e;
    int nb = 0;
    e = hipOccupancyMaxActiveBlocksPerMultiprocessor(&nb, fn, 256, 0);
    if (e != hipSuccess) return (int)e;
    *blocks_per_cu = nb;
    *vgprs = at.numRegs;
    *sgprs = 0;
    *lds_bytes = (int)at.sharedSizeBytes;
    return 0;
}

bool prt_launch_shade(hipStream_t st, PrtShadeInst inst, const PrtShadeArgs& a) {
    const uint32_t n_for_grid = a.n_rays_known == 0xFFFFFFFFu ? a.cap : (a.n_rays_known ? a.n_rays_known : 1u);
    const dim3 grid((uint32_t)((n_for_grid + SHADE_BLOCK - 1) / SHADE_BLOCK));
    const DevScene& sc = *a.sc;
    const PrtPrimary& pr = or_empty(a.primary);
    const DevEnv& e = or_empty(a.env);
    const DevTex& tex = or_empty(a.tex);
    const DevLights& lt = or_empty(a.lights);
    const DevMeshLights& m = or_empty(a.mesh_lights);
    const DevLightClusters& lc = or_empty(a.clusters);
    const PrtLightBufs& lb = or_empty(a.lb);
#define PRT_SHADE_RAYS a.in.o, a.in.d, a.in.t, a.in.hit, a.out.o, a.out.d, a.out.t, a.out.hit, a.out.hd2
#define PRT_SHADE_TAIL_D(D) a.rad, a.counts, a.work, a.depth, D, a.cap, a.sp
#define PRT_SHADE_TAIL PRT_SHADE_TAIL_D(a.max_depth)
#define PRT_SHADE_TAIL_LS PRT_SHADE_TAIL_D((a.last_segment ? a.max_depth | PRT_LAST_SEGMENT_FLAG : a.max_depth))
#define PRT_SHADE_ARGS_PLAIN sc, PRT_SHADE_RAYS, PRT_SHADE_TAIL_LS, pr
#define PRT_SHADE_ARGS_ENV sc, e, PRT_SHADE_RAYS, PRT_SHADE_TAIL_LS
#define PRT_SHADE_ARGS_TEX sc, tex, e, PRT_SHADE_RAYS, PRT_SHADE_TAIL_LS
#define PRT_SHADE_ARGS_NEE sc, lt, PRT_SHADE_RAYS, lb, PRT_SHADE_TAIL
#define PRT_SHADE_ARGS_NEE_ENV sc, lt, e, PRT_SHADE_RAYS, lb, PRT_SHADE_TAIL
#define PRT_SHADE_ARGS_NEE_MESH sc, lt, m, PRT_SHADE_RAYS, lb, PRT_SHADE_TAIL
#define PRT_SHADE_ARGS_NEE_MESH_ENV sc, lt, m, e, PRT_SHADE_RAYS, lb, PRT_SHADE_TAIL
#define PRT_SHADE_ARGS_NEE_TEX sc, tex, lt, m, e, PRT_SHADE_RAYS, lb, PRT_SHADE_TAIL
#define PRT_SHADE_ARGS_NEE_CLUS sc, lt, m, lc, PRT_SHADE_RAYS, lb, PRT_SHADE_TAIL
#define PRT_SHADE_ARGS_NEE_CLUS_ENV sc, lt, m, lc, e, PRT_SHADE_RAYS, lb, PRT_SHADE_TAIL
#define PRT_SHADE_ARGS_NEE_CLUS_TEX sc, tex, lt, m, lc, e, PRT_SHADE_RAYS, lb, PRT_SHADE_TAIL
#define PRT_SHADE_CASE(sig, kernel, tag, ...) \
    case PRT_INST(kernel, tag): hipLaunchKernelGGL((kernel<__VA_ARGS__>), grid, dim3(SHADE_BLOCK), 0, st, PRT_SHADE_ARGS_##sig); return true;
    switch (inst) {
        PRT_SHADE_INSTANCES(PRT_SHADE_CASE)
        default: return false;
    }
#undef PRT_SHADE_CASE
#undef PRT_SHADE_ARGS_NEE_CLUS_TEX
#undef PRT_SHADE_ARGS_NEE_CLUS_ENV
#undef PRT_SHADE_ARGS_NEE_CLUS
#undef PRT_SHADE_ARGS_NEE_TEX
#undef PRT_SHADE_ARGS_NEE_MESH_ENV
#undef PRT_SHADE_ARGS_NEE_MESH
#undef PRT_SHADE_ARGS_NEE_ENV
#undef PRT_SHADE_ARGS_NEE
#undef PRT_SHADE_ARGS_TEX
#undef PRT_SHADE_ARGS_ENV
#undef PRT_SHADE_ARGS_PLAIN
#undef PRT_SHADE_TAIL_LS
#undef PRT_SHADE_TAIL
#undef PRT_SHADE_TAIL_D
#undef PRT_SHADE_RAYS
}

void prt_launch_shade_divstats(hipStream_t st, const DevScene& sc, const PrtRayBuf& in, const uint32_t* counts, uint32_t iter,
                               uint32_t cap, unsigned long long* out, const PrtPrimary* primary) {
    hipLaunchKernelGGL(k_shade_divstats, dim3((cap + SHADE_BLOCK - 1u) / SHADE_BLOCK), dim3(SHADE_BLOCK), 0, st, sc, in.hit, counts, iter, cap, out,
                       primary ? *primary : PrtPrimary{}, primary ? 1 : 0);
}

void prt_launch_primary_hit(hipStream_t st, const DevScene& sc, const PrtPrimary& pr, const uint32_t* hit, float4* pix,
                            const uint32_t* counts) {
    hipLaunchKernelGGL(k_primary_hit, dim3(blocks_for(pr.n_pix_local)), dim3(256), 0, st, sc, pr, hit, pix, counts);
}

bool prt_launch_accumulate(hipStream_t st, PrtAccumulateInst inst, const PrtAccumulateArgs& a) {
    const uint32_t nb = blocks_for(a.tm.n_pix_local ? a.tm.n_pix_local : 1);
    const dim3 grid(nb < 8192u ? nb : 8192u);
    const int upd = a.update_film ? 1 : 0;
#define PRT_ACC_ARGS_PLAIN a.rad, a.film_local, a.tm, a.S, a.max_depth, upd, a.ray_stats, a.pix_end
#define PRT_ACC_ARGS_LIT a.rad, a.lrad, a.film_local, a.tm, a.S, a.max_depth, upd, a.ray_stats
#define PRT_ACC_ARGS_STAT a.rad, a.lrad, a.film_local, a.stat, a.tm, a.S, a.max_depth, upd, a.ray_stats, a.pix_end, a.list
#define PRT_ACC_CASE_N(sig, kernel) \
    case PRT_I_##kernel: hipLaunchKernelGGL(kernel, grid, dim3(256), 0, st, PRT_ACC_ARGS_##sig); return true;
#define PRT_ACC_CASE_T(sig, kernel, tag, ...) \
    case PRT_INST(kernel, tag): hipLaunchKernelGGL((kernel<__VA_ARGS__>), grid, dim3(256), 0, st, PRT_ACC_ARGS_##sig); return true;
    switch (inst) {
        PRT_ACCUMULATE_INSTANCES(PRT_ACC_CASE_N, PRT_ACC_CASE_T)
        default: return false;
    }
#undef PRT_ACC_CASE_T
#undef PRT_ACC_CASE_N
#undef PRT_ACC_ARGS_STAT
#undef PRT_ACC_ARGS_LIT
#undef PRT_ACC_ARGS_PLAIN
}

void prt_launch_resolve(hipStream_t st, const float4* gathered, uint32_t world, uint32_t stride, uint32_t W,
                        uint32_t H, float* rgb, float* weight) {
    hipLaunchKernelGGL(k_resolve, dim3(blocks_for((uint64_t)W * H)), dim3(256), 0, st, gathered, world, stride, W, H,
                       rgb, weight);
}

void prt_launch_tonemap(hipStream_t st, const float* rgb, const float* weight, uint32_t n_pix, float exposure,
                        float inv_gamma, uint8_t* out) {
    hipLaunchKernelGGL(k_tonemap, dim3(blocks_for((uint64_t)n_pix * 4u)), dim3(256), 0, st, rgb, weight, n_pix,
                       exposure, inv_gamma, out);
}

void prt_launch_camera_rays_lens(hipStream_t st, const DevCamera& cam, const DevLens& lens, uint32_t n, const float* px,
                                 const float* py, uint32_t* keys, float* o, float* d) {
    hipLaunchKernelGGL(k_camera_rays_lens, dim3(blocks_for(n)), dim3(256), 0, st, cam, lens, n, px, py, keys, o, d);
}
void prt_launch_camera_rays(hipStream_t st, const DevCamera& cam, uint32_t n, const float* px, const float* py,
                            float* o, float* d) {
    hipLaunchKernelGGL(k_camera_rays, dim3(blocks_for(n)), dim3(256), 0, st, cam, n, px, py, o, d);
}

void prt_launch_pack_rays(hipStream_t st, uint32_t n, const float* o, const float* d, const PrtRayBuf& out,
                          uint32_t* counts) {
    hipLaunchKernelGGL(k_pack_rays, dim3(blocks_for(n)), dim3(256), 0, st, n, o, d, out.o, out.d, counts);
}

void prt_launch_hit_records(hipStream_t st, const DevScene& sc, uint32_t n, const PrtRayBuf& in, PrtHit* out) {
    hipLaunchKernelGGL(k_hit_records, dim3(blocks_for(n)), dim3(256), 0, st, sc, n, in.o, in.d, in.hit, out);
}

void prt_launch_pack_occlusion_rays(hipStream_t st, uint32_t n, const float* o, const float* d, const float* tmax,
                                    const PrtRayBuf& out, uint32_t* counts) {
    hipLaunchKernelGGL(k_pack_occlusion_rays, dim3(blocks_for(n)), dim3(256), 0, st, n, o, d, tmax, out.o, out.d, out.hit,
                       out.hd2, counts);
}

void prt_launch_scan_prims_bounded(hipStream_t st, const DevScene& sc, const PrtRayBuf& in, const uint32_t* count_ptr,
                                   uint32_t* work, uint32_t max_rays) {
    hipLaunchKernelGGL(k_scan_prims_bounded, dim3(blocks_for(max_rays)), dim3(256), 0, st, sc, in.o, in.d, in.hit, in.hd2,
                       count_ptr, work);
}

void prt_launch_occlusion_bytes(hipStream_t st, const DevScene& sc, uint32_t n, const PrtRayBuf& in, const float* tmax,
                                uint8_t* out) {
    hipLaunchKernelGGL(k_occlusion_bytes, dim3(blocks_for(n)), dim3(256), 0, st, sc, n, in.o, in.d, in.hit, tmax, out);
}

void prt_launch_scatter_test(hipStream_t st, const DevScene& sc, uint32_t n, const float* in_d, const PrtHit* hits,
                             uint32_t* rng_io, uint32_t* scattered, float* atten, float* emitted, float* o_out,
                             float* d_out) {
    hipLaunchKernelGGL(k_scatter_test, dim3(blocks_for(n)), dim3(256), 0, st, sc, n, in_d, hits, rng_io, scattered,
                       atten, emitted, o_out, d_out);
}

void prt_launch_light_accum(hipStream_t st, const DevScene& sc, const PrtLightBufs& lb, const uint32_t* count_ptr,
                            uint32_t* work, uint32_t max_rays) {
    hipLaunchKernelGGL(k_light_accum, dim3(blocks_for(max_rays ? max_rays : 1u)), dim3(256), 0, st, sc, lb, count_ptr, work);
}

void prt_launch_sample_light_test(hipStream_t st, const DevScene& sc, const DevLights& lt, uint32_t n, const float* in_d,
                                  const PrtHit* hits, const uint32_t* keys, float* out_f, uint32_t* out_light, const DevMeshLights* ml,
                                  const DevEnv* env, const DevLightClusters* lc) {
    if (lc && ml) {
        if (env)
            hipLaunchKernelGGL(k_sample_light_test_clus_env, dim3(blocks_for(n)), dim3(256), 0, st, sc, lt, *ml, *lc, *env, n, in_d, hits, keys, out_f, out_light);
        else
            hipLaunchKernelGGL(k_sample_light_test_clus, dim3(blocks_for(n)), dim3(256), 0, st, sc, lt, *ml, *lc, n, in_d, hits, keys, out_f, out_light);
        return;
    }
    if (env) {
        if (ml)
            hipLaunchKernelGGL(k_sample_light_test_mesh_env, dim3(blocks_for(n)), dim3(256), 0, st, sc, lt, *ml, *env, n, in_d, hits, keys, out_f, out_light);
        else
            hipLaunchKernelGGL(k_sample_light_test_env, dim3(blocks_for(n)), dim3(256), 0, st, sc, lt, *env, n, in_d, hits, keys, out_f, out_light);
        return;
    }
    if (ml) {
        hipLaunchKernelGGL(k_sample_light_test_mesh, dim3(blocks_for(n)), dim3(256), 0, st, sc, lt, *ml, n, in_d, hits, keys, out_f, out_light);
        return;
    }
    hipLaunchKernelGGL(k_sample_light_test, dim3(blocks_for(n)), dim3(256), 0, st, sc, lt, n, in_d, hits, keys, out_f, out_light);
}

void prt_launch_light_cluster_pmf(hipStream_t st, const DevLightClusters& lc, uint32_t n, const float* x, uint32_t* M) {
    hipLaunchKernelGGL(k_light_cluster_pmf, dim3(blocks_for(n)), dim3(256), 0, st, lc, n, x, M);
}

void prt_launch_environment_eval(hipStream_t st, const DevEnv& env, uint32_t n, const float* dirs, float* rgb, uint32_t* texel,
                                 float* pdf_w) {
    hipLaunchKernelGGL(k_environment_eval, dim3(blocks_for(n)), dim3(256), 0, st, env, n, dirs, rgb, texel, pdf_w);
}

void prt_launch_texture_eval(hipStream_t st, const DevTex& tex, uint32_t n, const uint32_t* texture, const float* uv, float* rgb) {
    hipLaunchKernelGGL(k_texture_eval, dim3(blocks_for(n)), dim3(256), 0, st, tex, n, texture, uv, rgb);
}

void prt_launch_hit_uv(hipStream_t st, const DevScene& sc, const DevTex& tex, uint32_t n, const PrtRayBuf& in, float* uv, float* albedo) {
    hipLaunchKernelGGL(k_hit_uv, dim3(blocks_for(n)), dim3(256), 0, st, sc, tex, n, in.o, in.d, in.hit, uv, albedo);
}


void prt_launch_tile_select(hipStream_t st, const float4* film_local, const float2* stat, const PrtTileMap& tm, const uint32_t* prev,
                            uint32_t n_in, float threshold, float noise_floor, uint32_t* flags, uint32_t* out, uint32_t* count) {
    if (n_in) hipLaunchKernelGGL(k_tile_select, dim3((n_in + 3u) / 4u), dim3(256), 0, st, film_local, stat, tm, prev, n_in, threshold,
                                 noise_floor, flags);
    hipLaunchKernelGGL(k_tile_compact, dim3(1), dim3(1024), 0, st, flags, prev, n_in, out, count);
}
```

parallelraytracing_amd/csrc/prt_primary_cache.h:

```cpp
#pragma once
#include <cstdint>

#include "prt_route.h"

struct PrtPrimaryKey {
    bool valid;
    uint64_t camera_gen;
    uint64_t scene_gen;
    uint32_t W, H, rank, world, n_pix_local;
    uint32_t S_cur, max_depth;
    PrtRoutePlan plan;
    uint32_t walk_row;
    bool walk_prim;
    bool compact, walk, primary_hit, lens, jitter;
    uint32_t rr_depth;
    float clamp;
    bool listed;
    bool instrumented;
    bool exact;
};

inline bool prt_route_plan_equal(const PrtRoutePlan& a, const PrtRoutePlan& b) {
    return a.path == b.path && a.compact == b.compact && a.walk == b.walk && a.primary_hit == b.primary_hit && a.walk8 == b.walk8 &&
           a.fuse == b.fuse && a.raygen == b.raygen && a.shade0 == b.shade0 && a.shade == b.shade && a.accumulate == b.accumulate &&
           a.last_segment == b.last_segment;
}

inline bool prt_primary_reusable(const PrtPrimaryKey& held, const PrtPrimaryKey& now) {
    if (!held.valid || !now.valid) return false;
    if (now.jitter || now.lens || now.listed || now.instrumented || !now.compact) return false;
    return held.camera_gen == now.camera_gen && held.scene_gen == now.scene_gen && held.W == now.W && held.H == now.H &&
           held.rank == now.rank && held.world == now.world && held.n_pix_local == now.n_pix_local && held.S_cur == now.S_cur &&
           held.max_depth == now.max_depth && prt_route_plan_equal(held.plan, now.plan) && held.walk_row == now.walk_row &&
           held.walk_prim == now.walk_prim && held.compact == now.compact && held.walk == now.walk && held.primary_hit == now.primary_hit &&
           held.lens == now.lens && held.jitter == now.jitter && held.rr_depth == now.rr_depth && held.clamp == now.clamp &&
           held.listed == now.listed && held.instrumented == now.instrumented && held.exact == now.exact;
}
```

Measured before the change: 24390 Mrays/s.

## Switch path IDs to pixel-major order with a transposing accumulate kernel

Path IDs in compact mode are now encoded as pixel*S+sample instead of sample*n_pix+pixel whenever S is at least 8. Decoding uses a magic-number division, and a new pixel-major accumulate kernel stages radiance through LDS to transpose it. The aim is to keep a pixel's samples contiguous for better locality in the ray buffers and the accumulate reads, and to make ID decode cheaper. The trade-off is that ray coherence across neighbouring threads changes: adjacent IDs now come from the same pixel rather than neighbouring pixels, which may affect traversal divergence.

```diff
diff --git a/parallelraytracing_amd/csrc/prt_api.cpp b/parallelraytracing_amd/csrc/prt_api.cpp
--- a/parallelraytracing_amd/csrc/prt_api.cpp
+++ b/parallelraytracing_amd/csrc/prt_api.cpp
@@ -188,6 +188,7 @@
     float pad_coeff = kPadCoeff;
     int node_stride = 0;
     int compact_primary = 1;
+    int path_id_order = 1;
     int primary_walk = 1;
     const char* shade_instance = "";
     const char* batch_instance[4] = {"", "", "", ""};
@@ -207,7 +208,7 @@
     PrimaryMem prim;
     uint64_t prim_pid_entries = 0;
     uint32_t prim_pix_entries = 0;
-    PrtPrimaryKey primary_key{};
+    PrtPrimaryStageKey primary_key{};
     uint64_t camera_gen = 1, scene_gen = 1;
     uint32_t primary_counts[2] = {0u, 0u};
     int primary_reuse = 1;
@@ -378,14 +379,14 @@
 
 int ensure_primary_state(PrtContext* c, uint64_t n_paths, uint32_t n_pix_local) {
     if (n_paths > c->prim_pid_entries) {
-        c->primary_key.valid = false;
+        c->primary_key.batch.valid = false;
         c->prim_pid_entries = 0;
         const uint64_t n = std::max<uint64_t>(n_paths, 256);
         HIPCHECK(c, c->prim.pid.ensure(n * sizeof(uint32_t)));
         c->prim_pid_entries = n;
     }
     if (n_pix_local > c->prim_pix_entries) {
-        c->primary_key.valid = false;
+        c->primary_key.batch.valid = false;
         c->prim_pix_entries = 0;
         const uint32_t n = std::max<uint32_t>(n_pix_local, 256u);
         HIPCHECK(c, c->prim.list.ensure((size_t)n * sizeof(uint32_t)));
@@ -745,6 +746,7 @@
     f.last_segment = c->last_segment;
     const PrtRoutePlan plan = prt_plan_route(f);
     const bool lit = f.lit, compact = plan.compact, walk = plan.walk;
+    const bool pixel_major_ids = prt_path_id_pixel_major(compact, S_cur, c->path_id_order);
     const DevEnv denv = dev_env(c);
     const DevTex dtex = dev_tex(c);
     const DevLens dlens{c->lens.aperture, c->lens.focus_distance};
@@ -771,7 +773,8 @@
     auto accumulate_batch = [&]() -> int {
         if ((rc = begin_event(c, 3, &ep))) return rc;
         const PrtAccumulateArgs aa{d_rad, lit ? c->lb.lrad : nullptr, c->film.local.as<float4>(), c->film.stat.as<float2>(), tm, S_cur, max_depth,
-                                   accumulate, c->ray_stats_target, compact ? c->wk.pix.as<float4>() + tm.n_pix_local : nullptr, view.list};
+                                   accumulate, c->ray_stats_target, compact ? c->wk.pix.as<float4>() + tm.n_pix_local : nullptr, view.list,
+                                   pixel_major_ids};
         if (!prt_launch_accumulate(c->stream, plan.accumulate, aa)) return fail(c, PRT_ERR_INVALID, "no such accumulate instance");
         c->batch_instance[PRT_STAGE_ACCUMULATE] = prt_accumulate_name(plan.accumulate);
         if ((rc = end_event(c, &ep))) return rc;
@@ -794,7 +797,7 @@
     }
     if (compact && c->pix_entries < tm.n_pix_local) {
         c->pix_entries = 0;
-        c->primary_key.valid = false;
+        c->primary_key.batch.valid = false;
         HIPCHECK(c, c->wk.pix.ensure(4 * (size_t)tm.n_pix_local * sizeof(float4)));
         c->pix_entries = tm.n_pix_local;
         c->pix_records_blank = false;
@@ -805,7 +808,8 @@
     float4* const d_pix = c->wk.pix.as<float4>();
     PrtRayBuf rb0 = c->rb[0];
     if (persistent) rb0.t = c->prim.pid.as<float4>(), rb0.hd2 = c->prim.list.as<float>(), rb0.hit = c->prim.hit.as<uint32_t>();
-    PrtPrimaryKey now{};
+    PrtPrimaryStageKey now_stage{};
+    PrtPrimaryKey& now = now_stage.batch;
     now.valid = persistent && c->primary_reuse != 0 && !instrumented;
     if (now.valid) {
         const PrtWalkPlan wp0 = prt_plan_walk(walk_facts(c, c->tune, PRT_WALK_CLOSEST, walk ? tm.n_pix_local : n_paths, false, true));
@@ -818,7 +822,8 @@
         now.rr_depth = c->sampling.rr_depth, now.clamp = c->sampling.clamp;
         now.listed = view.list != nullptr, now.instrumented = instrumented, now.exact = exact;
     }
-    const bool reuse = prt_primary_reusable(c->primary_key, now);
+    now_stage.id_order = pixel_major_ids ? 1u : 0u, now_stage.id_S = pixel_major_ids ? S_cur : 0u;
+    const bool reuse = prt_primary_stage_reusable(c->primary_key, now_stage);
     c->primary_reuse_active = reuse ? 1u : 0u;
     if (reuse) ++c->primary_reused_batches;
     if (reuse) HIPCHECK(c, hipMemsetAsync(d_counts + PRT_CNT_STRIDE, 0, (size_t)max_depth * PRT_CNT_STRIDE * sizeof(uint32_t), c->stream));
@@ -831,16 +836,16 @@
         HIPCHECK(c, hipMemsetAsync(c->lb.lrad, 0, (size_t)n_paths * sizeof(float4), c->stream));
     }
     c->batch_walked = walk;
-    const PrtPrimary primary{(const uint32_t*)rb0.t, d_pix, {c->cam.pos.x, c->cam.pos.y, c->cam.pos.z}, tm.n_pix_local,
-                             1.0f / (float)tm.n_pix_local, first_sample, seed, walk ? 1u : 0u};
+    const PrtPrimary primary{(const uint32_t*)rb0.t, d_pix, {c->cam.pos.x, c->cam.pos.y, c->cam.pos.z},
+                             prt_path_id_order(tm.n_pix_local, S_cur, pixel_major_ids), first_sample, seed, walk ? 1u : 0u};
     PrtPrimary primary_list = primary;
-    if (walk) primary_list.pid = (const uint32_t*)rb0.hd2;
+    if (walk) primary_list.pid = (const uint32_t*)rb0.hd2, primary_list.ids = prt_path_id_order(tm.n_pix_local, S_cur, false);
     c->batch_instance[PRT_STAGE_RAYGEN] = prt_raygen_name(plan.raygen);
     if (!reuse) {
-        c->primary_key.valid = false;
+        c->primary_key.batch.valid = false;
         if ((rc = begin_event(c, 0, &ep))) return rc;
         const PrtRaygenArgs ra{&c->dsc, c->cam, tm, n_paths, first_sample, seed, max_depth, rb0, d_rad, d_counts, d_work, c->sampling,
-                               compact ? d_pix : nullptr, walk, f.env ? &denv : nullptr, f.lens ? &dlens : nullptr, view.list};
+                               compact ? d_pix : nullptr, walk, pixel_major_ids, f.env ? &denv : nullptr, f.lens ? &dlens : nullptr, view.list};
         if (!prt_launch_raygen(c->stream, plan.raygen, ra)) return fail(c, PRT_ERR_INVALID, "no such raygen instance");
         if ((rc = end_event(c, &ep))) return rc;
         if (exact) HIPCHECK(c, read_back(0));
@@ -887,7 +892,7 @@
             if (d == 0) c->primary_counts[0] = h_counts[0], c->primary_counts[1] = h_counts[32];
         }
         if (n_rays_known == 0u) break;
-        if (d == 0 && !reuse && now.valid) c->primary_key = now;
+        if (d == 0 && !reuse && now.valid) c->primary_key = now_stage;
         if (c->d_shade_div) prt_launch_shade_divstats(c->stream, c->dsc, in, d_counts, d, n_paths, c->d_shade_div, prim_d);
         if ((rc = begin_event(c, 2, &ep))) return rc;
         const PrtShadeInst shade = d == 0 ? plan.shade0 : plan.shade;
@@ -3961,6 +3966,7 @@
     else if (n == "last_segment" && value >= 0 && value <= 2) c->last_segment = (uint32_t)value;
     else if (n == "compact_primary" && (value == 0 || value == 1)) c->compact_primary = value;
     else if (n == "primary_walk" && (value == 0 || value == 1)) c->primary_walk = value;
+    else if (n == "path_id_order" && (value == 0 || value == 1)) c->path_id_order = value;
     else if (n == "node_stride" && (value == 0 || value == 5 || value == 8)) c->node_stride = value;
     else if (n == "pad_log2" && value >= 8 && value <= 22) c->pad_coeff = std::ldexp(1.0f, -value);
     else if (n == "tail" && value >= 0 && value <= 64) c->tune.tail = (uint32_t)value;
diff --git a/parallelraytracing_amd/csrc/prt_kernels.h b/parallelraytracing_amd/csrc/prt_kernels.h
--- a/parallelraytracing_amd/csrc/prt_kernels.h
+++ b/parallelraytracing_amd/csrc/prt_kernels.h
@@ -4,6 +4,7 @@
 #include <stdint.h>
 
 #include "../../include/prt.h"
+#include "prt_path_id.h"
 #include "prt_route.h"
 #include "prt_walk.h"
 #include "prt_scene_pod.h"
@@ -75,8 +76,7 @@
     const uint32_t* pid;
     const float4* pix;
     float origin[3];
-    uint32_t n_pix_local;
-    float inv_n;
+    PrtPathIdOrder ids;
     uint32_t first_sample, seed;
     uint32_t walk;
 };
@@ -157,6 +157,7 @@
     PrtSampling sp;
     float4* compact_pix;
     bool primary_walk;
+    bool pixel_major_ids;
     const DevEnv* env;
     const DevLens* lens;
     const uint32_t* list;
@@ -212,6 +213,7 @@
     unsigned long long* ray_stats;
     const float4* pix_end;
     const uint32_t* list;
+    bool pixel_major_ids;
 };
 bool prt_launch_accumulate(hipStream_t st, PrtAccumulateInst inst, const PrtAccumulateArgs& a);
 void prt_launch_resolve(hipStream_t st, const float4* gathered, uint32_t world, uint32_t stride, uint32_t W,
diff --git a/parallelraytracing_amd/csrc/prt_kernels.hip b/parallelraytracing_amd/csrc/prt_kernels.hip
--- a/parallelraytracing_amd/csrc/prt_kernels.hip
+++ b/parallelraytracing_amd/csrc/prt_kernels.hip
@@ -116,17 +116,8 @@
 }
 
 PRT_DEV void primary_ray(const PrtPrimary& pr, uint32_t i, f3& o, f3& d, uint32_t& pixel, uint32_t& sample, uint32_t* local_pixel = nullptr) {
-    uint32_t q = (uint32_t)((float)i * pr.inv_n);
-    uint32_t r = i - q * pr.n_pix_local;
-    if ((int32_t)r < 0) {
-        --q;
-        r += pr.n_pix_local;
-    }
-    if (r >= pr.n_pix_local) {
-        ++q;
-        r -= pr.n_pix_local;
-    }
-    sample = q;
+    uint32_t r;
+    prt_path_id_decode(pr.ids, i, r, sample);
     if (local_pixel) *local_pixel = r;
     const float4 P = pr.pix[r];
     o = mk3(pr.origin[0], pr.origin[1], pr.origin[2]);
@@ -236,8 +227,10 @@
                          float4* __restrict__ ro, float4* __restrict__ rd, float4* __restrict__ rt, uint32_t* __restrict__ hit,
                          float* __restrict__ hd2, float4* __restrict__ rad, uint32_t* __restrict__ counts,
                          uint32_t* __restrict__ work, uint32_t max_depth, PrtSampling sp_arg, float4* __restrict__ pix,
-                         const DevEnv* env, const DevLens* lens = nullptr, const uint32_t* __restrict__ list = nullptr) {
+                         const DevEnv* env, const DevLens* lens = nullptr, const uint32_t* __restrict__ list = nullptr,
+                         uint32_t pixel_major_ids = 0u) {
     const PrtSampling sp = SAMPLING ? sp_arg : PrtSampling{0u, 0u, 0.0f};
+    const PrtPathIdOrder ids{tm.n_pix_local, 0.0f, (COMPACT && pixel_major_ids) ? S : 0u, 0u, 0u};
     const uint32_t pl = blockIdx.x * (uint32_t)PRODUCER_BLOCK + threadIdx.x;
     if (blockIdx.y == 0 && pl < 8u) work[32u * pl] = 0u;
     if (blockIdx.y == 0 && pl == 8u) work[512] = 0u;
@@ -290,10 +283,10 @@
                 ((uint32_t*)hd2)[list_slot] = pl;
             }
         }
-        if (s1 - s0 < 8u) {
+        if (s1 - s0 < PRT_PATH_ID_MIN_SAMPLES) {
             if (in_range && slot0 != 0xFFFFFFFFu) {
                 for (uint32_t sl = s0; sl < s1; ++sl) {
-                    const uint32_t i = sl * tm.n_pix_local + pl;
+                    const uint32_t i = prt_path_id_encode(ids, pl, sl);
                     const uint32_t slot = front ? slot0 + (sl - s0) * stride : slot0 - (sl - s0) * stride;
                     if (COMPACT) {
                         ((uint32_t*)rt)[slot] = i;
@@ -334,7 +327,7 @@
                 }
                 if (lane < mult) {
                     const uint32_t slot = fr ? f + lane : f - lane;
-                    const uint32_t i = (s0 + lane) * tm.n_pix_local + plp;
+                    const uint32_t i = prt_path_id_encode(ids, plp, s0 + lane);
                     if (COMPACT) {
                         ((uint32_t*)rt)[slot] = i;
                     } else {
@@ -428,9 +421,10 @@
                                                             float4* __restrict__ rt, uint32_t* __restrict__ hit,
                                                             float* __restrict__ hd2, float4* __restrict__ rad,
                                                             uint32_t* __restrict__ counts, uint32_t* __restrict__ work,
-                                                            uint32_t max_depth, PrtSampling sp_arg, float4* __restrict__ pix) {
+                                                            uint32_t max_depth, PrtSampling sp_arg, float4* __restrict__ pix,
+                                                            uint32_t pixel_major_ids) {
     raygen_step<JITTER, SAMPLING, ABVH, COMPACT, false>(sc, cam, tm, S, first_sample, seed, ro, rd, rt, hit, hd2, rad, counts, work,
-                                                        max_depth, sp_arg, pix, nullptr);
+                                                        max_depth, sp_arg, pix, nullptr, nullptr, nullptr, COMPACT ? pixel_major_ids : 0u);
 }
 
 template <bool JITTER, bool ABVH>
@@ -1851,7 +1845,7 @@
                             f3 po, pd;
                             uint32_t pixel, sample, lp;
                             primary_ray(pr, ld_stream(&pr.pid[qi]), po, pd, pixel, sample, &lp);
-                            const float4 E = pr.pix[pr.n_pix_local + lp];
+                            const float4 E = pr.pix[pr.ids.n_pix_local + lp];
                             hid = __float_as_uint(E.y);
                             hd2_0 = E.z;
 #ifndef PRT_NO_OPAQUE_ORIGIN
@@ -2205,13 +2199,13 @@
             pid = ld_stream(&pr.pid[src]);
             uint32_t pixel, sample, lp;
             primary_ray(pr, pid, o, d, pixel, sample, &lp);
-            if (k >= nA) id = __float_as_uint(pr.pix[pr.n_pix_local + lp].y);
-            else if (pr.walk) id = hit[__float_as_uint(pr.pix[pr.n_pix_local + lp].x)];
+            if (k >= nA) id = __float_as_uint(pr.pix[pr.ids.n_pix_local + lp].y);
+            else if (pr.walk) id = hit[__float_as_uint(pr.pix[pr.ids.n_pix_local + lp].x)];
             rng = path_seed(pixel, pr.first_sample + sample, pr.seed);
             depth = 0u;
             thr = mk3(1.f, 1.f, 1.f);
-            pre_a = pr.pix[2u * pr.n_pix_local + lp];
-            pre_b = pr.pix[3u * pr.n_pix_local + lp];
+            pre_a = pr.pix[2u * pr.ids.n_pix_local + lp];
+            pre_b = pr.pix[3u * pr.ids.n_pix_local + lp];
         } else {
             const float4 O = ld_stream(&ro[src]);
             const float4 D = ld_stream(&rd[src]);
@@ -2282,8 +2276,8 @@
 __global__ void __launch_bounds__(256) k_primary_hit(DevScene sc, PrtPrimary pr, const uint32_t* __restrict__ hit,
                                                      float4* __restrict__ pix, const uint32_t* __restrict__ counts) {
     const uint32_t pl = blockIdx.x * 256u + threadIdx.x;
-    if (pl >= pr.n_pix_local) return;
-    const float4 E = pix[pr.n_pix_local + pl];
+    if (pl >= pr.ids.n_pix_local) return;
+    const float4 E = pix[pr.ids.n_pix_local + pl];
     float4 a = make_float4(0.f, 0.f, 0.f, __uint_as_float(HIT_DEAD)), b = make_float4(0.f, 0.f, 0.f, 0.f);
     if (__float_as_uint(E.w) == 0xFFFFFFFEu) {
         const uint32_t first = __float_as_uint(E.x);
@@ -2299,8 +2293,8 @@
             }
         }
     }
-    pix[2u * pr.n_pix_local + pl] = a;
-    pix[3u * pr.n_pix_local + pl] = b;
+    pix[2u * pr.ids.n_pix_local + pl] = a;
+    pix[3u * pr.ids.n_pix_local + pl] = b;
 }
 
 __global__ void __launch_bounds__(SHADE_BLOCK) k_shade_divstats(DevScene sc, const uint32_t* __restrict__ hit,
@@ -2318,7 +2312,7 @@
             f3 o_, d_;
             uint32_t pixel, sample, lp;
             primary_ray(pr, pr.pid[src], o_, d_, pixel, sample, &lp);
-            const float4 E = pr.pix[pr.n_pix_local + lp];
+            const float4 E = pr.pix[pr.ids.n_pix_local + lp];
             id = k >= nA ? __float_as_uint(E.y) : hit[__float_as_uint(E.x)];
         } else {
             id = hit[src];
@@ -2532,6 +2526,105 @@
     if (valid && update_film) {
         film_local[fl] = f;
         stat[fl] = m2;
+    }
+    }
+    __syncthreads();
+    if (threadIdx.x < max_depth) {
+        unsigned long long n = 0;
+        for (uint32_t e = threadIdx.x; e < max_depth; ++e) n += s_ends[e];
+        if (n) atomicAdd(&ray_stats[(blockIdx.x & (PRT_RAY_STAT_SLOTS - 1u)) * PRT_MAX_DEPTH + threadIdx.x], n);
+    }
+}
+
+#ifndef PRT_ACC_PM_CHUNK
+#define PRT_ACC_PM_CHUNK 8
+#endif
+#define PRT_ACC_PM_BLOCK (PRT_ACC_PM_CHUNK == 8 ? 256 : 128)
+template <bool STAT>
+__global__ void __launch_bounds__(PRT_ACC_PM_BLOCK) k_accumulate_pixel_major(const float4* __restrict__ rad, float4* __restrict__ film_local,
+                                                                float2* __restrict__ stat, PrtTileMap tm, uint32_t S, uint32_t max_depth,
+                                                                int update_film, unsigned long long* __restrict__ ray_stats,
+                                                                const float4* __restrict__ pix_end) {
+    __shared__ uint32_t s_ends[PRT_MAX_DEPTH];
+    constexpr uint32_t C = PRT_ACC_PM_CHUNK, ROW = C + 1u, BLOCK = PRT_ACC_PM_BLOCK;
+    __shared__ float4 s_t[BLOCK / 64u][64u * ROW];
+    if (threadIdx.x < PRT_MAX_DEPTH) s_ends[threadIdx.x] = 0u;
+    __syncthreads();
+    const PrtPathIdOrder ids{tm.n_pix_local, 0.0f, S, 0u, 0u};
+    const uint32_t lane = lane_id(), wave = threadIdx.x >> 6;
+    float4* const t = s_t[wave];
+    for (uint32_t pl0 = blockIdx.x * BLOCK; pl0 < tm.n_pix_local; pl0 += gridDim.x * BLOCK) {
+    const uint32_t pl = pl0 + threadIdx.x;
+    const uint32_t wave_pl = pl0 + 64u * wave;
+    uint32_t x, y;
+    const bool valid = pl < tm.n_pix_local && tile_pixel(tm, pl, x, y);
+    float4 f = valid ? film_local[pl] : make_float4(0.f, 0.f, 0.f, 0.f);
+    float2 m2 = make_float2(0.f, 0.f);
+    if (STAT && valid) m2 = stat[pl];
+    float4 E = make_float4(0.f, 0.f, 0.f, __uint_as_float(0xFFFFFFFEu));
+    if (valid && pix_end) E = pix_end[pl];
+    const bool ended = __float_as_uint(E.w) != 0xFFFFFFFEu;
+    const unsigned long long need = __ballot(valid && !ended);
+    const float weight = 1.0f;
+    const bool packed = max_depth <= 8u;
+    unsigned long long h = 0ull;
+    const uint32_t cs = lane % C, cq = lane / C;
+    float4 v[C];
+    auto load_chunk = [&](uint32_t s0) {
+#pragma unroll
+        for (uint32_t j = 0; j < C; ++j) {
+            const uint32_t q = (64u / C) * j + cq;
+            v[j] = (((need >> q) & 1ull) != 0ull && s0 + cs < S) ? ld_stream(&rad[prt_path_id_encode(ids, wave_pl + q, s0 + cs)]) : E;
+        }
+    };
+    load_chunk(0u);
+    for (uint32_t s0 = 0; s0 < S; s0 += C) {
+#pragma unroll
+        for (uint32_t j = 0; j < C; ++j) t[((64u / C) * j + cq) * ROW + cs] = v[j];
+        __builtin_amdgcn_fence(__ATOMIC_RELEASE, "wavefront");
+        __builtin_amdgcn_wave_barrier();
+        __builtin_amdgcn_fence(__ATOMIC_ACQUIRE, "wavefront");
+        if (s0 + C < S) load_chunk(s0 + C);
+#pragma unroll
+        for (uint32_t j = 0; j < C; ++j) {
+            if (s0 + j >= S) break;
+            uint32_t e = 0xFFFFFFFFu;
+            if (valid) {
+                const float4 r = ended ? E : t[lane * ROW + j];
+                f.x += r.x * weight;
+                f.y += r.y * weight;
+                f.z += r.z * weight;
+                f.w += weight;
+                if (STAT) {
+                    const float lum = __fadd_rn(__fadd_rn(__fmul_rn(0.2126f, r.x), __fmul_rn(0.7152f, r.y)), __fmul_rn(0.0722f, r.z));
+                    m2.x = __fadd_rn(m2.x, lum);
+                    m2.y = __fadd_rn(m2.y, __fmul_rn(lum, lum));
+                }
+                e = __float_as_uint(r.w);
+            }
+            if (packed) {
+                if (e < 8u) h += 1ull << (8u * e);
+            } else {
+                for (uint32_t dd = 0; dd < max_depth; ++dd) {
+                    const unsigned long long mk = __ballot(e == dd);
+                    if (mk != 0ull && lane == 0) atomicAdd(&s_ends[dd], (uint32_t)__popcll(mk));
+                }
+            }
+        }
+        if (packed && ((s0 / C) % 31u == 30u || s0 + C >= S)) {
+            for (uint32_t dd = 0; dd < max_depth; ++dd) {
+                const uint32_t n = (uint32_t)(h >> (8u * dd)) & 0xFFu;
+                if (n) atomicAdd(&s_ends[dd], n);
+            }
+            h = 0ull;
+        }
+        __builtin_amdgcn_fence(__ATOMIC_RELEASE, "wavefront");
+        __builtin_amdgcn_wave_barrier();
+        __builtin_amdgcn_fence(__ATOMIC_ACQUIRE, "wavefront");
+    }
+    if (valid && update_film) {
+        film_local[pl] = f;
+        if (STAT) stat[pl] = m2;
     }
     }
     __syncthreads();
@@ -3274,8 +3367,8 @@
     const DevLens& l = or_empty(a.lens);
 #define PRT_RAYGEN_HEAD a.cam, a.tm, S, a.first_sample, a.seed, a.out.o, a.out.d, a.out.t, a.out.hit
 #define PRT_RAYGEN_TAIL a.rad, a.counts, a.work, a.max_depth, a.sp
-#define PRT_RAYGEN_ARGS_PLAIN sc, PRT_RAYGEN_HEAD, a.out.hd2, PRT_RAYGEN_TAIL, nullptr
-#define PRT_RAYGEN_ARGS_COMPACT sc, PRT_RAYGEN_HEAD, a.primary_walk ? a.out.hd2 : nullptr, PRT_RAYGEN_TAIL, a.compact_pix
+#define PRT_RAYGEN_ARGS_PLAIN sc, PRT_RAYGEN_HEAD, a.out.hd2, PRT_RAYGEN_TAIL, nullptr, 0u
+#define PRT_RAYGEN_ARGS_COMPACT sc, PRT_RAYGEN_HEAD, a.primary_walk ? a.out.hd2 : nullptr, PRT_RAYGEN_TAIL, a.compact_pix, a.pixel_major_ids ? 1u : 0u
 #define PRT_RAYGEN_ARGS_ENV sc, e, PRT_RAYGEN_HEAD, a.out.hd2, PRT_RAYGEN_TAIL
 #define PRT_RAYGEN_ARGS_LENS sc, l, PRT_RAYGEN_HEAD, a.out.hd2, PRT_RAYGEN_TAIL
 #define PRT_RAYGEN_ARGS_LENS_ENV sc, e, l, PRT_RAYGEN_HEAD, a.out.hd2, PRT_RAYGEN_TAIL
@@ -3466,13 +3559,25 @@
 
 void prt_launch_primary_hit(hipStream_t st, const DevScene& sc, const PrtPrimary& pr, const uint32_t* hit, float4* pix,
                             const uint32_t* counts) {
-    hipLaunchKernelGGL(k_primary_hit, dim3(blocks_for(pr.n_pix_local)), dim3(256), 0, st, sc, pr, hit, pix, counts);
+    hipLaunchKernelGGL(k_primary_hit, dim3(blocks_for(pr.ids.n_pix_local)), dim3(256), 0, st, sc, pr, hit, pix, counts);
 }
 
 bool prt_launch_accumulate(hipStream_t st, PrtAccumulateInst inst, const PrtAccumulateArgs& a) {
     const uint32_t nb = blocks_for(a.tm.n_pix_local ? a.tm.n_pix_local : 1);
     const dim3 grid(nb < 8192u ? nb : 8192u);
     const int upd = a.update_film ? 1 : 0;
+    if (a.pixel_major_ids) {
+        if (inst != PRT_I_k_accumulate && inst != PRT_INST(k_accumulate_stat, ff)) return false;
+        const uint32_t nbp = (a.tm.n_pix_local + PRT_ACC_PM_BLOCK - 1u) / PRT_ACC_PM_BLOCK;
+        const dim3 grid_pm(nbp < 8192u ? (nbp ? nbp : 1u) : 8192u);
+        if (inst == PRT_I_k_accumulate)
+            hipLaunchKernelGGL((k_accumulate_pixel_major<false>), grid_pm, dim3(PRT_ACC_PM_BLOCK), 0, st, a.rad, a.film_local, a.stat, a.tm, a.S, a.max_depth, upd,
+                               a.ray_stats, a.pix_end);
+        else
+            hipLaunchKernelGGL((k_accumulate_pixel_major<true>), grid_pm, dim3(PRT_ACC_PM_BLOCK), 0, st, a.rad, a.film_local, a.stat, a.tm, a.S, a.max_depth, upd,
+                               a.ray_stats, a.pix_end);
+        return true;
+    }
 #define PRT_ACC_ARGS_PLAIN a.rad, a.film_local, a.tm, a.S, a.max_depth, upd, a.ray_stats, a.pix_end
 #define PRT_ACC_ARGS_LIT a.rad, a.lrad, a.film_local, a.tm, a.S, a.max_depth, upd, a.ray_stats
 #define PRT_ACC_ARGS_STAT a.rad, a.lrad, a.film_local, a.stat, a.tm, a.S, a.max_depth, upd, a.ray_stats, a.pix_end, a.list
diff --git a/parallelraytracing_amd/csrc/prt_path_id.h b/parallelraytracing_amd/csrc/prt_path_id.h
--- /dev/null
+++ b/parallelraytracing_amd/csrc/prt_path_id.h
@@ -0,0 +1,61 @@
+#pragma once
+#include <cstdint>
+
+#if defined(__HIPCC__)
+#define PRT_PATH_ID_FN __host__ __device__ inline
+#else
+#define PRT_PATH_ID_FN inline
+#endif
+
+#define PRT_PATH_ID_MIN_SAMPLES 8u
+
+struct PrtPathIdOrder {
+    uint32_t n_pix_local;
+    float inv_n;
+    uint32_t S;
+    uint32_t magic, shift;
+};
+
+inline PrtPathIdOrder prt_path_id_order(uint32_t n_pix_local, uint32_t S, bool pixel_major) {
+    PrtPathIdOrder o{};
+    o.n_pix_local = n_pix_local;
+    o.inv_n = n_pix_local ? 1.0f / (float)n_pix_local : 0.0f;
+    if (pixel_major && S >= 2u && S <= 0x80000000u) {
+        uint32_t L = 1u;
+        while (L < 32u && (1ull << L) < S) ++L;
+        o.S = S;
+        o.magic = (uint32_t)(((1ull << 32) * ((1ull << L) - S)) / S + 1ull);
+        o.shift = L - 1u;
+    }
+    return o;
+}
+
+inline bool prt_path_id_pixel_major(bool compact, uint32_t S, int path_id_order) {
+    return compact && S >= PRT_PATH_ID_MIN_SAMPLES && path_id_order != 0;
+}
+
+PRT_PATH_ID_FN uint32_t prt_path_id_encode(const PrtPathIdOrder& o, uint32_t pixel_local, uint32_t sample) {
+    return o.S ? pixel_local * o.S + sample : sample * o.n_pix_local + pixel_local;
+}
+
+PRT_PATH_ID_FN void prt_path_id_decode(const PrtPathIdOrder& o, uint32_t id, uint32_t& pixel_local, uint32_t& sample) {
+    if (o.S) {
+        const uint32_t h = (uint32_t)(((uint64_t)id * o.magic) >> 32);
+        const uint32_t q = (((id - h) >> 1) + h) >> o.shift;
+        pixel_local = q;
+        sample = id - q * o.S;
+        return;
+    }
+    uint32_t q = (uint32_t)((float)id * o.inv_n);
+    uint32_t r = id - q * o.n_pix_local;
+    if ((int32_t)r < 0) {
+        --q;
+        r += o.n_pix_local;
+    }
+    if (r >= o.n_pix_local) {
+        ++q;
+        r -= o.n_pix_local;
+    }
+    sample = q;
+    pixel_local = r;
+}
diff --git a/parallelraytracing_amd/csrc/prt_primary_cache.h b/parallelraytracing_amd/csrc/prt_primary_cache.h
--- a/parallelraytracing_amd/csrc/prt_primary_cache.h
+++ b/parallelraytracing_amd/csrc/prt_primary_cache.h
@@ -36,3 +36,13 @@
            held.lens == now.lens && held.jitter == now.jitter && held.rr_depth == now.rr_depth && held.clamp == now.clamp &&
            held.listed == now.listed && held.instrumented == now.instrumented && held.exact == now.exact;
 }
+
+struct PrtPrimaryStageKey {
+    PrtPrimaryKey batch;
+    uint32_t id_order;
+    uint32_t id_S;
+};
+
+inline bool prt_primary_stage_reusable(const PrtPrimaryStageKey& held, const PrtPrimaryStageKey& now) {
+    return prt_primary_reusable(held.batch, now.batch) && held.id_order == now.id_order && held.id_S == now.id_S;
+}
```

After: 24880 Mrays/s (median of 6 runs). 1.02x the previous value.
